# rogeliorjr/DyCON_Paper_Replication

Measured on AMD Instinct MI355X. Metric: train volumes/sec (96^3 patch), higher is better.
Workload: dtype bf16

## Files before the change

dycon_paper_replication_amd/_lib.py:

```python
from __future__ import annotations

import ctypes as C
import os

_HERE = os.path.dirname(os.path.abspath(__file__))
LIB_PATH = os.environ.get("DYCON_LIB", os.path.join(_HERE, "libdycon_hip.so"))

F32, BF16 = 0, 1
CONV_1X1, CONV_K3, CONV_K2S2 = 0, 1, 2

P, I, L, F, Z, U64 = C.c_void_p, C.c_int, C.c_longlong, C.c_float, C.c_size_t, C.c_uint64

SIGNATURES = {
    "dycon_version": (I, []),
    "dycon_last_error": (C.c_char_p, []),
    "dycon_bfrag_bytes": (Z, [I, I, I, I]),
    "dycon_pack_bfrag": (I, [P, P, I, I, I, I, I, L, L, L, L, I, P]),
    "dycon_pack_batch": (I, [P, I, I, P]),
    "dycon_pack_tcn": (I, [P, P, I, I, I, I, L, L, L, L, I, P]),
    "dycon_conv_gemm_workspace": (Z, [I, I, I, I, I, I, I, I, I]),
    "dycon_conv_gemm_plan": (I, [I, I, I, I, I, I, I, I, I, I, I, P]),
    "dycon_conv_kernel_name": (C.c_char_p, [I]),
    "dycon_conv_region_name": (C.c_char_p, [P]),
    "dycon_conv_gemm": (I, [P, P, P, P, I, I, I, I, I, I, I, I, I, I, I, P, Z, P]),
    "dycon_conv_gemm_splits": (I, [I, I, I, I, I, I, I, I, I]),
    "dycon_conv_gemm_ex": (I, [P, P, P, P, I, I, I, I, I, I, I, I, I, I, I, P, Z, I, P]),
    "dycon_conv_direct": (I, [P, I, P, P, P, I, I, I, I, I, I, I, I, I, P]),
    "dycon_conv_wgrad_workspace": (Z, [I, I, I, I, I, I, I]),
    "dycon_conv_wgrad_name": (C.c_char_p, [I, I, I, I, I, I, I, I, I]),
    "dycon_conv_wgrad": (I, [P, I, P, I, P, P, I, I, I, I, I, I, I, L, L, L, P, Z, P]),
    "dycon_colsum_workspace": (Z, [L, I]),
    "dycon_colsum": (I, [P, I, P, L, I, P, Z, P]),
    "dycon_norm_workspace": (Z, [I, L, I]),
    "dycon_norm_stats": (I, [P, I, I, L, I, I, F, P, P, P, F, P, Z, P]),
    "dycon_norm_fwd": (I, [P, P, I, I, L, I, I, F, P, P, P, I, P, P, P, P, F, P, Z, P]),
    "dycon_norm_fwd_is_fused": (I, [I, L, I, I]),
    "dycon_norm_fwd_slab": (I, [P, I, P, P, P, I, I, L, I, I, F, P, P, P, I, P, P, P]),
    "dycon_norm_apply": (I, [P, P, I, I, L, I, I, P, P, P, I, P, P, P]),
    "dycon_norm_bwd": (I, [P, I, P, P, I, I, L, I, I, P, P, P, I, P, P, P, P, Z, P]),
    "dycon_norm_bwd_ex": (I, [P, I, P, P, I, I, L, I, I, P, P, P, I, P, P, P, I, P, Z, P]),
    "dycon_norm_sum_dparams": (I, [P, I, I, P, P, P]),
    "dycon_norm_head_workspace": (Z, [I, L]),
    "dycon_norm_head_fwd": (I, [P, I, I, L, I, P, P, P, I, P, P, P, P, P]),
    "dycon_norm_head_bwd": (I, [P, P, P, I, I, L, I, P, P, P, I, P, P, P, P, P, Z, P]),
    "dycon_norm_head_dparams": (I, [P, I, L, P, P, P]),
    "dycon_norm_headc_workspace": (Z, [I, L, I]),
    "dycon_norm_headc_fwd": (I, [P, I, I, L, I, I, P, P, P, I, P, P, P, P, P]),
    "dycon_norm_headc_bwd": (I, [P, P, P, I, I, L, I, I, P, P, P, I, P, P, P, P, P, Z, P]),
    "dycon_norm_headc_dparams": (I, [P, I, L, I, P, P, P]),
    "dycon_conv_stats_chunks": (I, [I, I, I, I, I, I, I, I]),
    "dycon_conv_gemm_stats": (I, [P, P, P, P, I, I, I, I, I, I, I, P, Z, P]),
    "dycon_norm_fwd_parts": (I, [P, P, I, I, L, I, I, F, P, P, P, I, P, P, P, P, F, P, I, P]),
    "dycon_norm_stats_parts": (I, [I, I, L, I, I, F, P, P, P, F, P, I, P]),
    "dycon_norm_bwd_ab_offset": (Z, [I, L, I]),
    "dycon_norm_bwd_stats": (I, [P, P, I, I, L, I, I, P, P, P, I, P, P, P, P, Z, P]),
    "dycon_first_block_bwd_workspace": (Z, [I, I, I, I]),
    "dycon_first_block_bwd": (I, [P, P, P, I, I, I, I, I, I, P, P, P, I, P, P, P, P, P, L, L, L, P, Z, P]),
    "dycon_conv1_wgrad_normbwd_workspace": (Z, [I, I, I, I]),
    "dycon_conv1_wgrad_normbwd": (I, [P, P, P, I, I, I, I, I, I, P, P, P, I, P, P, P, P, L, L, L, P, Z, P]),
    "dycon_norm_acc_doubles": (Z, [I, L, I]),
    "dycon_norm_fwd_acc": (I, [P, P, I, I, L, I, I, F, P, P, P, I, P, P, P, P, F, P, P]),
    "dycon_norm_bwd_acc": (I, [P, P, P, I, I, L, I, I, P, P, P, I, P, P, P, P, P, Z, P]),
    "dycon_maxpool2_fwd": (I, [P, P, P, I, I, I, I, I, I, P]),
    "dycon_maxpool2_bwd": (I, [P, P, P, I, I, I, I, I, I, P]),
    "dycon_trilinear_fwd": (I, [P, P, I, I, I, I, I, I, I, I, I, I, I, I, P]),
    "dycon_trilinear_bwd": (I, [P, P, I, I, I, I, I, I, I, I, I, I, I, I, P]),
    "dycon_upconv_k3": (I, [P, P, P, P, I, I, I, I, I, I, I, P]),
    "dycon_copy_channels": (I, [P, I, I, P, I, I, L, I, I, P]),
    "dycon_relu_fwd": (I, [P, P, P, P, I, I, L, I, P]),
    "dycon_relu_bwd": (I, [P, P, P, P, I, I, L, I, P]),
    "dycon_scale_channels": (I, [P, P, P, I, I, L, I, P]),
    "dycon_mul_mask": (I, [P, P, F, P, I, L, P]),
    "dycon_dropout_philox": (I, [P, P, I, L, F, U64, U64, P]),
    "dycon_channel_mask_philox": (I, [P, L, F, U64, U64, P]),
    "dycon_add_noise": (I, [P, P, P, I, L, F, F, U64, U64, P]),
    "dycon_tanh": (I, [P, I, P, L, P]),
    "dycon_cast": (I, [P, I, P, I, L, P]),
    "dycon_add": (I, [P, P, P, I, L, P]),
    "dycon_seg_losses_fwd": (I, [P, P, P, I, I, I, L, F, P, I, P]),
    "dycon_seg_losses_bwd": (I, [P, P, P, I, I, I, L, F, P, P, I, P, I, P]),
    "dycon_seg_losses_finalize": (I, [P, I, I, L, F, P, P]),
    "dycon_step_loss": (I, [P, P, F, F, F, I, I, P, P, P]),
    "dycon_step_losses": (I, [P, P, I, I, L, F, C.c_double, F, I, F, F, F, I, I, P, P, P]),
    "dycon_seg_lossesc_nsums": (I, [I]),
    "dycon_seg_lossesc_fwd": (I, [P, P, P, I, I, I, L, I, F, I, P, I, P]),
    "dycon_seg_lossesc_bwd": (I, [P, P, P, I, I, I, L, I, F, P, P, I, P, I, P]),
    "dycon_seg_lossesc_finalize": (I, [P, I, I, L, I, F, P, P]),
    "dycon_step_lossesc": (I, [P, P, I, I, L, I, F, C.c_double, F, I, F, F, F, I, I, P, P, P]),
    "dycon_softmax_mse_fwd": (I, [P, P, P, L, I, L, I, P]),
    "dycon_softmax_mse_bwd": (I, [P, P, P, P, L, I, L, I, P]),
    "dycon_softmax_kl_fwd": (I, [P, P, L, I, L, I, P, P, P]),
    "dycon_softmax_kl_bwd": (I, [P, P, L, I, L, I, I, P, P, P]),
    "dycon_dice_fwd": (I, [P, P, I, I, L, I, L, I, P, F, P, P, P]),
    "dycon_dice_bwd": (I, [P, P, I, I, L, I, L, I, P, F, P, P, P, P]),
    "dycon_dice1_fwd": (I, [P, P, I, L, I, L, I, P, P, P]),
    "dycon_dice1_bwd": (I, [P, P, I, L, I, L, I, P, P, P, P]),
    "dycon_entropy_fwd": (I, [P, L, I, L, F, P, P, P, P]),
    "dycon_entropy_bwd": (I, [P, L, I, L, F, P, P, P, P]),
    "dycon_sym_mse_fwd": (I, [P, P, L, P, P, P]),
    "dycon_sym_mse_bwd": (I, [P, P, L, P, P, P]),
    "dycon_kl_rows_fwd": (I, [P, L, P, L, L, L, L, I, P, P, P]),
    "dycon_kl_rows_bwd": (I, [P, L, P, L, L, L, L, I, P, P, L, P]),
    "dycon_focal_fwd": (I, [P, P, I, L, I, L, F, P, I, P, P, P]),
    "dycon_focal_bwd": (I, [P, P, I, L, I, L, F, P, I, P, P, P]),
    "dycon_uncl_fwd": (I, [P, P, L, I, L, F, P, P, P]),
    "dycon_uncl_bwd": (I, [P, P, L, I, L, F, P, P, P]),
    "dycon_l2norm_fwd": (I, [P, P, P, I, L, I, F, P]),
    "dycon_l2norm_bwd": (I, [P, P, P, P, I, L, I, F, P]),
    "dycon_mask_pool": (I, [P, I, P, I, I, I, I, I, I, I, P]),
    "dycon_fecl_workspace": (Z, [I, I, I]),
    "dycon_fecl_fwd": (I, [P, P, P, P, I, I, I, I, F, F, I, F, F, P, P, P, Z, P]),
    "dycon_fecl_finalize": (I, [P, C.c_double, F, I, P, P]),
    "dycon_set_scalars": (I, [P, I, F, F, F, F, F, F, F, F, P]),
    "dycon_fecl_bwd": (I, [P, P, P, P, I, I, I, I, F, F, I, F, F, P, P, P, P, Z, P]),
    "dycon_fecl_rows_workspace": (Z, [I, I, I]),
    "dycon_fecl_fwd_rows": (I, [P, P, P, P, I, I, I, I, F, F, P, P, Z, Z, P]),
    "dycon_fecl_gambling_finalize": (I, [P, P, I, I, I, I, P, P, P, P, Z, P, Z, P]),
    "dycon_fecl_gambling_grad": (I, [P, P, L, P, P]),
    "dycon_gambling_softmax_fwd": (I, [P, P, L, I, P]),
    "dycon_gambling_softmax_bwd": (I, [P, P, P, L, I, P]),
    "dycon_gambling_uncertainty_fwd": (I, [P, I, I, I, I, I, I, I, P, I, P]),
    "dycon_gambling_uncertainty_bwd": (I, [P, I, I, I, I, I, I, I, P, P, I, P]),
    "dycon_sumsq": (I, [P, L, P, P]),
    "dycon_sgd_ema": (I, [P, P, P, P, L, L, P, F, F, F, F, F, F, P, P]),
    "dycon_nonfinite_flag": (I, [P, P, P]),
    "dycon_sw_accumulate": (I, [P, I, I, I, I, P, P, P, I, I, I, P]),
    "dycon_sw_accumulate_c": (I, [P, I, I, I, I, I, P, P, P, I, I, I, P]),
    "dycon_sw_finalize": (I, [P, P, L, F, P, P, P]),
    "dycon_binary_overlap": (I, [P, P, I, L, P, P]),
    "dycon_batch_overlap": (I, [P, P, I, I, L, P, P]),
    "dycon_sw_accumulate_all": (I, [P, I, I, I, I, I, P, P, P, I, I, I, P, P, P]),
    "dycon_sw_finalize_argmax": (I, [P, P, I, L, P, P, P]),
    "dycon_argmax_labels": (I, [P, I, L, P, P]),
    "dycon_class_confusion": (I, [P, P, I, L, I, P, P]),
    "dycon_batch_class_confusion": (I, [P, P, I, I, L, I, P, P]),
    "dycon_surface_workspace": (Z, [I, I, I, I]),
    "dycon_surface_hist": (I, [P, I, P, I, I, I, I, I, I, I, P, P, P, Z, P]),
    "dycon_surface_metrics": (I, [P, P, I, I, C.c_double, P, P]),
    "dycon_cc_workspace": (Z, [I, I, I, I]),
    "dycon_cc_roots": (I, [P, I, I, I, I, I, I, I, P, P]),
    "dycon_cc_labels": (I, [P, I, I, I, I, P, P, P, Z, P]),
    "dycon_cc_largest": (I, [P, I, P, I, I, I, I, I, P, P, P, P, Z, P]),
    "dycon_simhist_workspace": (Z, [I, I, I, I]),
    "dycon_simhist": (I, [P, P, I, I, I, I, F, I, P, P, P, P, Z, P]),
    "dycon_tap_gather": (I, [P, P, I, I, I, I, I, I, P, I, P]),
    "dycon_pack_wblocks": (I, [P, P, I, P, I, I, I, I, P, Z, I, P]),
    "dycon_unpack_wgrad": (I, [P, L, I, P, P, P, I, I, I, P]),
    "dycon_sample_colsum": (I, [P, I, P, I, L, I, F, I, P]),
    "dycon_sample_bcast": (I, [P, P, P, I, I, L, I, F, P]),
    "dycon_small_gemm": (I, [P, L, L, P, L, L, P, L, I, I, I, I, P]),
    "dycon_copy_segments": (I, [P, P, P, I, P]),
    "dycon_kernel_timing": (I, [I]),
    "dycon_kernel_timing_count": (L, []),
    "dycon_kernel_timing_fetch": (I, [L, L, P, P, P]),
    "dycon_kernel_timing_name": (C.c_char_p, [I]),
}


class ConvPlan(C.Structure):
    _fields_ = [("family", I), ("splits", I), ("chunks", I), ("weights", I), ("workspace", Z)]


CONV_NONE, CONV_C1, CONV_P16, CONV_P32, CONV_LDS, CONV_HALO, CONV_TILE, CONV_GEMM = range(8)
CONV_W_FRAG, CONV_W_CHUNK16 = 0, 1


class View(C.Structure):
    _fields_ = [("p", P), ("sn", L), ("sc", L), ("sv", L)]


class DyconLibraryError(RuntimeError):
    pass


_lib = None


def load():
    global _lib
    if _lib is not None:
        return _lib
    if not os.path.exists(LIB_PATH):
        raise DyconLibraryError(
            f"{LIB_PATH} not found: the HIP extension is not built.  Run "
            "`python -c 'import __graft_entry__ as g; g.build()'` from the repo root.  "
            "There is no CPU/PyTorch fallback for the DyCON hot path.")
    lib = C.CDLL(LIB_PATH)
    for name, (res, args) in SIGNATURES.items():
        try:
            fn = getattr(lib, name)
        except AttributeError as e:
            raise DyconLibraryError(f"{LIB_PATH} does not export {name}") from e
        fn.restype = res
        fn.argtypes = args
    _lib = lib
    return lib


class Recorder:

    def __init__(self):
        self.entries, self.keep = [], []

    def replay(self):
        for e in self.entries:
            if type(e) is list:
                rc = e[0](*e[1])
                if rc:
                    raise DyconLibraryError(f"{e[2]} failed ({rc}) in replay: {load().dycon_last_error().decode()}")
            else:
                e()


RECORDER = None

HIP_EVENT_DISABLE_TIMING, HIP_EVENT_NO_SYSTEM_FENCE = 0x2, 0x20000000
_hip = None


def hip():
    global _hip
    if _hip is None:
        h = C.CDLL("libamdhip64.so")
        h.hipEventCreateWithFlags.restype, h.hipEventCreateWithFlags.argtypes = I, [C.POINTER(P), C.c_uint]
        h.hipEventRecord.restype, h.hipEventRecord.argtypes = I, [P, P]
        h.hipStreamWaitEvent.restype, h.hipStreamWaitEvent.argtypes = I, [P, P, C.c_uint]
        h.hipEventDestroy.restype, h.hipEventDestroy.argtypes = I, [P]
        _hip = h
    return _hip


class HipEvent:
    __slots__ = ("h",)

    def __init__(self):
        ev = P()
        rc = hip().hipEventCreateWithFlags(C.byref(ev), HIP_EVENT_DISABLE_TIMING | HIP_EVENT_NO_SYSTEM_FENCE)
        if rc:
            raise DyconLibraryError(f"hipEventCreateWithFlags failed ({rc})")
        self.h = ev.value

    def __del__(self):
        try:
            if self.h and _hip is not None:
                _hip.hipEventDestroy(self.h)
        except Exception:
            pass


def hip_call(name, *args, keep=None):
    fn = getattr(hip(), name)
    rc = fn(*args)
    if rc:
        raise DyconLibraryError(f"{name} failed ({rc})")
    if RECORDER is not None:
        RECORDER.entries.append([fn, list(args), name])
        if keep is not None:
            RECORDER.keep.append(keep)


def call(name, *args):
    lib = load()
    fn = getattr(lib, name)
    rc = fn(*args)
    if rc != 0:
        raise DyconLibraryError(f"{name} failed ({rc}): {lib.dycon_last_error().decode()}")
    if RECORDER is not None:
        RECORDER.entries.append([fn, list(args), name])


_QUERY_CACHE = {}


def query(name, *args):
    key = (name,) + args
    try:
        return _QUERY_CACHE[key]
    except KeyError:
        v = _QUERY_CACHE[key] = getattr(load(), name)(*args)
        return v
```

dycon_paper_replication_amd/csrc/norm.hip:

```cpp
#include "common.h"
#include <type_traits>

struct NormPlan { int chunks; long long rows_per_chunk; };
static NormPlan norm_plan(long long V) {
    NormPlan p;
    constexpr long long maxc = 256, minr = 128;
    long long rpc = (V + maxc - 1) / maxc;
    if (rpc < minr) rpc = minr;
    p.rows_per_chunk = rpc;
    p.chunks = (int)((V + rpc - 1) / rpc);
    return p;
}

template <typename T, int MODE>
__global__ __launch_bounds__(256) void norm_partial_kernel(const T* __restrict__ S, const T* __restrict__ GY,
                                                           float* __restrict__ part, long long V, int C, int G,
                                                           long long rows_per_chunk, const float* __restrict__ stats,
                                                           const float* __restrict__ gamma, const float* __restrict__ beta,
                                                           int relu, int from_y, const float* __restrict__ chan_scale,
                                                           double* __restrict__ acc = nullptr, int nslots = 1) {
    constexpr int VN = Vec16<T>::N;
    typedef typename std::conditional<sizeof(T) == 4, double, float>::type A;
    __shared__ A sm[2][256][VN + 1];
    const int n = blockIdx.y, chunk = blockIdx.x;
// ... 417 lines not shown
            if (running_mean && gridDim.x == 1 && G == C) {
                running_mean[g] = (1.f - momentum) * running_mean[g] + momentum * (float)mean;
                const double unb = cnt > 1.0 ? var * cnt / (cnt - 1.0) : var;
                running_var[g] = (1.f - momentum) * running_var[g] + momentum * (float)unb;
            }
        }
    }
    T* yp = Y + (long long)n * V * C + c0;
    const T* sp = skip ? skip + (long long)n * V * C + c0 : nullptr;
    Vec16<T> sr[NF_ROWS][NVEC];
    if (sp) {
#pragma unroll
        for (int i = 0; i < NF_ROWS; ++i) {
            const long long v = threadIdx.x + 256 * i, vc = v < V ? v : V - 1;
#pragma unroll
            for (int q = 0; q < NVEC; ++q) sr[i][q] = ld16(sp + vc * C + q * VN);
        }
    }
#pragma unroll
    for (int i = 0; i < NF_ROWS; ++i) {
        const long long v = threadIdx.x + 256 * i;
        if (v < V) {
#pragma unroll
            for (int q = 0; q < NVEC; ++q) {
                Vec16<T> y;
#pragma unroll
                for (int k = 0; k < VN; ++k) {
                    float f = xr[i][q].get(k) * sc[q * VN + k] + sh[q * VN + k];
                    if (relu) f = f < 0.f ? 0.f : f;
                    f *= cs[q * VN + k];
                    if (sp) f += sr[i][q].get(k);
                    y.set(k, f);
                }
                st16(yp + v * C + q * VN, y);
            }
        }
    }
}

template <typename T, int SPAN, int CPG, int NF_ROWS>
__global__ __launch_bounds__(256) void norm_fused_bwd_kernel(const T* __restrict__ X, const T* __restrict__ GY, T* __restrict__ GX,
                                                             long long V, int C, int G, const float* __restrict__ stats,
                                                             const float* __restrict__ gamma, const float* __restrict__ beta,
                                                             int relu, const float* __restrict__ chan_scale,
                                                             float* __restrict__ dpart ) {
    constexpr int VN = Vec16<T>::N, NVEC = SPAN / VN;
    __shared__ float sm[4 * 2 * SPAN];
    constexpr int cpg = CPG;
    const int n = blockIdx.x, c0 = blockIdx.y * SPAN;
    const T* xp = X + (long long)n * V * C + c0;
    const T* gp = GY + (long long)n * V * C + c0;
    float mean[SPAN], rstd[SPAN], gm[SPAN], bt[SPAN], cs[SPAN];
#pragma unroll
    for (int k = 0; k < SPAN; ++k) {
        const int c = c0 + k, g = c / cpg;
        mean[k] = stats[((long long)n * G + g) * 2];
        rstd[k] = stats[((long long)n * G + g) * 2 + 1];
        gm[k] = gamma ? gamma[c] : 1.f;
        bt[k] = beta ? beta[c] : 0.f;
        cs[k] = chan_scale ? chan_scale[(long long)n * C + c] : 1.f;
    }
    float acc[2 * SPAN];
#pragma unroll
    for (int k = 0; k < 2 * SPAN; ++k) acc[k] = 0.f;
    Vec16<T> xr[NF_ROWS][NVEC], gr[NF_ROWS][NVEC];
#pragma unroll
    for (int i = 0; i < NF_ROWS; ++i) {
        const long long v = threadIdx.x + 256 * i, vc = v < V ? v : V - 1;
#pragma unroll
        for (int q = 0; q < NVEC; ++q) { xr[i][q] = ld16(xp + vc * C + q * VN); gr[i][q] = ld16(gp + vc * C + q * VN); }
    }
#pragma unroll
    for (int i = 0; i < NF_ROWS; ++i) {
        const bool ok = (long long)threadIdx.x + 256 * i < V;
#pragma unroll
        for (int q = 0; q < NVEC; ++q) {
#pragma unroll
            for (int k = 0; k < VN; ++k) {
                const int j = q * VN + k;
                const float xh = (xr[i][q].get(k) - mean[j]) * rstd[j];
                float g = gr[i][q].get(k) * cs[j];
                if ((relu && !(gm[j] * xh + bt[j] > 0.f)) || !ok) g = 0.f;
                acc[j] += g;
                acc[SPAN + j] += g * xh;
            }
        }
    }
    block_reduce_vec<2 * SPAN>(acc, sm);
    if (dpart && threadIdx.x == 0) {
#pragma unroll
        for (int k = 0; k < SPAN; ++k) {
            float* d = dpart + ((long long)n * C + c0 + k) * 2;
            d[0] = acc[k];
            d[1] = acc[SPAN + k];
        }
    }
    float A[SPAN], Bq[SPAN];
    const float inv_cnt = 1.f / ((float)V * (float)cpg);
#pragma unroll
    for (int k = 0; k < SPAN; ++k) {
        const int gl = k / cpg;
        float a = 0.f, bq = 0.f;
#pragma unroll
        for (int j = 0; j < SPAN; ++j)
            if (j / cpg == gl) { a += gm[j] * acc[j]; bq += gm[j] * acc[SPAN + j]; }
        A[k] = a * inv_cnt;
        Bq[k] = bq * inv_cnt;
    }
    T* op = GX + (long long)n * V * C + c0;
#pragma unroll
    for (int i = 0; i < NF_ROWS; ++i) {
        const long long v = threadIdx.x + 256 * i;
        if (v < V) {
#pragma unroll
            for (int q = 0; q < NVEC; ++q) {
                Vec16<T> o;
#pragma unroll
                for (int k = 0; k < VN; ++k) {
                    const int j = q * VN + k;
                    const float xh = (xr[i][q].get(k) - mean[j]) * rstd[j];
                    float g = gr[i][q].get(k) * cs[j];
                    if (relu && !(gm[j] * xh + bt[j] > 0.f)) g = 0.f;
                    o.set(k, rstd[j] * (gm[j] * g - (A[j] + xh * Bq[j])));
                }
                st16(op + v * C + q * VN, o);
            }
        }
    }
}

__global__ void norm_sum_dparams_kernel(const float* __restrict__ dpart, int Nb, int C, float* dgamma, float* dbeta) {
    const int c = blockIdx.x * blockDim.x + threadIdx.x;
    if (c >= C) return;
    float s0 = 0.f, s1 = 0.f;
    for (int n = 0; n < Nb; ++n) { s0 += dpart[((long long)n * C + c) * 2]; s1 += dpart[((long long)n * C + c) * 2 + 1]; }
    if (dbeta) dbeta[c] = s0;
    if (dgamma) dgamma[c] = s1;
}

static bool norm_fused_ok(int dtype, long long V, int C, int G) {
    const int VN = dtype == DYCON_BF16 ? 8 : 4, cpg = C / G;
    const int span = cpg > VN ? cpg : VN;
    return V <= 2048 && (cpg & (cpg - 1)) == 0 && cpg <= 16 && C % span == 0 && (span == 4 || span == 8 || span == 16);
}

extern "C" size_t dycon_norm_workspace(int Nb, long long V, int C) {
    const NormPlan p = norm_plan(V);
    return ((size_t)Nb * p.chunks * C * 2 + (size_t)Nb * C * 2 + 64) * sizeof(float);
}

static int norm_check(const char* who, int dtype, int Nb, long long V, int C, int G) {
    const int VN = dtype == DYCON_BF16 ? 8 : 4;
    DYCON_REQUIRE(Nb > 0 && V > 0 && C > 0 && G > 0 && C % G == 0, "%s: bad shape Nb=%d V=%lld C=%d G=%d", who, Nb, V, C, G);
    DYCON_REQUIRE(C % VN == 0 && C / VN <= 256, "%s: C=%d must be a multiple of %d and <= %d", who, C, VN, 256 * VN);
    DYCON_REQUIRE(Nb <= 65535, "%s: Nb too large", who);
    return DYCON_OK;
}

extern "C" int dycon_norm_fwd_is_fused(int dtype, long long V, int C, int G) {
    return (G > 0 && C % G == 0 && norm_fused_ok(dtype, V, C, G)) ? 1 : 0;
}

extern "C" int dycon_norm_fwd_slab(const float* slab, int splits, const float* conv_bias, void* x_out, void* y, int dtype, int Nb,
                                   long long V, int C, int G, float eps, float* stats, const float* gamma, const float* beta,
                                   int relu, const void* skip, const float* chan_scale, dycon_stream_t stream) {
    DYCON_REQUIRE(slab && x_out && y && stats && splits > 0, "norm_fwd_slab: bad arguments");
    DYCON_REQUIRE(dtype == DYCON_BF16, "norm_fwd_slab: bf16 storage only");
    if (int e = norm_check("norm_fwd_slab", dtype, Nb, V, C, G)) return e;
    DYCON_REQUIRE(norm_fused_ok(dtype, V, C, G), "norm_fwd_slab: this shape is not served by the one-launch norm (ask dycon_norm_fwd_is_fused)");
    const int cpg = C / G, span = cpg > 8 ? cpg : 8;
    const long long MN = (long long)Nb * V * C;
    dim3 grid(Nb, C / span);
#define DYCON_NFS_(SP, CP, RW) norm_fused_fwd_kernel<bf16, SP, CP, true, RW><<<grid, 256, 0, stream>>>((bf16*)x_out, (bf16*)y, V, C, G, eps, stats, gamma, beta, relu, (const bf16*)skip, chan_scale, nullptr, nullptr, 0.f, slab, splits, MN, conv_bias)
#define DYCON_NFS(SP, CP) do { if (V <= 256) DYCON_NFS_(SP, CP, 1); else DYCON_NFS_(SP, CP, 8); } while (0)
    if (cpg == 1) DYCON_NFS(8, 1); else if (cpg == 2) DYCON_NFS(8, 2); else if (cpg == 4) DYCON_NFS(8, 4);
    else if (cpg == 8) DYCON_NFS(8, 8); else DYCON_NFS(16, 16);
#undef DYCON_NFS
#undef DYCON_NFS_
    DYCON_LAUNCH_CHECK();
    return DYCON_OK;
}

extern "C" int dycon_norm_stats(const void* x, int dtype, int Nb, long long V, int C, int G, float eps, float* stats,
                                float* running_mean, float* running_var, float momentum, float* workspace, size_t ws_bytes,
                                dycon_stream_t stream) {
    DYCON_REQUIRE(x && stats && workspace, "norm_stats: null pointer");
    if (int e = norm_check("norm_stats", dtype, Nb, V, C, G)) return e;
    DYCON_REQUIRE(ws_bytes >= dycon_norm_workspace(Nb, V, C), "norm_stats: workspace too small");
    const NormPlan p = norm_plan(V);
    dim3 grid(p.chunks, Nb);
    DYCON_DISPATCH(dtype, {
        norm_partial_kernel<T, 0><<<grid, 256, 0, stream>>>((const T*)x, nullptr, workspace, V, C, G, p.rows_per_chunk, nullptr,
                                                            nullptr, nullptr, 0, 0, nullptr);
    });
    DYCON_LAUNCH_CHECK();
    norm_finalize_stats_kernel<<<Nb * G, 256, 0, stream>>>(workspace, Nb, p.chunks, C, G, V, eps, stats, running_mean, running_var, momentum);
    DYCON_LAUNCH_CHECK();
    return DYCON_OK;
}

extern "C" int dycon_norm_fwd(const void* x, void* y, int dtype, int Nb, long long V, int C, int G, float eps, float* stats,
                              const float* gamma, const float* beta, int relu, const void* skip, const float* chan_scale,
                              float* running_mean, float* running_var, float momentum, float* workspace, size_t ws_bytes,
                              dycon_stream_t stream) {
    DYCON_REQUIRE(x && y && stats, "norm_fwd: null pointer");
    if (int e = norm_check("norm_fwd", dtype, Nb, V, C, G)) return e;
    if (norm_fused_ok(dtype, V, C, G)) {
        const int VN = dtype == DYCON_BF16 ? 8 : 4, cpg = C / G;
        const int span = cpg > VN ? cpg : VN;
        dim3 grid(Nb, C / span);
#define DYCON_NF_(TT, SP, CP, RW) norm_fused_fwd_kernel<TT, SP, CP, false, RW><<<grid, 256, 0, stream>>>((TT*)const_cast<void*>(x), (TT*)y, V, C, G, eps, stats, gamma, beta, relu, (const TT*)skip, chan_scale, running_mean, running_var, momentum, nullptr, 0, 0, nullptr)
#define DYCON_NF(TT, SP, CP) do { if (V <= 256) DYCON_NF_(TT, SP, CP, 1); else DYCON_NF_(TT, SP, CP, 8); } while (0)
        if (dtype == DYCON_BF16) {
            if (cpg == 1) DYCON_NF(bf16, 8, 1); else if (cpg == 2) DYCON_NF(bf16, 8, 2); else if (cpg == 4) DYCON_NF(bf16, 8, 4);
            else if (cpg == 8) DYCON_NF(bf16, 8, 8); else DYCON_NF(bf16, 16, 16);
        } else {
            if (cpg == 1) DYCON_NF(float, 4, 1); else if (cpg == 2) DYCON_NF(float, 4, 2); else if (cpg == 4) DYCON_NF(float, 4, 4);
            else if (cpg == 8) DYCON_NF(float, 8, 8); else DYCON_NF(float, 16, 16);
        }
#undef DYCON_NF
#undef DYCON_NF_
        DYCON_LAUNCH_CHECK();
        return DYCON_OK;
    }
    DYCON_REQUIRE(workspace, "norm_fwd: workspace missing");
    if (int e = dycon_norm_stats(x, dtype, Nb, V, C, G, eps, stats, running_mean, running_var, momentum, workspace, ws_bytes, stream)) return e;
    return dycon_norm_apply(x, y, dtype, Nb, V, C, G, stats, gamma, beta, relu, skip, chan_scale, stream);
}

static int apply_grid(long long V, int C, int VN) {
    constexpr long long vpt = 4, cap = 2048;
    long long blocks = (V * C / VN + 256 * vpt - 1) / (256 * vpt);
    if (blocks > cap) blocks = cap;
    if (blocks < 1) blocks = 1;
    return (int)blocks;
}

extern "C" int dycon_norm_apply(const void* x, void* y, int dtype, int Nb, long long V, int C, int G, const float* stats,
                                const float* gamma, const float* beta, int relu, const void* skip, const float* chan_scale,
                                dycon_stream_t stream) {
    DYCON_REQUIRE(x && y && stats, "norm_apply: null pointer");
    if (int e = norm_check("norm_apply", dtype, Nb, V, C, G)) return e;
    DYCON_DISPATCH(dtype, {
        dim3 grid(apply_grid(V, C, Vec16<T>::N), Nb);
        norm_apply_kernel<T, false><<<grid, 256, 3 * C * sizeof(float), stream>>>((const T*)x, (T*)y, V, C, G, stats, gamma, beta, relu,
                                                                                  (const T*)skip, chan_scale);
    });
    DYCON_LAUNCH_CHECK();
    return DYCON_OK;
}

extern "C" int dycon_norm_fwd_parts(const void* x, void* y, int dtype, int Nb, long long V, int C, int G, float eps, float* stats,
                                    const float* gamma, const float* beta, int relu, const void* skip, const float* chan_scale,
                                    float* running_mean, float* running_var, float momentum, const float* part, int chunks,
                                    dycon_stream_t stream) {
    DYCON_REQUIRE(x && y && stats && part && chunks > 0, "norm_fwd_parts: bad arguments");
    if (int e = norm_check("norm_fwd_parts", dtype, Nb, V, C, G)) return e;
    norm_finalize_stats_kernel<<<Nb * G, 256, 0, stream>>>(part, Nb, chunks, C, G, V, eps, stats, running_mean, running_var, momentum);
    DYCON_LAUNCH_CHECK();
    return dycon_norm_apply(x, y, dtype, Nb, V, C, G, stats, gamma, beta, relu, skip, chan_scale, stream);
}

extern "C" int dycon_norm_stats_parts(int dtype, int Nb, long long V, int C, int G, float eps, float* stats, float* running_mean,
                                      float* running_var, float momentum, const float* part, int chunks, dycon_stream_t stream) {
    DYCON_REQUIRE(stats && part && chunks > 0, "norm_stats_parts: bad arguments");
    if (int e = norm_check("norm_stats_parts", dtype, Nb, V, C, G)) return e;
    norm_finalize_stats_kernel<<<Nb * G, 256, 0, stream>>>(part, Nb, chunks, C, G, V, eps, stats, running_mean, running_var, momentum);
    DYCON_LAUNCH_CHECK();
    return DYCON_OK;
}

extern "C" int dycon_norm_bwd(const void* src, int from_y, const void* gy, void* gx, int dtype, int Nb, long long V, int C,
                              int G, const float* stats, const float* gamma, const float* beta, int relu,
                              const float* chan_scale, float* dgamma, float* dbeta, float* workspace, size_t ws_bytes,
                              dycon_stream_t stream) {
    return dycon_norm_bwd_ex(src, from_y, gy, gx, dtype, Nb, V, C, G, stats, gamma, beta, relu, chan_scale, dgamma, dbeta, 0, workspace,
                             ws_bytes, stream);
}

extern "C" size_t dycon_norm_bwd_ab_offset(int Nb, long long V, int C) {
    const NormPlan p = norm_plan(V);
    return (size_t)Nb * p.chunks * C * 2;
}
extern "C" int dycon_norm_bwd_stats(const void* src, const void* gy, int dtype, int Nb, long long V, int C, int G, const float* stats,
                                    const float* gamma, const float* beta, int relu, const float* chan_scale, float* dgamma,
                                    float* dbeta, float* workspace, size_t ws_bytes, dycon_stream_t stream) {
    DYCON_REQUIRE(src && gy && stats && workspace, "norm_bwd_stats: null pointer");
    if (int e = norm_check("norm_bwd_stats", dtype, Nb, V, C, G)) return e;
    DYCON_REQUIRE(ws_bytes >= dycon_norm_workspace(Nb, V, C), "norm_bwd_stats: workspace too small");
    const NormPlan p = norm_plan(V);
    float* ab = workspace + dycon_norm_bwd_ab_offset(Nb, V, C);
    dim3 grid(p.chunks, Nb);
    DYCON_DISPATCH(dtype, {
        norm_partial_kernel<T, 1><<<grid, 256, 0, stream>>>((const T*)src, (const T*)gy, workspace, V, C, G, p.rows_per_chunk,
                                                            stats, gamma, beta, relu, 0, chan_scale);
    });
    DYCON_LAUNCH_CHECK();
    const int nfin = Nb * G + ((dgamma || dbeta) ? C : 0);
    norm_finalize_bwd_kernel<<<nfin, 256, 0, stream>>>(workspace, Nb, p.chunks, C, G, gamma, ab, dgamma, dbeta);
    DYCON_LAUNCH_CHECK();
    return DYCON_OK;
}

extern "C" int dycon_norm_sum_dparams(const float* workspace, int Nb, int C, float* dgamma, float* dbeta, dycon_stream_t stream) {
    DYCON_REQUIRE(workspace && Nb > 0 && C > 0 && (dgamma || dbeta), "norm_sum_dparams: bad arguments");
    norm_sum_dparams_kernel<<<cdiv(C, 256), 256, 0, stream>>>(workspace, Nb, C, dgamma, dbeta);
    DYCON_LAUNCH_CHECK();
    return DYCON_OK;
}

extern "C" int dycon_norm_bwd_ex(const void* src, int from_y, const void* gy, void* gx, int dtype, int Nb, long long V, int C,
                                 int G, const float* stats, const float* gamma, const float* beta, int relu,
                                 const float* chan_scale, float* dgamma, float* dbeta, int defer_dparams, float* workspace,
                                 size_t ws_bytes, dycon_stream_t stream) {
    DYCON_REQUIRE(src && gy && gx && stats && workspace, "norm_bwd: null pointer");
    if (int e = norm_check("norm_bwd", dtype, Nb, V, C, G)) return e;
    DYCON_REQUIRE(ws_bytes >= dycon_norm_workspace(Nb, V, C), "norm_bwd: workspace too small");
    if (!from_y && norm_fused_ok(dtype, V, C, G)) {
        const int VN = dtype == DYCON_BF16 ? 8 : 4, cpg = C / G;
        const int span = cpg > VN ? cpg : VN;
        const bool want = dgamma || dbeta;
        dim3 grid(Nb, C / span);
#define DYCON_NB_(TT, SP, CP, RW) norm_fused_bwd_kernel<TT, SP, CP, RW><<<grid, 256, 0, stream>>>((const TT*)src, (const TT*)gy, (TT*)gx, V, C, G, stats, gamma, beta, relu, chan_scale, want ? workspace : nullptr)
#define DYCON_NB(TT, SP, CP) do { if (V <= 256) DYCON_NB_(TT, SP, CP, 1); else DYCON_NB_(TT, SP, CP, 8); } while (0)
        if (dtype == DYCON_BF16) {
            if (cpg == 1) DYCON_NB(bf16, 8, 1); else if (cpg == 2) DYCON_NB(bf16, 8, 2); else if (cpg == 4) DYCON_NB(bf16, 8, 4);
            else if (cpg == 8) DYCON_NB(bf16, 8, 8); else DYCON_NB(bf16, 16, 16);
        } else {
            if (cpg == 1) DYCON_NB(float, 4, 1); else if (cpg == 2) DYCON_NB(float, 4, 2); else if (cpg == 4) DYCON_NB(float, 4, 4);
            else if (cpg == 8) DYCON_NB(float, 8, 8); else DYCON_NB(float, 16, 16);
        }
#undef DYCON_NB
#undef DYCON_NB_
        DYCON_LAUNCH_CHECK();
        if (want && !defer_dparams) {
            norm_sum_dparams_kernel<<<cdiv(C, 256), 256, 0, stream>>>(workspace, Nb, C, dgamma, dbeta);
            DYCON_LAUNCH_CHECK();
        }
        return DYCON_OK;
    }
    const NormPlan p = norm_plan(V);
    float* ab = workspace + (size_t)Nb * p.chunks * C * 2;
    dim3 grid(p.chunks, Nb);
    DYCON_DISPATCH(dtype, {
        norm_partial_kernel<T, 1><<<grid, 256, 0, stream>>>((const T*)src, (const T*)gy, workspace, V, C, G, p.rows_per_chunk,
                                                            stats, gamma, beta, relu, from_y, chan_scale);
    });
    DYCON_LAUNCH_CHECK();
    const int nfin = Nb * G + ((dgamma || dbeta) ? C : 0);
    norm_finalize_bwd_kernel<<<nfin, 256, 0, stream>>>(workspace, Nb, p.chunks, C, G, gamma, ab, dgamma, dbeta);
    DYCON_LAUNCH_CHECK();
    DYCON_DISPATCH(dtype, {
        dim3 grid2(apply_grid(V, C, Vec16<T>::N), Nb);
        norm_bwd_apply_kernel<T, false><<<grid2, 256, 7 * C * sizeof(float), stream>>>((const T*)src, (const T*)gy, (T*)gx, V, C, G, stats,
                                                                                       gamma, beta, ab, relu, from_y, chan_scale);
    });
    DYCON_LAUNCH_CHECK();
    return DYCON_OK;
}

constexpr int HC = 16;
constexpr int HK_MAX = 8;
constexpr int hpart_len(int hk) { return hk * HC + hk; }

template <typename T> __device__ __forceinline__ float round_to(float v) { T t; stf(&t, v); return ldf(&t); }

template <int HK> __device__ __forceinline__ void ld_row(const float* __restrict__ p, float (&r)[HK]) {
    if constexpr (HK % 4 == 0) {
#pragma unroll
        for (int k = 0; k < HK; k += 4) {
            const float4 t = *reinterpret_cast<const float4*>(p + k);
            r[k] = t.x; r[k + 1] = t.y; r[k + 2] = t.z; r[k + 3] = t.w;
        }
    } else if constexpr (HK % 2 == 0) {
#pragma unroll
        for (int k = 0; k < HK; k += 2) {
            const float2 t = *reinterpret_cast<const float2*>(p + k);
            r[k] = t.x; r[k + 1] = t.y;
        }
    } else {
#pragma unroll
        for (int k = 0; k < HK; ++k) r[k] = p[k];
    }
}
template <int HK> __device__ __forceinline__ void st_row(float* __restrict__ p, const float (&r)[HK]) {
    if constexpr (HK % 4 == 0) {
#pragma unroll
        for (int k = 0; k < HK; k += 4) *reinterpret_cast<float4*>(p + k) = make_float4(r[k], r[k + 1], r[k + 2], r[k + 3]);
    } else if constexpr (HK % 2 == 0) {
#pragma unroll
        for (int k = 0; k < HK; k += 2) *reinterpret_cast<float2*>(p + k) = make_float2(r[k], r[k + 1]);
    } else {
#pragma unroll
        for (int k = 0; k < HK; ++k) p[k] = r[k];
    }
}

template <typename T, int HK>
__device__ __forceinline__ void norm_apply_head_body(const T* __restrict__ X, long long V, int G, const float* __restrict__ stats,
                                                     const float* __restrict__ gamma, const float* __restrict__ beta, int relu,
                                                     const float* __restrict__ chan_scale, const float* __restrict__ W,
                                                     const float* __restrict__ hb, float* __restrict__ L) {
    constexpr int VN = Vec16<T>::N;
    __shared__ float ss[3 * HC + HK * HC + HK];
    const int n = blockIdx.y, cpg = HC / G;
    if (threadIdx.x < HC) {
        const int c = threadIdx.x, g = c / cpg;
        const float mean = stats[((long long)n * G + g) * 2], rstd = stats[((long long)n * G + g) * 2 + 1];
        const float gm = gamma ? gamma[c] : 1.f, bt = beta ? beta[c] : 0.f;
        ss[c] = rstd * gm;
        ss[HC + c] = bt - mean * rstd * gm;
        ss[2 * HC + c] = chan_scale ? chan_scale[(long long)n * HC + c] : 1.f;
    }
    if (threadIdx.x < HK * HC) ss[3 * HC + threadIdx.x] = W[threadIdx.x];
    if (threadIdx.x < HK) ss[3 * HC + HK * HC + threadIdx.x] = hb ? hb[threadIdx.x] : 0.f;
    __syncthreads();
    constexpr bool WREG = HK == 1;
    float sc[HC], sh[HC], dr[HC], wr[WREG ? HK * HC : 1], hbias[HK];
#pragma unroll
    for (int c = 0; c < HC; ++c) { sc[c] = ss[c]; sh[c] = ss[HC + c]; dr[c] = ss[2 * HC + c]; }
    if constexpr (WREG) {
#pragma unroll
        for (int j = 0; j < HK * HC; ++j) wr[j] = ss[3 * HC + j];
    }
#pragma unroll
    for (int k = 0; k < HK; ++k) hbias[k] = ss[3 * HC + HK * HC + k];
    const float* wl = ss + 3 * HC;
    const T* xp = X + (long long)n * V * HC;
    float* lp = L + (long long)n * V * HK;
    for (long long v = (long long)blockIdx.x * 256 + threadIdx.x; v < V; v += (long long)gridDim.x * 256) {
        float o[HK];
#pragma unroll
        for (int k = 0; k < HK; ++k) o[k] = hbias[k];
#pragma unroll
        for (int c0 = 0; c0 < HC; c0 += VN) {
            const Vec16<T> x = ld16(xp + v * HC + c0);
#pragma unroll
            for (int k = 0; k < VN; ++k) {
                const int c = c0 + k;
                float y = x.get(k) * sc[c] + sh[c];
                if (relu) y = y < 0.f ? 0.f : y;
                y = round_to<T>(y * dr[c]);
#pragma unroll
                for (int kk = 0; kk < HK; ++kk) o[kk] = fmaf(y, WREG ? wr[WREG ? kk * HC + c : 0] : wl[kk * HC + c], o[kk]);
            }
        }
        st_row<HK>(lp + v * HK, o);
    }
}
template <typename T, int HK>
__global__ __launch_bounds__(256) void norm_apply_headc_kernel(const T* __restrict__ X, long long V, int G,
                                                               const float* __restrict__ stats, const float* __restrict__ gamma,
                                                               const float* __restrict__ beta, int relu,
                                                               const float* __restrict__ chan_scale, const float* __restrict__ W,
                                                               const float* __restrict__ hb, float* __restrict__ L) {
    norm_apply_head_body<T, HK>(X, V, G, stats, gamma, beta, relu, chan_scale, W, hb, L);
}

template <typename T, int HK>
__device__ __forceinline__ void norm_head_partial_body(const T* __restrict__ S, const float* __restrict__ GL, float* __restrict__ part,
                                                       float* __restrict__ hpart, long long V, int G, long long rows_per_chunk,
                                                       const float* __restrict__ stats, const float* __restrict__ gamma,
                                                       const float* __restrict__ beta, int relu, const float* __restrict__ chan_scale,
                                                       const float* __restrict__ W) {
    constexpr int VN = Vec16<T>::N;
    constexpr int NGRP = HC / VN, RPI = 256 / NGRP;
    constexpr int NQ = 2 + HK;
    constexpr int NR = NQ < 4 ? NQ : 4;
    constexpr int HPART = hpart_len(HK);
    constexpr bool WREG = HK == 1;
    __shared__ float sm[NR][256][VN + 1];
    __shared__ float sb[256][HK];
    __shared__ float sw[WREG ? 1 : HK * HC];
    const int n = blockIdx.y, chunk = blockIdx.x;
    const int cg = threadIdx.x % NGRP, rr = threadIdx.x / NGRP;
    const long long v0 = chunk * rows_per_chunk, v1 = min(V, v0 + rows_per_chunk);
    const int cpg = HC / G;
    if constexpr (!WREG) {
        if (threadIdx.x < HK * HC) sw[threadIdx.x] = W[threadIdx.x];
        __syncthreads();
    }
    float acc[NQ][VN], e[HK];
    float mean[VN], rstd[VN], gm[VN], bt[VN], cs[VN], sc[VN], sh[VN], wr[WREG ? HK : 1][VN];
#pragma unroll
    for (int kk = 0; kk < HK; ++kk) e[kk] = 0.f;
#pragma unroll
    for (int k = 0; k < VN; ++k) {
        const int c = cg * VN + k, g = c / cpg;
#pragma unroll
        for (int q = 0; q < NQ; ++q) acc[q][k] = 0.f;
        cs[k] = chan_scale ? chan_scale[(long long)n * HC + c] : 1.f;
        mean[k] = stats[((long long)n * G + g) * 2];
        rstd[k] = stats[((long long)n * G + g) * 2 + 1];
        gm[k] = gamma ? gamma[c] : 1.f;
        bt[k] = beta ? beta[c] : 0.f;
        sc[k] = rstd[k] * gm[k];
        sh[k] = bt[k] - mean[k] * rstd[k] * gm[k];
        if constexpr (WREG) {
#pragma unroll
            for (int kk = 0; kk < HK; ++kk) wr[kk][k] = W[kk * HC + c];
        }
    }
    const float* wl = sw + cg * VN;
    const T* sp = S + ((long long)n * V) * HC + cg * VN;
    const float* gp = GL + (long long)n * V * HK;
    for (long long v = v0 + rr; v < v1; v += RPI) {
        const Vec16<T> s = ld16(sp + v * HC);
        float gl[HK];
        ld_row<HK>(gp + v * HK, gl);
#pragma unroll
        for (int k = 0; k < VN; ++k) {
            float gyv = 0.f;
#pragma unroll
            for (int kk = 0; kk < HK; ++kk) gyv = fmaf(gl[kk], WREG ? wr[WREG ? kk : 0][k] : wl[kk * HC + k], gyv);
            float g = round_to<T>(gyv) * cs[k];
            const float x = s.get(k);
            const float xh = (x - mean[k]) * rstd[k];
            if (relu && !(gm[k] * xh + bt[k] > 0.f)) g = 0.f;
            acc[0][k] += g;
            acc[1][k] += g * xh;
            float y = x * sc[k] + sh[k];
            if (relu) y = y < 0.f ? 0.f : y;
            y = round_to<T>(y * cs[k]);
#pragma unroll
            for (int kk = 0; kk < HK; ++kk) acc[2 + kk][k] += gl[kk] * y;
        }
        if (cg == 0) {
#pragma unroll
            for (int kk = 0; kk < HK; ++kk) e[kk] += gl[kk];
        }
    }
#pragma unroll
    for (int kk = 0; kk < HK; ++kk) sb[threadIdx.x][kk] = e[kk];
    const long long item = (long long)n * gridDim.x + chunk;
#pragma unroll
    for (int r0 = 0; r0 < NQ; r0 += NR) {
        if (r0) __syncthreads();
#pragma unroll
        for (int j = 0; j < NR; ++j) {
            if (r0 + j < NQ) {
#pragma unroll
                for (int k = 0; k < VN; ++k) sm[j][threadIdx.x][k] = acc[r0 + j < NQ ? r0 + j : 0][k];
            }
        }
        __syncthreads();
        if (threadIdx.x < NR * HC) {
            const int j = threadIdx.x / HC, o = threadIdx.x % HC, og = o / VN, ok = o % VN, q = r0 + j;
            if (q < NQ) {
                float s0 = 0.f;
                for (int i = 0; i < RPI; ++i) s0 += sm[j][i * NGRP + og][ok];
                if (q < 2) part[((item * HC) + o) * 2 + q] = s0;
                else hpart[item * HPART + (q - 2) * HC + o] = s0;
            }
        } else if (r0 == 0 && threadIdx.x >= 128 && threadIdx.x < 128 + HK) {
            const int kk = threadIdx.x - 128;
            float s0 = 0.f;
            for (int i = 0; i < 256; ++i) s0 += sb[i][kk];
            hpart[item * HPART + HK * HC + kk] = s0;
        }
    }
}
template <typename T, int HK>
__global__ __launch_bounds__(256) void norm_head_partialc_kernel(const T* __restrict__ S, const float* __restrict__ GL,
                                                                 float* __restrict__ part, float* __restrict__ hpart, long long V,
                                                                 int G, long long rows_per_chunk, const float* __restrict__ stats,
                                                                 const float* __restrict__ gamma, const float* __restrict__ beta,
                                                                 int relu, const float* __restrict__ chan_scale,
                                                                 const float* __restrict__ W) {
    norm_head_partial_body<T, HK>(S, GL, part, hpart, V, G, rows_per_chunk, stats, gamma, beta, relu, chan_scale, W);
}

__global__ __launch_bounds__(256) void norm_headc_finalize_kernel(const float* __restrict__ hpart, int items, int hk,
                                                                 float* __restrict__ dW, float* __restrict__ db) {
    const int j = blockIdx.x, hpart_n = hpart_len(hk);
    double s0 = 0.0, s1 = 0.0;
    for (int e = threadIdx.x; e < items; e += 256) s0 += hpart[(long long)e * hpart_n + j];
    block_sum2_double(s0, s1);
    if (threadIdx.x == 0) {
        if (j < hk * HC) { if (dW) dW[j] = (float)s0; }
        else if (db) db[j - hk * HC] = (float)s0;
    }
}

template <typename T, int HK>
__device__ __forceinline__ void norm_head_bwd_apply_body(const T* __restrict__ S, const float* __restrict__ GL, T* __restrict__ GX,
                                                         long long V, int G, const float* __restrict__ stats,
                                                         const float* __restrict__ gamma, const float* __restrict__ beta,
                                                         const float* __restrict__ ab, int relu, const float* __restrict__ chan_scale,
                                                         const float* __restrict__ W) {
    constexpr int VN = Vec16<T>::N;
    constexpr int NGRP = HC / VN;
    constexpr bool WREG = HK == 1;
    __shared__ float sw[WREG ? 1 : HK * HC];
    if constexpr (!WREG) {
        if (threadIdx.x < HK * HC) sw[threadIdx.x] = W[threadIdx.x];
        __syncthreads();
    }
    const int n = blockIdx.y, cpg = HC / G;
    const float inv_cnt = 1.f / ((float)V * (float)cpg);
    const long long total = V * NGRP;
    const int cg = threadIdx.x % NGRP;
    float mu[VN], rs[VN], gmv[VN], btv[VN], pa[VN], pb[VN], dr[VN], wr[WREG ? HK : 1][VN];
#pragma unroll
    for (int k = 0; k < VN; ++k) {
        const int c = cg * VN + k, g = c / cpg;
        mu[k] = stats[((long long)n * G + g) * 2];
// ... 428 lines not shown
```

dycon_paper_replication_amd/engine.py:

```python
from __future__ import annotations

from collections import OrderedDict
from typing import Dict, Optional

import torch

from . import ops
from ._lib import CONV_1X1, CONV_C1, CONV_K2S2, CONV_K3, CONV_W_CHUNK16

UNET_FILTERS = (16, 32, 64, 128, 256)
VNET_NORMS = ("groupnorm", "instancenorm", "batchnorm", "none")


def _projection_spec(spec, c_in):
    spec["projection.0.weight"] = (512, c_in, 1, 1, 1)
    spec["projection.0.bias"] = (512,)
    spec["projection.1.weight"] = (512,)
    spec["projection.1.bias"] = (512,)
    spec["projection.3.weight"] = (256, 512, 1, 1, 1)
    spec["projection.3.bias"] = (256,)
    spec["projection.4.weight"] = (256,)
    spec["projection.4.bias"] = (256,)


def projection_buffers():
    return OrderedDict([("projection.1.running_mean", (512,)), ("projection.1.running_var", (512,)),
                        ("projection.1.num_batches_tracked", ()), ("projection.4.running_mean", (256,)),
                        ("projection.4.running_var", (256,)), ("projection.4.num_batches_tracked", ())])


def vnet_param_spec(in_ch=1, n_classes=2, normalization="groupnorm", nf=16):
    if normalization not in VNET_NORMS:
        raise ValueError(f"normalization must be one of {VNET_NORMS}")
    spec = OrderedDict()
    affine = normalization in ("groupnorm", "batchnorm")
    step = 2 if normalization == "none" else 3

    def block(name, n, cin, cout):
        for i in range(n):
            ci = cin if i == 0 else cout
            spec[f"{name}.conv.{step * i}.weight"] = (cout, ci, 3, 3, 3)
            spec[f"{name}.conv.{step * i}.bias"] = (cout,)
            if affine:
                spec[f"{name}.conv.{step * i + 1}.weight"] = (cout,)
                spec[f"{name}.conv.{step * i + 1}.bias"] = (cout,)

    def down(name, cin, cout):
        spec[f"{name}.conv.0.weight"] = (cout, cin, 2, 2, 2)
        spec[f"{name}.conv.0.bias"] = (cout,)
        if affine:
            spec[f"{name}.conv.1.weight"] = (cout,)
            spec[f"{name}.conv.1.bias"] = (cout,)

    def up(name, cin, cout):
        spec[f"{name}.conv.0.weight"] = (cin, cout, 2, 2, 2)
        spec[f"{name}.conv.0.bias"] = (cout,)
        if affine:
            spec[f"{name}.conv.1.weight"] = (cout,)
            spec[f"{name}.conv.1.bias"] = (cout,)

    block("block_one", 1, in_ch, nf); down("block_one_dw", nf, 2 * nf)
    block("block_two", 2, 2 * nf, 2 * nf); down("block_two_dw", 2 * nf, 4 * nf)
    block("block_three", 3, 4 * nf, 4 * nf); down("block_three_dw", 4 * nf, 8 * nf)
    block("block_four", 3, 8 * nf, 8 * nf); down("block_four_dw", 8 * nf, 16 * nf)
    block("block_five", 3, 16 * nf, 16 * nf); up("block_five_up", 16 * nf, 8 * nf)
    block("block_six", 3, 8 * nf, 8 * nf); up("block_six_up", 8 * nf, 4 * nf)
    block("block_seven", 3, 4 * nf, 4 * nf); up("block_seven_up", 4 * nf, 2 * nf)
    block("block_eight", 2, 2 * nf, 2 * nf); up("block_eight_up", 2 * nf, nf)
    block("block_nine", 1, nf, nf)
    spec["out_conv.weight"] = (n_classes, nf, 1, 1, 1)
    spec["out_conv.bias"] = (n_classes,)
    _projection_spec(spec, 16 * nf)
    return spec


def vnet_norm_sites(normalization="groupnorm"):
    if normalization == "none":
        return []
    sites = []
    for blk, n, nxt in (("block_one", 1, "block_one_dw"), ("block_two", 2, "block_two_dw"), ("block_three", 3, "block_three_dw"),
                        ("block_four", 3, "block_four_dw"), ("block_five", 3, "block_five_up"), ("block_six", 3, "block_six_up"),
                        ("block_seven", 3, "block_seven_up"), ("block_eight", 2, "block_eight_up"), ("block_nine", 1, None)):
        sites += [f"{blk}.conv.{3 * i + 1}" for i in range(n)]
        if nxt:
            sites.append(f"{nxt}.conv.1")
    return sites


ASPP_BN_SITES = tuple(f"aspp.aspp{j}.bn" for j in range(1, 5)) + ("aspp.bn_after_pool", "aspp.bn1")


def net_buffers(net_type, normalization="groupnorm", params=None):
    bufs = OrderedDict()
    if net_type == "vnet" and normalization == "batchnorm":
        spec = params if params is not None else vnet_param_spec(normalization=normalization)
        for site in vnet_norm_sites(normalization):
            c = tuple(spec[site + ".weight"])
            bufs[site + ".running_mean"], bufs[site + ".running_var"], bufs[site + ".num_batches_tracked"] = c, c, ()
    if net_type == "unet_3D" and params is not None and "aspp.conv1.weight" in params:
        for site in ASPP_BN_SITES:
            c = tuple(params[site + ".weight"])
            bufs[site + ".running_mean"], bufs[site + ".running_var"], bufs[site + ".num_batches_tracked"] = c, c, ()
    bufs.update(projection_buffers())
    return bufs


def aspp_param_spec(spec, c=256):
    for j, k in ((1, 1), (2, 3), (3, 3), (4, 3)):
        spec[f"aspp.aspp{j}.atrous_conv.weight"] = (c, c, k, k, k)
        spec[f"aspp.aspp{j}.bn.weight"] = (c,)
        spec[f"aspp.aspp{j}.bn.bias"] = (c,)
    spec["aspp.global_avg_pool.1.weight"] = (c, c, 1, 1, 1)
    spec["aspp.bn_after_pool.weight"] = (c,)
    spec["aspp.bn_after_pool.bias"] = (c,)
    spec["aspp.conv1.weight"] = (c, 5 * c, 1, 1, 1)
    spec["aspp.bn1.weight"] = (c,)
    spec["aspp.bn1.bias"] = (c,)


def unet_param_spec(in_ch=1, n_classes=2, use_aspp=False):
    spec = OrderedDict()
    f = UNET_FILTERS

    def uc(prefix, cin, cout):
        spec[f"{prefix}.conv1.0.weight"] = (cout, cin, 3, 3, 3)
        spec[f"{prefix}.conv1.0.bias"] = (cout,)
        spec[f"{prefix}.conv2.0.weight"] = (cout, cout, 3, 3, 3)
        spec[f"{prefix}.conv2.0.bias"] = (cout,)

    uc("conv1", in_ch, f[0]); uc("conv2", f[0], f[1]); uc("conv3", f[1], f[2]); uc("conv4", f[2], f[3])
    uc("center", f[3], f[4])
    uc("up_concat4.conv", f[4] + f[3], f[3]); uc("up_concat3.conv", f[3] + f[2], f[2])
    uc("up_concat2.conv", f[2] + f[1], f[1]); uc("up_concat1.conv", f[1] + f[0], f[0])
    spec["final.weight"] = (n_classes, f[0], 1, 1, 1)
    spec["final.bias"] = (n_classes,)
    spec["out_conv2.weight"] = (n_classes, f[0], 1, 1, 1)
    spec["out_conv2.bias"] = (n_classes,)
    if use_aspp:
        aspp_param_spec(spec, f[4])
    _projection_spec(spec, f[4])
    return spec


def param_spec(net_type, in_ch=1, n_classes=2, normalization="groupnorm", use_aspp=False):
    if net_type == "vnet":
        if use_aspp:
            raise ValueError("use_aspp applies to the U-Net only (the reference's VNet takes no use_aspp)")
        return vnet_param_spec(in_ch, n_classes, normalization)
    if net_type == "unet_3D":
        return unet_param_spec(in_ch, n_classes, use_aspp)
    raise ValueError(f"unknown net_type {net_type!r}")


class DropoutSpec:

    def __init__(self, mode="off", masks=None, seed=0, offset=0):
        self.mode, self.masks, self.seed, self.offset = mode, masks or {}, seed, offset


class Engine:
    def __init__(self, net_type: str, params: Dict[str, torch.Tensor], grads: Optional[Dict[str, torch.Tensor]] = None,
                 buffers: Optional[Dict[str, torch.Tensor]] = None, dtype=torch.float32, scale_factor=2,
                 normalization="groupnorm"):
        if net_type == "vnet" and normalization not in VNET_NORMS:
            raise ValueError(f"normalization must be one of {VNET_NORMS} (VNet.py:17-24)")
        self.net_type, self.p, self.g, self.buf = net_type, params, grads, buffers or {}
        self.dtype, self.scale_factor, self.normalization = dtype, scale_factor, normalization
        self.gen = 0
        self._packed = {}
        self._jobs, self._jobs_dev, self._packed_gen = [], None, -1
        self._xjobs = []
        self.use_aspp = net_type == "unet_3D" and "aspp.conv1.weight" in params
        self._aspp_plans = {}
        self._jobs_split, self._pack_event = False, None
        self.on_param_grads = None
        self.wgrad_stream = None
        self.wgrad_stream2 = None
        self._wg_flip = 0
        self.feat_stream = None
        self.mark = None
        self.Gs = {}
        self._head_range = (0, 0)
        self._wws = {}
        self.fuse_finish = False
        self.conv_stats = False
        self.conv_stats96 = False
        self._stat_parts = {}
        self._deferred = {}
        self._pending_dparams = []
        self.tape = []
        self.G = {}

    def params_changed(self):
        self.gen += 1

    def _pk(self, key, kind, w, T, Cin, N, N0, s_t, s_c, s_n1, s_n0, flip=False):
        hit = self._packed.get(key)
        if hit is not None and hit[0] == self.gen:
            return hit[1]
        buf = hit[1] if hit is not None else None
        if kind == "frag":
            buf = ops.pack_bfrag(w, self.dtype, T, Cin, N, N0, s_t, s_c, s_n1, s_n0, flip, out=buf)
            code = 0 if self.dtype == torch.bfloat16 else 1
        else:
            buf = ops.pack_tcn(w, T, Cin, N, N0, s_t, s_c, s_n1, s_n0, flip, out=buf)
            code = 2
        if hit is None:
            self._jobs.append((key, ops.pack_job(w, buf, code, T, Cin, N, N0, s_t, s_c, s_n1, s_n0, flip)))
            self._jobs_dev = None
        self._packed[key] = (self.gen, buf)
        return buf

    def _pk_chunked16(self, key, w, nchunks, N, s_t, s_c, s_n0, flip=False):
        hit = self._packed.get(key)
        if hit is not None and hit[0] == self.gen:
            return hit[1]
        per = ops.query("dycon_bfrag_bytes", ops.BF16, 27, 16, N) // 2
        buf = hit[1] if hit is not None else torch.empty(per * nchunks, dtype=torch.bfloat16, device=w.device)
        wflat = w.reshape(-1)
        for ch in range(nchunks):
            src, dst = wflat[ch * 16 * s_c:], buf[ch * per:(ch + 1) * per]
            ops.pack_bfrag(src, self.dtype, 27, 16, N, N, s_t, s_c, 0, s_n0, flip, out=dst)
            if hit is None:
                self._jobs.append(((key, ch), ops.pack_job(src, dst, 0, 27, 16, N, N, s_t, s_c, 0, s_n0, flip)))
                self._jobs_dev = None
        self._packed[key] = (self.gen, buf)
        return buf

    def repack(self, early=None, helper=None):
        self._pack_event = None
        if (not self._jobs and not self._xjobs) or self._packed_gen == self.gen:
            return
        split = early is not None and helper is not None
        if self._jobs_dev is None or self._jobs_split != split:
            dev = next(iter(self._packed.values()))[1].device
            name = lambda key: (key[0][0] if isinstance(key[0], tuple) else key[0])
            first = [j for k, j in self._jobs if split and name(k).startswith(early)]
            rest = [j for k, j in self._jobs if not (split and name(k).startswith(early))]
            self._jobs_dev = [(ops.upload_pack_jobs(js, dev), len(js), max(1, min(512, (max(j[6] for j in js) + 2047) // 2048)))
                              for js in (first, rest) if js]
            self._jobs_split = split
        if split and len(self._jobs_dev) == 2:
            (d0, n0, b0), (d1, n1, b1) = self._jobs_dev
            ops.pack_batch(d0, n0, b0)
            ops.fork(ops.cur_stream(), helper)
            with ops.on_stream(helper, light=True):
                ops.pack_batch(d1, n1, b1)
                self._repack_blocks()
                ev1 = ops.Event()
                ev1.record(helper)
            self._pack_event = ev1
        else:
            for d, n, b in self._jobs_dev:
                ops.pack_batch(d, n, b)
            self._repack_blocks()
        for key, _ in self._jobs:
            key = key[0] if isinstance(key[0], tuple) else key
            self._packed[key] = (self.gen, self._packed[key][1])
        self._packed_gen = self.gen

    def _pk_blocks(self, key, tables, KB, NB, kblk, nblk, device):
        hit = self._packed.get(key)
        if hit is not None and hit[0] == self.gen:
            return hit[1]
        buf = ops.pack_wblocks(tables, KB, NB, kblk, nblk, self.dtype, device, out=hit[1] if hit is not None else None)
        if hit is None:
            self._xjobs.append((key, tables, KB, NB, kblk, nblk))
        self._packed[key] = (self.gen, buf)
        return buf

    def _repack_blocks(self):
        for key, tables, KB, NB, kblk, nblk in self._xjobs:
            buf = self._packed[key][1]
            ops.pack_wblocks(tables, KB, NB, kblk, nblk, self.dtype, buf.device, out=buf)
            self._packed[key] = (self.gen, buf)

    def pack_ready(self):
        ev = getattr(self, "_pack_event", None)
        if ev is not None:
            ev.wait(ops.cur_stream())
            self._pack_event = None

    def _sync_to(self, key, g):
        if self.feat_stream is None:
            return
        cur = ops.cur_stream()
        src = self.Gs.get(key)
        if src is not None and src != cur:
            ops.fork(src, cur)
            g.record_stream(cur)

    def _take(self, t):
        g = self.G.pop(id(t))
        self._sync_to(id(t), g)
        self.Gs.pop(id(t), None)
        return g

    def _peek(self, t):
        g = self.G.get(id(t))
        if g is not None:
            self._sync_to(id(t), g)
        return g

    def _put(self, t, g):
        self.G[id(t)] = g
        if self.feat_stream is not None:
            self.Gs[id(t)] = ops.cur_stream()

    def _give(self, t, g):
        cur = self._peek(t)
        self._put(t, g if cur is None else ops.add(cur, g))

    def _conv(self, name, x, kind, need_gx=True, out_dtype=None, norm_groups=0):
        w, b = self.p[name + ".weight"], self.p[name + ".bias"]
        dtype = self.dtype
        if kind == "deconv":
            Cin, Cout = w.shape[0], w.shape[1]
        else:
            Cout, Cin = w.shape[0], w.shape[1]
        T = {"k3": 27, "k2s2": 8, "deconv": 8, "1x1": 1}[kind]
        mode = {"k3": CONV_K3, "k2s2": CONV_K2S2, "deconv": CONV_1X1, "1x1": CONV_1X1}[kind]
        gq = 8 if dtype == torch.bfloat16 else 4
        skinny = (Cin % gq != 0) or (Cout % 16 != 0)
        out_dtype = out_dtype or dtype
        plan = ops.conv_plan_for(x, mode, Cout, Cout) if kind == "k3" and out_dtype == dtype else None
        first_lds = plan is not None and plan.family == CONV_C1

        def conv_with_stats(wf, want):
            chunks = plan.chunks if (norm_groups and want) else 0
            if not chunks:
                return None
            y, part = ops.conv_gemm_stats(x, wf, b, Cout, chunks)
            self._stat_parts[id(y)] = (part, chunks)
            return y

        if first_lds:
            wf = self._pk((name, "f1"), "frag", w, 27, 1, Cout, Cout, 1, 27, 0, 27)
            y = conv_with_stats(wf, self.conv_stats96 and Cout == 16)
            if y is None:
                y = ops.conv_gemm(x, wf, b, CONV_K3, Cout, Cout)
        elif skinny:
            assert kind in ("k3", "1x1"), "skinny path only for the first conv and the 1x1 heads"
            wt = self._pk((name, "tcn"), "tcn", w, T, Cin, Cout, Cout, 1, T, 0, Cin * T)
            y = ops.conv_direct(x, wt, b, mode, Cout, out_dtype)
        elif kind == "deconv":
            wf = self._pk((name, "f"), "frag", w, 1, Cin, 8 * Cout, Cout, 0, Cout * 8, 1, 8)
            y = ops.conv_gemm(x, wf, b, CONV_1X1, 8 * Cout, Cout, scatter=True)
        elif plan is not None and plan.weights == CONV_W_CHUNK16:
            wf = self._pk_chunked16((name, "f48"), w, 3, Cout, 1, 27, Cin * 27)
            y = ops.conv_gemm(x, wf, b, mode, Cout, Cout)
        else:
            wf = self._pk((name, "f"), "frag", w, T, Cin, Cout, Cout, 1, T, 0, Cin * T)
            Vo = (x.shape[1] * x.shape[2] * x.shape[3]) // (8 if kind == "k2s2" else 1)
            want_stats = self.conv_stats96 if (Cin, Cout) == (16, 16) else self.conv_stats
            y = conv_with_stats(wf, want_stats and kind == "k3" and out_dtype == dtype and dtype == torch.bfloat16)
            if y is None and (norm_groups and self.fuse_finish and dtype == torch.bfloat16 and out_dtype == dtype
                              and ops.norm_fwd_is_fused(x, Vo, Cout, norm_groups)):
                y, dc = ops.conv_gemm(x, wf, b, mode, Cout, Cout, defer_finish=True)
                if dc is not None:
                    self._deferred[id(y)] = dc
            elif y is None:
                y = ops.conv_gemm(x, wf, b, mode, Cout, Cout)

        if self.recording:
            def wgrad(gy):
                gw, gb = self.g[name + ".weight"], self.g[name + ".bias"]
                wkey = (name, tuple(x.shape[:4]))
                ws = self._wws.get(wkey)
                if kind == "deconv":
                    if ws is None:
                        ws = self._wws[wkey] = (ops._ws(ops.query("dycon_colsum_workspace", gy.numel() // gy.shape[-1], gy.shape[-1]), gy),
                                                ops.conv_wgrad_workspace(gy, x, CONV_K2S2))
                    ops.colsum(gy, gb, ws=ws[0])
                    ops.conv_wgrad(gy, x, gw, CONV_K2S2, 1, 8, Cout * 8, ws=ws[1])
                else:
                    if ws is None:
                        ws = self._wws[wkey] = ops.conv_wgrad_workspace(x, gy, mode)
                    ops.conv_wgrad(x, gy, gw, mode, 1 if T > 1 else 0, T, Cin * T, dbias=gb, ws=ws)
                if self.on_param_grads is not None:
                    self.on_param_grads(name + ".weight")

            def bwd():
                gy = self._take(y)
                if self.wgrad_stream is not None:
                    wst = self.wgrad_stream
                    if self.wgrad_stream2 is not None:
                        self._wg_flip = (self._wg_flip + 1) % 2
                        wst = (self.wgrad_stream, self.wgrad_stream2)[self._wg_flip]
                    ops.fork(ops.cur_stream(), wst)
                    with ops.on_stream(wst, light=True):
                        self._flush_dparams()
                        wgrad(gy)
                    gy.record_stream(wst)
                else:
                    wgrad(gy)
                if not need_gx:
                    return
                cur = self._peek(x)
                if skinny:
                    wd = self._pk((name, "tcn_d"), "tcn", w, 1, Cout, Cin, Cin, 0, Cin, 0, 1)
                    gx = ops.conv_direct(gy, wd, None, CONV_1X1, Cin, x.dtype, out=cur, accumulate=cur is not None)
                elif kind == "k3":
                    if ops.conv_plan_for(gy, CONV_K3, Cin, Cin).weights == CONV_W_CHUNK16:
                        wd = self._pk_chunked16((name, "d48"), w, 3, Cin, 1, Cin * 27, 27, flip=True)
                    else:
                        wd = self._pk((name, "d"), "frag", w, 27, Cout, Cin, Cin, 1, Cin * 27, 0, 27, flip=True)
                    gx = ops.conv_gemm(gy, wd, None, CONV_K3, Cin, Cin, out=cur, accumulate=cur is not None)
                elif kind == "k2s2":
                    wd = self._pk((name, "d"), "frag", w, 1, Cout, 8 * Cin, Cin, 0, Cin * 8, 1, 8)
                    gx = ops.conv_gemm(gy, wd, None, CONV_1X1, 8 * Cin, Cin, scatter=True, out=cur, accumulate=cur is not None)
                elif kind == "deconv":
                    wd = self._pk((name, "d"), "frag", w, 8, Cout, Cin, Cin, 1, 8, 0, Cout * 8)
                    gx = ops.conv_gemm(gy, wd, None, CONV_K2S2, Cin, Cin, out=cur, accumulate=cur is not None)
                else:
                    wd = self._pk((name, "d"), "frag", w, 1, Cout, Cin, Cin, 0, Cin, 0, 1)
                    gx = ops.conv_gemm(gy, wd, None, CONV_1X1, Cin, Cin, out=cur, accumulate=cur is not None)
                self._put(x, gx)
            self.tape.append(bwd)
        return y

    def _flush_dparams(self):
        for pend in self._pending_dparams:
            ops.norm_sum_dparams(pend)
            pend[0].record_stream(ops.cur_stream())
        self._pending_dparams = []

    def _norm_site(self, prefix, z, kind):
        B, C = z.shape[0], z.shape[-1]
        V = z.numel() // (B * C)
        if kind == "in":
            return B, V, C, C, None, None, None, None
        if kind not in ("gn", "bn"):
            raise ValueError(kind)
        gamma, beta = self.p[prefix + ".weight"], self.p[prefix + ".bias"]
        if kind == "gn":
            return B, V, C, 16, gamma, beta, None, None
        return 1, B * V, C, C, gamma, beta, self.buf.get(prefix + ".running_mean"), self.buf.get(prefix + ".running_var")

    @staticmethod
    def _eval_stats(rm, rv):
        return torch.stack([rm, torch.rsqrt(rv + 1e-5)], 1).reshape(-1).contiguous()

    def _count_batch(self, prefix):
        nbt = self.buf.get(prefix + ".num_batches_tracked")
        if nbt is not None:
            ops.rec(lambda: nbt.add_(1))

    def _norm(self, prefix, z, kind, relu=True, skip=None, training=True, chan_scale=None):
        if kind == "bn" and chan_scale is not None:
            y = self._norm(prefix, z, kind, relu=relu, skip=skip, training=training)
            y2 = ops.scale_channels(y, chan_scale)
            if self.recording:
                def bwd_scale():
                    self._give(y, ops.scale_channels(self._take(y2), chan_scale))
                self.tape.append(bwd_scale)
            return y2
        if kind == "none":
            assert relu
            y = ops.relu_fwd(z, skip, chan_scale)
            if self.recording:
                def bwd_relu():
                    gy = self._take(y)
                    if skip is not None:
                        self._give(skip, gy)
                    self._give(z, ops.relu_bwd(z, gy, chan_scale))
                self.tape.append(bwd_relu)
            return y
        Nb, V, C, G, gamma, beta, rm, rv = self._norm_site(prefix, z, kind)
        if kind == "bn" and not training:
            stats = self._eval_stats(rm, rv)
            y = ops.norm_apply(z, stats, Nb, V, C, G, gamma, beta, relu, skip, chan_scale=chan_scale)
        elif id(z) in self._stat_parts and kind in ("gn", "in"):
            part, chunks = self._stat_parts.pop(id(z))
            y, stats = ops.norm_fwd_parts(z, part, chunks, Nb, V, C, G, gamma, beta, relu, skip, chan_scale)
        elif id(z) in self._deferred:
            y, stats = ops.norm_fwd_slab(z, self._deferred.pop(id(z)), Nb, V, C, G, gamma, beta, relu, skip, chan_scale)
        else:
            upd = kind == "bn" and training and self.update_bn
            y, stats = ops.norm_fwd(z, Nb, V, C, G, gamma, beta, relu, skip, chan_scale, 1e-5, rm if upd else None,
                                    rv if upd else None, 0.1)
            if upd:
                self._count_batch(prefix)
        if self.recording:
            def bwd():
                gy = self._take(y)
                if skip is not None:
                    self._give(skip, gy)
                dg = self.g[prefix + ".weight"] if gamma is not None else None
                db = self.g[prefix + ".bias"] if beta is not None else None
                if self.wgrad_stream is not None and dg is not None:
                    gz, pend = ops.norm_bwd(z, False, gy, stats, Nb, V, C, G, gamma, beta, relu, dg, db, chan_scale=chan_scale,
                                            defer_dparams=True)
                    if pend is not None:
                        self._pending_dparams.append(pend)
                else:
                    gz = ops.norm_bwd(z, False, gy, stats, Nb, V, C, G, gamma, beta, relu, dg, db, chan_scale=chan_scale)
                if self.on_param_grads is not None and gamma is not None:
                    self.on_param_grads(prefix + ".weight")
                self._give(z, gz)
            self.tape.append(bwd)
        return y

    def _first_block(self, name, x, kind, training):
        cname, nname = f"{name}.conv.0", f"{name}.conv.1"
        rec, self.recording = self.recording, False
        try:
            z = self._conv(cname, x, "k3", need_gx=False, norm_groups=(16 if kind == "gn" else (16 if kind == "in" else 0)))
        finally:
            self.recording = rec
        Nb, V, C, G, gamma, beta, rm, rv = self._norm_site(nname, z, kind)
        upd = kind == "bn" and training and self.update_bn
        if id(z) in self._stat_parts and kind in ("gn", "in"):
            part, chunks = self._stat_parts.pop(id(z))
            y, stats = ops.norm_fwd_parts(z, part, chunks, Nb, V, C, G, gamma, beta, True, None, None)
        else:
            self._stat_parts.pop(id(z), None)
            y, stats = ops.norm_fwd(z, Nb, V, C, G, gamma, beta, True, None, None, 1e-5, rm if upd else None, rv if upd else None, 0.1)
        if upd:
            self._count_batch(nname)
        if rec:
            def bwd():
                gy = self._take(y)
                dg = self.g[nname + ".weight"] if gamma is not None else None
                db = self.g[nname + ".bias"] if beta is not None else None
                gw, gb = self.g[cname + ".weight"], self.g[cname + ".bias"]
                wws = self._wws.get((cname, "#fb", tuple(x.shape[:4])))
                if wws is None:
                    wws = self._wws[(cname, "#fb", tuple(x.shape[:4]))] = ops._ws(ops.query("dycon_first_block_bwd_workspace", *x.shape[:4]), x)
                ops.first_block_bwd(x, z, gy, stats, Nb, G, gw, gb, gamma, beta, True, dg, db, None, ws=wws)
                if self.on_param_grads is not None:
                    if gamma is not None:
                        self.on_param_grads(nname + ".weight")
                    self.on_param_grads(cname + ".weight")
            self.tape.append(bwd)
        return y

    def _norm_head(self, prefix, z, kind, head, training=True, chan_scale=None):
        Nb, V, C, G, gamma, beta, rm, rv = self._norm_site(prefix, z, kind)
        hw, hb = self.p[head + ".weight"], self.p[head + ".bias"]
        if kind == "bn" and not training:
            self._stat_parts.pop(id(z), None)
            stats = self._eval_stats(rm, rv)
        elif id(z) in self._stat_parts and kind in ("gn", "in"):
            part, chunks = self._stat_parts.pop(id(z))
            stats = ops.norm_stats_parts(z, part, chunks, Nb, V, C, G)
        else:
            self._stat_parts.pop(id(z), None)
            upd = kind == "bn" and training and self.update_bn
            stats = ops.norm_stats(z, Nb, V, C, G, 1e-5, rm if upd else None, rv if upd else None, 0.1)
            if upd:
                self._count_batch(prefix)
        logits = ops.norm_head_fwd(z, stats, Nb, V, G, hw, hb, gamma, beta, True, chan_scale)
        if self.recording:
            def bwd():
                gl = self._take(logits)
                dg = self.g[prefix + ".weight"] if gamma is not None else None
                db = self.g[prefix + ".bias"] if beta is not None else None
                gz, pend = ops.norm_head_bwd(z, gl, stats, Nb, V, G, hw, gamma, beta, True, dg, db, chan_scale)
                gw, gb = self.g[head + ".weight"], self.g[head + ".bias"]
                if self.wgrad_stream is not None:
                    ops.fork(ops.cur_stream(), self.wgrad_stream)
                    with ops.on_stream(self.wgrad_stream, light=True):
                        ops.norm_head_dparams(pend, gw, gb)
                    pend[0].record_stream(self.wgrad_stream)
                else:
                    ops.norm_head_dparams(pend, gw, gb)
                if self.on_param_grads is not None:
                    self.on_param_grads(head + ".weight")
                    if gamma is not None:
                        self.on_param_grads(prefix + ".weight")
                self._give(z, gz)
            self.tape.append(bwd)
        return logits

    def _channel_scale(self, B, C, key, p, site, device):
        d = self.dropout
        if d.mode == "off":
            return None
        if d.mode == "mask":
            m = d.masks.get(key)
            if m is None:
                return None
            return (m.to(torch.float32) / (1.0 - p)).contiguous().reshape(-1)
        return ops.channel_mask_philox(B * C, p, d.seed, d.offset + site * (1 << 20), device)

    def _drop_elements(self, x, key, p, site):
        d = self.dropout
        if d.mode == "off":
            return x
        if d.mode == "mask":
            m = d.masks.get(key)
            if m is None:
                return x
            f = lambda t: ops.mul_mask(t, m, 1.0 / (1.0 - p))
        else:
            off = d.offset + site * (1 << 40)
            f = lambda t: ops.dropout_philox(t, p, d.seed, off)
        y = f(x)
        if self.recording:
            def bwd():
                self._give(x, f(self._take(y)))
            self.tape.append(bwd)
        return y

    def _aspp_tables(self, dhw):
        key = tuple(dhw)
        t = self._aspp_plans.get(key)
        if t is None:
            import ctypes as C
            from .aspp import ASPP_BRANCHES, TapPlan
            plan = TapPlan(dhw, ASPP_BRANCHES)
            ws = [self.p[f"aspp.aspp{j}.atrous_conv.weight"] for j in range(1, 5)]
            c = ws[0].shape[0]
            t = {"plan": plan, "fwd": plan.fwd_tables(ws, c), "dgrad": plan.dgrad_tables(ws, c), "c": c, "gkey": None}
            dev = ws[0].device
            t["aff"] = aff = torch.empty(16 * c, dtype=torch.float32, device=dev)
            t["dgb"] = dgb = torch.empty(8 * c, dtype=torch.float32, device=dev)
            sites = [f"aspp.aspp{j}.bn" for j in range(1, 5)]

            def segs(pairs):
                return (ops.host_array(C.c_void_p, [a.data_ptr() for a, _ in pairs]),
                        ops.host_array(C.c_void_p, [b.data_ptr() for _, b in pairs]),
                        ops.host_array(C.c_int, [a.numel() for a, _ in pairs]), len(pairs))
            gather = []
            for q, leaf in enumerate((".weight", ".bias")):
                gather += [(self.p[sj + leaf], aff[(4 * q + j) * c:(4 * q + j + 1) * c]) for j, sj in enumerate(sites)]
            stats = []
            if all(sj + ".running_mean" in self.buf for sj in sites):
                for q, leaf in enumerate((".running_mean", ".running_var")):
                    stats += [(self.buf[sj + leaf], aff[(8 + 4 * q + j) * c:(8 + 4 * q + j + 1) * c]) for j, sj in enumerate(sites)]
            t["gather"] = segs(gather + stats)
            if stats:
                t["scatter_stats"] = segs([(b, a) for a, b in stats])
            t["segs"] = segs
            self._aspp_plans[key] = t
        return t

    def _aspp_grad_tables(self, t):
        wn = [f"aspp.aspp{j}.atrous_conv.weight" for j in range(1, 5)]
        bn = [f"aspp.aspp{j}.bn{leaf}" for leaf in (".weight", ".bias") for j in range(1, 5)]
        gs = [self.g[n] for n in wn + bn]
        key = tuple(g.data_ptr() for g in gs)
        if t["gkey"] != key:
            c, dgb = t["c"], t["dgb"]
            t["unpack"] = t["plan"].unpack_tables(gs[:4])
            t["scatter_dgb"] = t["segs"]([(dgb[i * c:(i + 1) * c], g) for i, g in enumerate(gs[4:])])
            t["gkey"] = key

    def _aspp(self, x, training):
        B, d, h, w, c = x.shape
        V, M = d * h * w, B * d * h * w
        t = self._aspp_tables((d, h, w))
        plan, NB = t["plan"], 4
        N = NB * c
        dev, f32 = x.device, dict(dtype=torch.float32, device=x.device)
        upd = training and self.update_bn
        wf = self._pk_blocks(("aspp", "f", (d, h, w)), t["fwd"], plan.KB, NB, c, c, dev)
        a = x if plan.KB == 1 else ops.tap_gather(x, plan.taps_host, plan.KB)
        z = ops.conv_gemm(a, wf, None, CONV_1X1, N, N)
        aff = t["aff"]
        ops.copy_segments(t["gather"])
        gam, bet, rm, rv = aff[:N], aff[N:2 * N], aff[2 * N:3 * N], aff[3 * N:]
        if training:
            ybr, st = ops.norm_fwd(z, 1, M, N, N, gam, bet, True, None, None, 1e-5, rm if upd else None, rv if upd else None, 0.1)
            if upd and "scatter_stats" in t:
                ops.copy_segments(t["scatter_stats"])
                for j in range(1, 5):
                    self._count_batch(f"aspp.aspp{j}.bn")
        else:
            st = self._eval_stats(rm, rv)
            ybr = ops.norm_apply(z, st, 1, M, N, N, gam, bet, True)
        wp, wc1 = self.p["aspp.global_avg_pool.1.weight"], self.p["aspp.conv1.weight"]
        wc1_pool = wc1.reshape(-1)[N:]
        v = ops.sample_colsum(x, torch.empty((B, c), **f32), 1.0 / V)
        zp = ops.small_gemm(v, 1, c, wp, 1, c, torch.empty((B, c), **f32), c, B, c, c)
        pool_bn = B > 1
        if pool_bn:
            pg, pb_ = self.p["aspp.bn_after_pool.weight"], self.p["aspp.bn_after_pool.bias"]
            prm, prv = self.buf.get("aspp.bn_after_pool.running_mean"), self.buf.get("aspp.bn_after_pool.running_var")
            if training:
                pv, pst = ops.norm_fwd(zp, 1, B, c, c, pg, pb_, True, None, None, 1e-5, prm if upd else None, prv if upd else None, 0.1)
                if upd:
                    self._count_batch("aspp.bn_after_pool")
            else:
                pst = self._eval_stats(prm, prv)
                pv = ops.norm_apply(zp, pst, 1, B, c, c, pg, pb_, True)
        else:
            pv = ops.relu_fwd(zp)
        bias = ops.small_gemm(pv, 1, c, wc1_pool, 1, 5 * c, torch.empty((B, c), **f32), c, B, c, c)
        wc1f = self._pk(("aspp.conv1", "f"), "frag", wc1, 1, N, c, c, 0, 1, 0, 5 * c)
        z1 = ops.conv_gemm(ybr, wc1f, None, CONV_1X1, c, c)
        ops.sample_bcast(z1, bias, z1)
        if self.recording:
            def bwd():
                gz1 = self._take(z1)
                g = self.g
                self._flush_dparams()
                self._aspp_grad_tables(t)
                wc1d = self._pk(("aspp.conv1", "d"), "frag", wc1, 1, c, N, N, 0, 5 * c, 0, 1)
                gbr = ops.conv_gemm(gz1, wc1d, None, CONV_1X1, N, N)
                ops.conv_wgrad(ybr, gz1, g["aspp.conv1.weight"], CONV_1X1, 0, 1, 5 * c)
                gbias = ops.sample_colsum(gz1, torch.empty((B, c), **f32), 1.0)
                gw1p = g["aspp.conv1.weight"].reshape(-1)[N:]
                ops.small_gemm(gbias, c, 1, pv, c, 1, gw1p, 5 * c, c, c, B)
                gpv = ops.small_gemm(gbias, 1, c, wc1_pool, 5 * c, 1, torch.empty((B, c), **f32), c, B, c, c)
                if pool_bn:
                    gzp = ops.norm_bwd(zp, False, gpv, pst, 1, B, c, c, pg, pb_, True, g["aspp.bn_after_pool.weight"],
                                       g["aspp.bn_after_pool.bias"])
                else:
                    gzp = ops.relu_bwd(zp, gpv)
                ops.small_gemm(gzp, c, 1, v, c, 1, g["aspp.global_avg_pool.1.weight"], c, c, c, B)
                gv = ops.small_gemm(gzp, 1, c, wp, c, 1, torch.empty((B, c), **f32), c, B, c, c)
                dgb = t["dgb"]
                gz = ops.norm_bwd(z, False, gbr, st, 1, M, N, N, gam, bet, True, dgb[:N], dgb[N:])
                ops.copy_segments(t["scatter_dgb"])
                dense = torch.empty(plan.KB * c * N, **f32)
                ops.conv_wgrad(a, gz, dense, CONV_1X1, 0, N, 1)
                ops.unpack_wgrad(dense, N, plan.KB, t["unpack"], c, c)
                wd = self._pk_blocks(("aspp", "d", (d, h, w)), t["dgrad"], plan.KB * NB, 1, c, c, dev)
                ag = gz if plan.KB == 1 else ops.tap_gather(gz, plan.neg_taps_host, plan.KB)
                gx = ops.conv_gemm(ag, wd, None, CONV_1X1, c, c)
                ops.sample_bcast(gx, gv, gx, 1.0 / V)
                if self.on_param_grads is not None:
                    names = ["aspp.bn1.weight", "aspp.conv1.weight"]
                    names += (["aspp.bn_after_pool.weight"] if pool_bn else []) + ["aspp.global_avg_pool.1.weight"]
                    for j in range(4, 0, -1):
                        names += [f"aspp.aspp{j}.bn.weight", f"aspp.aspp{j}.atrous_conv.weight"]
                    for n in names:
                        self.on_param_grads(n)
                self._give(x, gx)
            self.tape.append(bwd)
        y = self._norm("aspp.bn1", z1, "bn", relu=True, training=training)
        return self._drop_elements(y, "drop_aspp", 0.5, 2)

    def _head(self, center, training):
        if self.use_aspp:
            center = self._aspp(center, training)
        B, d, h, w, C = center.shape
        s = self.scale_factor
        c = ops.trilinear_fwd(center, (d * s, h * s, w * s), True)
        if self.recording:
            def bwd():
                self._give(center, ops.trilinear_bwd(self._take(c), center.shape, True))
            self.tape.append(bwd)
        hdn = self._conv("projection.0", c, "1x1")
        hdn = self._norm("projection.1", hdn, "bn", relu=True, training=training)
        out = self._conv("projection.3", hdn, "1x1")
        return self._norm("projection.4", out, "bn", relu=False, training=training)

    def _mark_ready(self):
        if self.feat_stream is None:
            return None
        ev = ops.Event()
        ev.record(ops.cur_stream())
        return ev

    def _head_branch(self, center, ready, training):
        h0 = len(self.tape)
        if self.feat_stream is None:
            feats = self._head(center, training)
        else:
            with ops.on_stream(self.feat_stream):
                ready.wait(self.feat_stream)
                feats = self._head(center, training)
            center.record_stream(self.feat_stream)
        self._head_range = (h0, len(self.tape))
        return feats

    def _fuses_first_block(self, x, nk, training):
        w1 = self.p["block_one.conv.0.weight"]
        return (self.dtype == torch.bfloat16 and nk != "none" and not (nk == "bn" and not training)
                and w1.shape[0] == 16 and w1.shape[1] == 1 and x.shape[0] <= 16)

    def _vnet(self, x, training):
        nk = {"groupnorm": "gn", "instancenorm": "in", "batchnorm": "bn", "none": "none"}[self.normalization]
        st = 2 if nk == "none" else 3

        def ngroups(t, conv):
            return 16 if nk == "gn" else (self.p[conv + ".weight"].shape[0] if nk == "in" else 0)

        def block(name, t, n, first=False, drop=None):
            for i in range(n):
                t = self._conv(f"{name}.conv.{st * i}", t, "k3", need_gx=not (first and i == 0), norm_groups=ngroups(t, f"{name}.conv.{st * i}"))
                cs = None
                if drop is not None and i == n - 1:
                    cs = self._channel_scale(t.shape[0], t.shape[-1], drop[0], 0.5, drop[1], t.device)
                t = self._norm(f"{name}.conv.{st * i + 1}", t, nk, chan_scale=cs, training=training)
            return t

        def down(name, t):
            return self._norm(f"{name}.conv.1", self._conv(f"{name}.conv.0", t, "k2s2", norm_groups=ngroups(t, f"{name}.conv.0")), nk,
                              training=training)

        def up(name, t, skip):
            return self._norm(f"{name}.conv.1", self._conv(f"{name}.conv.0", t, "deconv"), nk, skip=skip, training=training)

        if self._fuses_first_block(x, nk, training):
            x1 = self._first_block("block_one", x, nk, training)
        else:
            x1 = block("block_one", x, 1, first=True)
        self.pack_ready()
        x2 = block("block_two", down("block_one_dw", x1), 2)
        x3 = block("block_three", down("block_two_dw", x2), 3)
        x4 = block("block_four", down("block_three_dw", x3), 3)
        x5 = block("block_five", down("block_four_dw", x4), 3, drop=("drop5", 0))
        x5_ready = self._mark_ready()
        u = up("block_five_up", x5, x4)
        u = up("block_six_up", block("block_six", u, 3), x3)
        u = up("block_seven_up", block("block_seven", u, 3), x2)
        u = up("block_eight_up", block("block_eight", u, 2), x1)
        w9, wo = self.p["block_nine.conv.0.weight"], self.p["out_conv.weight"]
        head_ok = w9.shape[0] == 16 and 1 <= wo.shape[0] <= 8
        bn_drop = nk == "bn" and self.dropout.mode != "off"
        if nk != "none" and head_ok and not bn_drop:
            z9 = self._conv("block_nine.conv.0", u, "k3", norm_groups=ngroups(u, "block_nine.conv.0"))
            cs9 = self._channel_scale(z9.shape[0], z9.shape[-1], "drop9", 0.5, 1, z9.device)
            logits = self._norm_head("block_nine.conv.1", z9, nk, "out_conv", training=training, chan_scale=cs9)
        else:
            x9 = block("block_nine", u, 1, drop=("drop9", 1))
            logits = self._conv("out_conv", x9, "1x1", out_dtype=torch.float32)
        feats = self._head_branch(x5, x5_ready, training)
        return logits, feats, None

    def _unet(self, x, training, want_sdf):
        def uconv(prefix, t, first=False):
            c1, c2 = self.p[prefix + ".conv1.0.weight"].shape[0], self.p[prefix + ".conv2.0.weight"].shape[0]
            t = self._norm(None, self._conv(prefix + ".conv1.0", t, "k3", need_gx=not first, norm_groups=c1), "in")
            return self._norm(None, self._conv(prefix + ".conv2.0", t, "k3", norm_groups=c2), "in")

        def pool(t):
            y, idx = ops.maxpool2_fwd(t)
            if self.recording:
                def bwd():
                    self._give(t, ops.maxpool2_bwd(self._take(y), idx, t.shape))
                self.tape.append(bwd)
            return y

        def upcat(prefix, skip, low):
            B, D, H, W, C1 = skip.shape
            C2 = low.shape[-1]
            cat = torch.empty((B, D, H, W, C1 + C2), dtype=skip.dtype, device=skip.device)
            ops.copy_channels(skip, 0, cat, 0, C1)
            ops.trilinear_fwd(low, (D, H, W), False, out=cat, coff=C1)
            if self.recording:
                def bwd():
                    gc = self._take(cat)
                    gs = torch.empty(skip.shape, dtype=gc.dtype, device=gc.device)
                    ops.copy_channels(gc, 0, gs, 0, C1)
                    self._give(skip, gs)
                    self._give(low, ops.trilinear_bwd(gc, low.shape, False, coff=C1))
                self.tape.append(bwd)
            return uconv(prefix + ".conv", cat)

        c1 = uconv("conv1", x, first=True)
        c2 = uconv("conv2", pool(c1))
        c3 = uconv("conv3", pool(c2))
        c4 = uconv("conv4", pool(c3))
        center = self._drop_elements(uconv("center", pool(c4)), "drop_center", 0.3, 0)
        center_ready = self._mark_ready()
        u4 = upcat("up_concat4", c4, center)
        u3 = upcat("up_concat3", c3, u4)
        u2 = upcat("up_concat2", c2, u3)
        u1 = self._drop_elements(upcat("up_concat1", c1, u2), "drop_up1", 0.3, 1)
        logits = self._conv("out_conv2", u1, "1x1", out_dtype=torch.float32)
        feats = self._head_branch(center, center_ready, training)
        sdf = None
        if want_sdf:
            rec, self.recording = self.recording, False
            sdf = ops.tanh(self._conv("final", u1, "1x1", out_dtype=torch.float32))
            self.recording = rec
        return logits, feats, sdf

    def forward(self, x, training=True, record=True, dropout: Optional[DropoutSpec] = None, update_bn=True,
                want_sdf=False):
        assert x.dim() == 5 and x.is_contiguous()
        self.recording = bool(record)
        self.update_bn = update_bn
        self.dropout = dropout or DropoutSpec("off")
        self.tape, self.G = [], {}
        self._deferred = {}
        self._stat_parts = {}
        if x.dtype != self.dtype:
            x = ops.cast(x, self.dtype)
        if self.net_type == "vnet":
            logits, feats, sdf = self._vnet(x, training)
            if want_sdf:
                sdf = ops.tanh(logits)
        else:
            logits, feats, sdf = self._unet(x, training, want_sdf)
        self._out = (logits, feats)
        return logits, feats, sdf

    def backward(self, g_logits: Optional[torch.Tensor], g_feats: Optional[torch.Tensor]):
        logits, feats = self._out
        if g_logits is None:
            g_logits = torch.zeros_like(logits)
        if g_feats is None:
            g_feats = torch.zeros_like(feats)
        self.Gs = {}
        self._put(logits, g_logits)
        if self.feat_stream is not None:
            with ops.on_stream(self.feat_stream):
                self._put(feats, g_feats)
        else:
            self._put(feats, g_feats)
        h0, h1 = self._head_range
        for i in range(len(self.tape) - 1, -1, -1):
            if self.feat_stream is not None and h0 <= i < h1:
                with ops.on_stream(self.feat_stream):
                    self.tape[i]()
            else:
                self.tape[i]()
        cs = ops.cur_stream()
        if self._pending_dparams:
            ops.fork(cs, self.wgrad_stream)
            with ops.on_stream(self.wgrad_stream, light=True):
                self._flush_dparams()
        if self.mark is not None:
            self.mark("bwd_chain_end", cs)
            if self.feat_stream is not None:
                self.mark("feat_bwd_end", self.feat_stream)
            if self.wgrad_stream is not None:
                self.mark("wgrad_end", self.wgrad_stream)
        if self.feat_stream is not None:
            ops.fork(self.feat_stream, cs)
        if self.wgrad_stream is not None:
            ops.fork(self.wgrad_stream, cs)
            if self.wgrad_stream2 is not None:
                ops.fork(self.wgrad_stream2, cs)
        self.tape, self.G = [], {}
```

dycon_paper_replication_amd/ops.py:

```python
from __future__ import annotations

import collections
import ctypes
import functools
from typing import Optional

import torch

from . import _lib
from ._lib import BF16, CONV_1X1, CONV_K2S2, CONV_K3, F32, call, query

_DT = {torch.float32: F32, torch.bfloat16: BF16}


def dt(t: torch.Tensor) -> int:
    try:
        return _DT[t.dtype]
    except KeyError:
        raise TypeError(f"unsupported dtype {t.dtype}: the HIP path stores fp32 or bf16") from None


_STREAMS = []


# ... 171 lines not shown
    nbytes = query("dycon_bfrag_bytes", d, T, Cin, N)
    if out is None:
        out = torch.empty(nbytes // (2 if d == BF16 else 4), dtype=dtype, device=w.device)
    call("dycon_pack_bfrag", _p(w), _p(out), d, T, Cin, N, N0, s_t, s_c, s_n1, s_n0, int(flip), _s())
    return out


def pack_tcn(w: torch.Tensor, T, Cin, N, N0, s_t, s_c, s_n1, s_n0, flip=False, out=None):
    if out is None:
        out = torch.empty(T * Cin * N, dtype=torch.float32, device=w.device)
    call("dycon_pack_tcn", _p(w), _p(out), T, Cin, N, N0, s_t, s_c, s_n1, s_n0, int(flip), _s())
    return out


PACK_JOB_DTYPE = [("w", "<u8"), ("out", "<u8"), ("s_t", "<i8"), ("s_c", "<i8"), ("s_n1", "<i8"), ("s_n0", "<i8"), ("total", "<i8"),
                  ("kind", "<i4"), ("T", "<i4"), ("Cin", "<i4"), ("N", "<i4"), ("N0", "<i4"), ("flip", "<i4"), ("NT", "<i4"), ("pad_", "<i4")]


def pack_job(w, out, kind, T, Cin, N, N0, s_t, s_c, s_n1, s_n0, flip):
    return (w.data_ptr(), out.data_ptr(), s_t, s_c, s_n1, s_n0, out.numel(), kind, T, Cin, N, N0, int(flip), (N + 15) // 16, 0)


def upload_pack_jobs(jobs, device):
    import numpy as np
    arr = np.array(jobs, dtype=np.dtype(PACK_JOB_DTYPE))
    assert arr.dtype.itemsize == 88
    return torch.from_numpy(arr.view(np.uint8).copy()).to(device)


def pack_batch(jobs_dev, njobs, blocks_per_job=8):
    call("dycon_pack_batch", _p(jobs_dev), njobs, blocks_per_job, _s())


ConvPlan = collections.namedtuple("ConvPlan", "family splits chunks weights workspace name")


@functools.lru_cache(maxsize=None)
def conv_plan(dtype, mode, scatter, accumulate, B, D, H, W, Cin, N, Cout):
    lib, p = _lib.load(), _lib.ConvPlan()
    rc = lib.dycon_conv_gemm_plan(dtype, mode, scatter, accumulate, B, D, H, W, Cin, N, Cout, ctypes.byref(p))
    if rc:
        raise _lib.DyconLibraryError(f"dycon_conv_gemm_plan failed ({rc}): {lib.dycon_last_error().decode()}")
    return ConvPlan(p.family, p.splits, p.chunks, p.weights, p.workspace, lib.dycon_conv_region_name(ctypes.byref(p)).decode())


def conv_plan_for(x, mode, N, Cout, scatter=False, accumulate=False):
    B, D, H, W, Cin = x.shape
    return conv_plan(dt(x), mode, int(scatter), int(accumulate), B, D, H, W, Cin, N, Cout)


class DeferredConv:
    __slots__ = ("ws", "splits", "bias")

    def __init__(self, ws, splits, bias):
        self.ws, self.splits, self.bias = ws, splits, bias


_TAPS = {CONV_K3: 27, CONV_K2S2: 8, CONV_1X1: 1}


def conv_gemm(x, wfrag, bias, mode, N, Cout, scatter=False, out=None, accumulate=False, defer_finish=False):
    B, D, H, W, Cin = x.shape
    plan = conv_plan_for(x, mode, N, Cout, scatter, accumulate)
    if defer_finish:
        assert out is None and not accumulate and not scatter
        if plan.splits <= 1:
            return conv_gemm(x, wfrag, bias, mode, N, Cout), None
    if out is None:
        assert not accumulate
        if scatter:
            shape = (B, 2 * D, 2 * H, 2 * W, Cout)
        elif mode == CONV_K2S2:
            shape = (B, D // 2, H // 2, W // 2, N)
        else:
            shape = (B, D, H, W, N)
        out = torch.empty(shape, dtype=x.dtype, device=x.device)
    nws = plan.workspace
    ws = _ws(nws, x) if nws else None
    args = (_p(x), _p(wfrag), _p(bias), _p(out), dt(x), mode, int(scatter), int(accumulate), B, D, H, W, Cin, N, Cout, _p(ws), nws)
    if PROFILER is None and not defer_finish:
        call("dycon_conv_gemm", *args, _s())
        return out
    rows = out.numel() // Cout if not scatter else x.numel() // Cin
    with _Region(plan.name, (x.numel() + out.numel() * (2 if accumulate else 1)) * _es(x) + _TAPS[mode] * Cin * N * _es(x),
                 2 * rows * _TAPS[mode] * Cin * N):
        call("dycon_conv_gemm_ex", *args, int(defer_finish), _s())
    return (out, DeferredConv(ws, plan.splits, bias)) if defer_finish else out


def conv_stats_chunks(x, Cin, Cout):
    return conv_plan_for(x, CONV_K3, Cout, Cout).chunks


def conv_gemm_stats(x, wfrag, bias, Cout, chunks):
    B, D, H, W, Cin = x.shape
    y = torch.empty((B, D, H, W, Cout), dtype=x.dtype, device=x.device)
    part = torch.empty(B * chunks * Cout * 2, dtype=torch.float32, device=x.device)
    with _Region(conv_plan_for(x, CONV_K3, Cout, Cout).name, (x.numel() + y.numel()) * _es(x) + 27 * Cin * Cout * _es(x),
                 2 * (y.numel() // Cout) * 27 * Cin * Cout):
        call("dycon_conv_gemm_stats", _p(x), _p(wfrag), _p(bias), _p(y), dt(x), B, D, H, W, Cin, Cout, _p(part), part.numel() * 4, _s())
    return y, part


def conv_direct(x, w_tcn, bias, mode, N, out_dtype, out=None, accumulate=False):
    B, D, H, W, Cin = x.shape
    if out is None:
        assert not accumulate
        shape = (B, D // 2, H // 2, W // 2, N) if mode == CONV_K2S2 else (B, D, H, W, N)
        out = torch.empty(shape, dtype=out_dtype, device=x.device)
    taps = _TAPS[mode]
    with _Region("conv_direct", x.numel() * _es(x) + out.numel() * _es(out), 2 * (out.numel() // N) * taps * Cin * N):
        call("dycon_conv_direct", _p(x), dt(x), _p(w_tcn), _p(bias), _p(out), dt(out), mode, int(accumulate),
             B, D, H, W, Cin, N, _s())
    return out


def conv_wgrad_workspace(x, gy, mode):
    B, D, H, W, Cin = x.shape
    return _ws(query("dycon_conv_wgrad_workspace", mode, B, D, H, W, Cin, gy.shape[-1]), x)


def conv_wgrad(x, gy, dw, mode, s_t, s_c, s_n, dbias=None, ws=None):
    B, D, H, W, Cin = x.shape
    Cout = gy.shape[-1]
    if ws is None:
        ws = _ws(query("dycon_conv_wgrad_workspace", mode, B, D, H, W, Cin, Cout), x)
    taps = _TAPS[mode]
    rname = "" if PROFILER is None else _lib.load().dycon_conv_wgrad_name(dt(x), dt(gy), mode, B, D, H, W, Cin, Cout).decode()
    with _Region(rname, x.numel() * _es(x) + gy.numel() * _es(gy) + taps * Cin * Cout * 4, 2 * (gy.numel() // Cout) * taps * Cin * Cout):
        call("dycon_conv_wgrad", _p(x), dt(x), _p(gy), dt(gy), _p(dw), _p(dbias), mode, B, D, H, W, Cin, Cout, s_t, s_c, s_n,
             _p(ws), ws.numel() * 4, _s())
    return dw


def colsum(x2d_like, out, ws=None):
    C = x2d_like.shape[-1]
    rows = x2d_like.numel() // C
    if ws is None:
        ws = _ws(query("dycon_colsum_workspace", rows, C), x2d_like)
    with _Region("colsum", x2d_like.numel() * _es(x2d_like), x2d_like.numel()):
        call("dycon_colsum", _p(x2d_like), dt(x2d_like), _p(out), rows, C, _p(ws), ws.numel() * 4, _s())
    return out


def norm_stats(x, Nb, V, C, G, eps=1e-5, running_mean=None, running_var=None, momentum=0.1):
    stats = torch.empty(Nb * G * 2, dtype=torch.float32, device=x.device)
    ws = _ws(query("dycon_norm_workspace", Nb, V, C), x)
    with _Region("norm_stats", x.numel() * _es(x), 3 * x.numel()):
        call("dycon_norm_stats", _p(x), dt(x), Nb, V, C, G, eps, _p(stats), _p(running_mean), _p(running_var), momentum,
             _p(ws), ws.numel() * 4, _s())
    return stats


def norm_fwd(x, Nb, V, C, G, gamma=None, beta=None, relu=True, skip=None, chan_scale=None, eps=1e-5, running_mean=None,
             running_var=None, momentum=0.1, acc=None):
    y = torch.empty_like(x)
    stats = torch.empty(Nb * G * 2, dtype=torch.float32, device=x.device)
    if acc is not None:
        with _Region("norm_fwd", x.numel() * _es(x) * (4 if skip is not None else 3), 6 * x.numel()):
            call("dycon_norm_fwd_acc", _p(x), _p(y), dt(x), Nb, V, C, G, eps, _p(stats), _p(gamma), _p(beta), int(relu), _p(skip),
                 _p(chan_scale), _p(running_mean), _p(running_var), momentum, _p(acc), _s())
        return y, stats
    ws = _ws(query("dycon_norm_workspace", Nb, V, C), x)
    nb = x.numel() * _es(x)
    with _Region("norm_fwd", nb * (4 if skip is not None else 3), 6 * x.numel(),
                 parts=[("partial", nb, 3 * x.numel()), ("apply", nb * (3 if skip is not None else 2), 3 * x.numel())]):
        call("dycon_norm_fwd", _p(x), _p(y), dt(x), Nb, V, C, G, eps, _p(stats), _p(gamma), _p(beta), int(relu), _p(skip),
             _p(chan_scale), _p(running_mean), _p(running_var), momentum, _p(ws), ws.numel() * 4, _s())
    return y, stats


def norm_fwd_parts(x, part, chunks, Nb, V, C, G, gamma=None, beta=None, relu=True, skip=None, chan_scale=None, eps=1e-5,
                   running_mean=None, running_var=None, momentum=0.1):
    y = torch.empty_like(x)
    stats = torch.empty(Nb * G * 2, dtype=torch.float32, device=x.device)
    with _Region("norm_fwd", x.numel() * _es(x) * (3 if skip is not None else 2), 3 * x.numel()):
        call("dycon_norm_fwd_parts", _p(x), _p(y), dt(x), Nb, V, C, G, eps, _p(stats), _p(gamma), _p(beta), int(relu), _p(skip),
             _p(chan_scale), _p(running_mean), _p(running_var), momentum, _p(part), chunks, _s())
    return y, stats


def norm_stats_parts(x, part, chunks, Nb, V, C, G, eps=1e-5, running_mean=None, running_var=None, momentum=0.1):
    stats = torch.empty(Nb * G * 2, dtype=torch.float32, device=x.device)
    with _Region("norm_stats", 0, 0):
        call("dycon_norm_stats_parts", dt(x), Nb, V, C, G, eps, _p(stats), _p(running_mean), _p(running_var), momentum, _p(part), chunks, _s())
    return stats


def norm_fwd_is_fused(x, V, C, G):
    return bool(query("dycon_norm_fwd_is_fused", dt(x), V, C, G))


def norm_fwd_slab(x_out, dc: DeferredConv, Nb, V, C, G, gamma=None, beta=None, relu=True, skip=None, chan_scale=None, eps=1e-5):
    y = torch.empty_like(x_out)
    stats = torch.empty(Nb * G * 2, dtype=torch.float32, device=x_out.device)
    with _Region("norm_fwd", x_out.numel() * _es(x_out) * (4 if skip is not None else 3), 6 * x_out.numel()):
        call("dycon_norm_fwd_slab", _p(dc.ws), dc.splits, _p(dc.bias), _p(x_out), _p(y), dt(x_out), Nb, V, C, G, eps, _p(stats),
             _p(gamma), _p(beta), int(relu), _p(skip), _p(chan_scale), _s())
    return y, stats


def norm_apply(x, stats, Nb, V, C, G, gamma=None, beta=None, relu=True, skip=None, out=None, chan_scale=None):
    if out is None:
        out = torch.empty_like(x)
    with _Region("norm_apply", x.numel() * _es(x) * (3 if skip is not None else 2), 3 * x.numel()):
        call("dycon_norm_apply", _p(x), _p(out), dt(x), Nb, V, C, G, _p(stats), _p(gamma), _p(beta), int(relu), _p(skip),
             _p(chan_scale), _s())
    return out


def norm_bwd(src, from_y, gy, stats, Nb, V, C, G, gamma=None, beta=None, relu=True, dgamma=None, dbeta=None, out=None,
             chan_scale=None, acc=None, defer_dparams=False):
    if out is None:
        out = torch.empty_like(gy)
    if acc is not None and not from_y:
        fused = norm_fwd_is_fused(gy, V, C, G)
        ws = _ws(query("dycon_norm_workspace", Nb, V, C), gy) if fused else None
        with _Region("norm_bwd", gy.numel() * _es(gy) * 5, 12 * gy.numel()):
            call("dycon_norm_bwd_acc", _p(src), _p(gy), _p(out), dt(gy), Nb, V, C, G, _p(stats), _p(gamma), _p(beta), int(relu),
                 _p(chan_scale), _p(dgamma), _p(dbeta), _p(acc), _p(ws), ws.numel() * 4 if fused else 0, _s())
        return out
    ws = _ws(query("dycon_norm_workspace", Nb, V, C), gy)
    nb = gy.numel() * _es(gy)
    deferred = bool(defer_dparams) and not from_y and (dgamma is not None or dbeta is not None) and norm_fwd_is_fused(gy, V, C, G)
    with _Region("norm_bwd", nb * 5, 12 * gy.numel(), parts=[("partial", 2 * nb, 6 * gy.numel()), ("apply", 3 * nb, 6 * gy.numel())]):
        call("dycon_norm_bwd_ex", _p(src), int(from_y), _p(gy), _p(out), dt(gy), Nb, V, C, G, _p(stats), _p(gamma), _p(beta),
             int(relu), _p(chan_scale), _p(dgamma), _p(dbeta), int(deferred), _p(ws), ws.numel() * 4, _s())
    if defer_dparams:
        return out, ((ws, Nb, C, dgamma, dbeta) if deferred else None)
    return out


def norm_head_fwd(x, stats, Nb, V, G, head_w, head_b, gamma=None, beta=None, relu=True, chan_scale=None):
    K = head_w.shape[0]
    logits = torch.empty(x.shape[:-1] + (K,), dtype=torch.float32, device=x.device)
    with _Region("norm_fwd", x.numel() * _es(x) + logits.numel() * 4, 8 * x.numel()):
        if K == 2:
            call("dycon_norm_head_fwd", _p(x), dt(x), Nb, V, G, _p(stats), _p(gamma), _p(beta), int(relu), _p(chan_scale), _p(head_w),
                 _p(head_b), _p(logits), _s())
        else:
            call("dycon_norm_headc_fwd", _p(x), dt(x), Nb, V, G, K, _p(stats), _p(gamma), _p(beta), int(relu), _p(chan_scale),
                 _p(head_w), _p(head_b), _p(logits), _s())
    return logits


def norm_head_bwd(x, g_logits, stats, Nb, V, G, head_w, gamma=None, beta=None, relu=True, dgamma=None, dbeta=None, chan_scale=None):
    K = head_w.shape[0]
    gx = torch.empty_like(x)
    ws = _ws(query("dycon_norm_head_workspace", Nb, V) if K == 2 else query("dycon_norm_headc_workspace", Nb, V, K), x)
    nb = x.numel() * _es(x)
    with _Region("norm_bwd", nb * 3 + g_logits.numel() * 8, 14 * x.numel(),
                 parts=[("partial", nb + g_logits.numel() * 4, 7 * x.numel()), ("apply", 2 * nb + g_logits.numel() * 4, 7 * x.numel())]):
        if K == 2:
            call("dycon_norm_head_bwd", _p(x), _p(g_logits), _p(gx), dt(x), Nb, V, G, _p(stats), _p(gamma), _p(beta), int(relu),
                 _p(chan_scale), _p(head_w), _p(dgamma), _p(dbeta), _p(ws), ws.numel() * 4, _s())
        else:
            call("dycon_norm_headc_bwd", _p(x), _p(g_logits), _p(gx), dt(x), Nb, V, G, K, _p(stats), _p(gamma), _p(beta), int(relu),
                 _p(chan_scale), _p(head_w), _p(dgamma), _p(dbeta), _p(ws), ws.numel() * 4, _s())
    return gx, (ws, Nb, V, K)


def norm_head_dparams(pending, d_head_w, d_head_b):
    ws, Nb, V, K = pending
    if K == 2:
        call("dycon_norm_head_dparams", _p(ws), Nb, V, _p(d_head_w), _p(d_head_b), _s())
    else:
        call("dycon_norm_headc_dparams", _p(ws), Nb, V, K, _p(d_head_w), _p(d_head_b), _s())


def norm_bwd_stats(src, gy, stats, Nb, V, C, G, gamma=None, beta=None, relu=True, dgamma=None, dbeta=None, chan_scale=None):
    ws = _ws(query("dycon_norm_workspace", Nb, V, C), gy)
    with _Region("norm_bwd", gy.numel() * _es(gy) * 2, 6 * gy.numel()):
        call("dycon_norm_bwd_stats", _p(src), _p(gy), dt(gy), Nb, V, C, G, _p(stats), _p(gamma), _p(beta), int(relu), _p(chan_scale),
             _p(dgamma), _p(dbeta), _p(ws), ws.numel() * 4, _s())
    off = query("dycon_norm_bwd_ab_offset", Nb, V, C)
    return ws, ws[off:off + Nb * G * 2]


def first_block_bwd(x, z, gy, stats, Nb, G, dw, dbias, gamma=None, beta=None, relu=True, dgamma=None, dbeta=None, chan_scale=None, ws=None):
    B, D, H, W, _ = x.shape
    if ws is None:
        ws = _ws(query("dycon_first_block_bwd_workspace", B, D, H, W), x)
    with _Region("wgrad_k3_bf16", (x.numel() + z.numel() + gy.numel()) * 2 + 27 * 16 * 4, 6 * (gy.numel() // 16) * 27 * 16):
        call("dycon_first_block_bwd", _p(x), _p(z), _p(gy), B, D, H, W, Nb, G, _p(stats), _p(gamma), _p(beta), int(relu),
             _p(chan_scale), _p(dgamma), _p(dbeta), _p(dw), _p(dbias), 1, 27, 27, _p(ws), ws.numel() * 4, _s())
    return dw


def conv1_wgrad_normbwd(x, z, gy, stats, ab, Nb, G, dw, dbias, gamma=None, beta=None, relu=True, chan_scale=None, ws=None):
    B, D, H, W, _ = x.shape
    if ws is None:
        ws = _ws(query("dycon_conv1_wgrad_normbwd_workspace", B, D, H, W), x)
    with _Region("wgrad_k3_bf16", (x.numel() + z.numel() + gy.numel()) * 2 + 27 * 16 * 4, 2 * (gy.numel() // 16) * 27 * 16):
        call("dycon_conv1_wgrad_normbwd", _p(x), _p(z), _p(gy), B, D, H, W, Nb, G, _p(stats), _p(gamma), _p(beta), int(relu),
             _p(chan_scale), _p(ab), _p(dw), _p(dbias), 1, 27, 27, _p(ws), ws.numel() * 4, _s())
    return dw


def norm_sum_dparams(pending):
    ws, Nb, C, dgamma, dbeta = pending
    call("dycon_norm_sum_dparams", _p(ws), Nb, C, _p(dgamma), _p(dbeta), _s())


def maxpool2_fwd(x):
    B, D, H, W, C = x.shape
    y = torch.empty((B, D // 2, H // 2, W // 2, C), dtype=x.dtype, device=x.device)
    idx = torch.empty(y.shape, dtype=torch.uint8, device=x.device)
    call("dycon_maxpool2_fwd", _p(x), _p(y), _p(idx), dt(x), B, D, H, W, C, _s())
    return y, idx


def maxpool2_bwd(gy, idx, in_shape):
    B, D, H, W, C = in_shape
    gx = torch.empty(in_shape, dtype=gy.dtype, device=gy.device)
    call("dycon_maxpool2_bwd", _p(gy), _p(idx), _p(gx), dt(gy), B, D, H, W, C, _s())
    return gx


def trilinear_fwd(x, out_dhw, align_corners, out=None, coff=0):
    B, D, H, W, C = x.shape
    Do, Ho, Wo = out_dhw
    if out is None:
        out = torch.empty((B, Do, Ho, Wo, C), dtype=x.dtype, device=x.device)
    call("dycon_trilinear_fwd", _p(x), _p(out), dt(x), B, D, H, W, Do, Ho, Wo, C, out.shape[-1], coff, int(align_corners), _s())
    return out


def trilinear_bwd(gy, in_shape, align_corners, coff=0):
    B, D, H, W, C = in_shape
    _, Do, Ho, Wo, ld = gy.shape
    gx = torch.empty(in_shape, dtype=gy.dtype, device=gy.device)
    call("dycon_trilinear_bwd", _p(gy), _p(gx), dt(gy), B, D, H, W, Do, Ho, Wo, C, ld, coff, int(align_corners), _s())
    return gx


def upconv_k3(x, wfrag, bias, Cout, out=None):
    B, D, H, W, Cin = x.shape
    if out is None:
        out = torch.empty((B, 2 * D, 2 * H, 2 * W, Cout), dtype=x.dtype, device=x.device)
    with _Region("upconv_k3", (x.numel() + out.numel()) * _es(x) + 27 * Cin * Cout * _es(x), 2 * (out.numel() // Cout) * 27 * Cin * Cout):
        call("dycon_upconv_k3", _p(x), _p(wfrag), _p(bias), _p(out), dt(x), B, D, H, W, Cin, Cout, _s())
    return out


def copy_channels(src, soff, dst, doff, C):
    rows = src.numel() // src.shape[-1]
    call("dycon_copy_channels", _p(src), src.shape[-1], soff, _p(dst), dst.shape[-1], doff, rows, C, dt(src), _s())
    return dst


def scale_channels(x, scale):
    B, C = x.shape[0], x.shape[-1]
    V = x.numel() // (B * C)
    y = torch.empty_like(x)
    call("dycon_scale_channels", _p(x), _p(scale), _p(y), dt(x), B, V, C, _s())
    return y


def relu_fwd(z, skip=None, chan_scale=None):
    B, C = z.shape[0], z.shape[-1]
    y = torch.empty_like(z)
    with _Region("relu", z.numel() * _es(z) * (3 if skip is not None else 2), z.numel()):
        call("dycon_relu_fwd", _p(z), _p(skip), _p(chan_scale), _p(y), dt(z), B, z.numel() // (B * C), C, _s())
    return y


def relu_bwd(z, gy, chan_scale=None):
    B, C = z.shape[0], z.shape[-1]
    gz = torch.empty_like(gy)
    with _Region("relu", z.numel() * _es(z) * 3, z.numel()):
        call("dycon_relu_bwd", _p(z), _p(gy), _p(chan_scale), _p(gz), dt(z), B, z.numel() // (B * C), C, _s())
    return gz


def mul_mask(x, mask, inv_keep):
    y = torch.empty_like(x)
    call("dycon_mul_mask", _p(x), _p(mask), inv_keep, _p(y), dt(x), x.numel(), _s())
    return y


def dropout_philox(x, p, seed, offset):
    y = torch.empty_like(x)
    call("dycon_dropout_philox", _p(x), _p(y), dt(x), x.numel(), p, seed, offset, _s())
    return y


def channel_mask_philox(n, p, seed, offset, device):
    s = torch.empty(n, dtype=torch.float32, device=device)
    call("dycon_channel_mask_philox", _p(s), n, p, seed, offset, _s())
    return s


def add_noise(x, noise=None, sigma=0.1, clip=0.2, seed=0, offset=0):
    y = torch.empty_like(x)
    call("dycon_add_noise", _p(x), _p(noise), _p(y), dt(x), x.numel(), sigma, clip, seed, offset, _s())
    return y


def tanh(x):
    y = torch.empty(x.shape, dtype=torch.float32, device=x.device)
    call("dycon_tanh", _p(x), dt(x), _p(y), x.numel(), _s())
    return y


def cast(x, dtype):
    y = torch.empty(x.shape, dtype=dtype, device=x.device)
    call("dycon_cast", _p(x), dt(x), _p(y), _DT[dtype], x.numel(), _s())
    return y


def add(a, b=None, out=None):
    if out is None:
        out = torch.empty_like(a)
    call("dycon_add", _p(a), _p(b), _p(out), dt(a), a.numel(), _s())
    return out


def _label_bytes(labels):
    if labels.dtype == torch.int64:
        return 8
    if labels.dtype == torch.uint8:
        return 1
    raise TypeError("labels must be int64 or uint8")


def seg_losses_fwd(s_logits, t_logits, labels, LB, beta, fast=False, out=None):
    B = s_logits.shape[0]
    V = s_logits.numel() // (2 * B)
    sums = out if out is not None else torch.empty(16, dtype=torch.float64, device=s_logits.device)
    call("dycon_seg_losses_fwd", _p(s_logits), _p(t_logits), _p(labels), _label_bytes(labels), B, LB, V, float(beta), _p(sums), int(fast), _s())
    return sums


def seg_losses_bwd(s_logits, t_logits, labels, LB, beta, sums, coef, cons_kind=0, fast=False):
    B = s_logits.shape[0]
    V = s_logits.numel() // (2 * B)
    g = torch.empty_like(s_logits)
    call("dycon_seg_losses_bwd", _p(s_logits), _p(t_logits), _p(labels), _label_bytes(labels), B, LB, V, float(beta), _p(sums),
         _p(coef), cons_kind, _p(g), int(fast), _s())
    return g


def seg_losses_finalize(sums, B, LB, V, beta):
    vals = torch.empty(8, dtype=torch.float32, device=sums.device)
    call("dycon_seg_losses_finalize", _p(sums), B, LB, V, float(beta), _p(vals), _s())
    return vals


def step_losses(sums, fecl_out, B, LB, V, beta, fecl_rows, lambda_cross, has_teacher, l_w, cons_w, u_w, dice_kind, cons_kind,
                nonfinite=None):
    out = torch.empty(8, dtype=torch.float32, device=sums.device)
    call("dycon_step_losses", _p(sums), _p(fecl_out), B, LB, V, float(beta), float(fecl_rows), float(lambda_cross), int(bool(has_teacher)),
         float(l_w), float(cons_w), float(u_w), dice_kind, cons_kind, _p(out), _p(nonfinite), _s())
    return out


def seg_lossesc_nsums(classes):
    n = _lib.query("dycon_seg_lossesc_nsums", int(classes))
    if n <= 0:
        raise ValueError(f"the C-class voxel losses take 2..8 classes, got {classes}")
    return n


def seg_lossesc_fwd(s_logits, t_logits, labels, LB, beta, cons_kind=2, fast=False, out=None):
    B, C = s_logits.shape[0], s_logits.shape[-1]
    V = s_logits.numel() // (C * B)
    n = seg_lossesc_nsums(C)
    sums = out if out is not None else torch.empty(n, dtype=torch.float64, device=s_logits.device)
    assert sums.numel() >= n and t_logits.shape == s_logits.shape
    call("dycon_seg_lossesc_fwd", _p(s_logits), _p(t_logits), _p(labels), _label_bytes(labels), B, LB, V, C, float(beta), int(cons_kind),
         _p(sums), int(fast), _s())
    return sums


def seg_lossesc_bwd(s_logits, t_logits, labels, LB, beta, sums, coef, cons_kind=0, fast=False):
    B, C = s_logits.shape[0], s_logits.shape[-1]
    V = s_logits.numel() // (C * B)
    g = torch.empty_like(s_logits)
    call("dycon_seg_lossesc_bwd", _p(s_logits), _p(t_logits), _p(labels), _label_bytes(labels), B, LB, V, C, float(beta), _p(sums),
         _p(coef), cons_kind, _p(g), int(fast), _s())
    return g


def seg_lossesc_finalize(sums, B, LB, V, classes, beta):
    vals = torch.empty(8, dtype=torch.float32, device=sums.device)
    call("dycon_seg_lossesc_finalize", _p(sums), B, LB, V, int(classes), float(beta), _p(vals), _s())
    return vals


def step_lossesc(sums, fecl_out, B, LB, V, classes, beta, fecl_rows, lambda_cross, has_teacher, l_w, cons_w, u_w, dice_kind, cons_kind,
                 nonfinite=None):
    out = torch.empty(8, dtype=torch.float32, device=sums.device)
    call("dycon_step_lossesc", _p(sums), _p(fecl_out), B, LB, V, int(classes), float(beta), float(fecl_rows), float(lambda_cross),
         int(bool(has_teacher)), float(l_w), float(cons_w), float(u_w), dice_kind, cons_kind, _p(out), _p(nonfinite), _s())
    return out


def step_loss(vals, fecl, l_w, cons_w, u_w, dice_kind, cons_kind, nonfinite=None):
    out = torch.empty(8, dtype=torch.float32, device=vals.device)
    call("dycon_step_loss", _p(vals), _p(fecl), float(l_w), float(cons_w), float(u_w), dice_kind, cons_kind, _p(out),
         _p(nonfinite), _s())
    return out


def l2norm_fwd(x, eps=1e-12):
    C = x.shape[-1]
    R = x.numel() // C
    y = torch.empty_like(x)
    norms = torch.empty(R, dtype=torch.float32, device=x.device)
    call("dycon_l2norm_fwd", _p(x), _p(y), _p(norms), dt(x), R, C, eps, _s())
    return y, norms


def l2norm_bwd(y, norms, gy, eps=1e-12):
    C = y.shape[-1]
    gx = torch.empty_like(gy)
    call("dycon_l2norm_bwd", _p(y), _p(norms), _p(gy), _p(gx), dt(y), y.numel() // C, C, eps, _s())
    return gx


def mask_pool(labels, k):
    B, D, H, W = labels.shape
    kd, kh, kw = (k, k, k) if isinstance(k, int) else k
    m = torch.empty((B, (D // kd) * (H // kh) * (W // kw)), dtype=torch.float32, device=labels.device)
    call("dycon_mask_pool", _p(labels), _label_bytes(labels), _p(m), B, D, H, W, kd, kh, kw, _s())
    return m


class FeclState:
    __slots__ = ("out", "ws", "loss", "rows")


def fecl_fwd(feat, teacher, mask, gambling, temperature, gamma, use_focal, cross_thresh, lambda_cross, out=None):
    B, N, Dm = feat.shape
    st = FeclState()
    st.out = out if out is not None else torch.empty(4, dtype=torch.float64, device=feat.device)
    st.loss = torch.empty(1, dtype=torch.float32, device=feat.device)
    st.ws = _ws(query("dycon_fecl_workspace", B, N, Dm), feat)
    call("dycon_fecl_fwd", _p(feat), _p(teacher), _p(mask), _p(gambling), dt(feat), B, N, Dm, temperature, gamma,
         int(use_focal), cross_thresh, lambda_cross, _p(st.out), _p(st.loss), _p(st.ws), st.ws.numel() * 4, _s())
    return st.loss, st


def fecl_finalize(st, rows, lambda_cross, has_teacher):
    call("dycon_fecl_finalize", _p(st.out), float(rows), float(lambda_cross), int(bool(has_teacher)), _p(st.loss), _s())
    return st.loss


def set_scalars(dst, values):
    v = [float(x) for x in values] + [0.0] * (8 - len(values))
    call("dycon_set_scalars", _p(dst), len(values), *v, _s())
    return dst


def fecl_bwd(feat, teacher, mask, gambling, temperature, gamma, use_focal, cross_thresh, lambda_cross, st, coef):
    B, N, Dm = feat.shape
    g = torch.empty_like(feat)
    call("dycon_fecl_bwd", _p(feat), _p(teacher), _p(mask), _p(gambling), dt(feat), B, N, Dm, temperature, gamma,
         int(use_focal), cross_thresh, lambda_cross, _p(st.out), _p(coef), _p(g), _p(st.ws), st.ws.numel() * 4, _s())
    return g


def _gambling_channels(x):
    if x.dtype != torch.float32 or x.dim() < 1 or not 1 <= x.shape[-1] <= 8:
        raise ValueError(f"gambling_softmax: expected fp32 (..., C) with C in 1..8, got {tuple(x.shape)} {x.dtype}")


def gambling_softmax(x):
    _gambling_channels(x)
    y = torch.empty_like(x)
    call("dycon_gambling_softmax_fwd", _p(x), _p(y), x.numel() // x.shape[-1], x.shape[-1], _s())
    return y


def gambling_softmax_bwd(y, gy):
    _gambling_channels(y)
    if gy.shape != y.shape or gy.dtype != torch.float32:
        raise ValueError("gambling_softmax_bwd: gy must match y (fp32)")
    gx = torch.empty_like(y)
    call("dycon_gambling_softmax_bwd", _p(y), _p(gy), _p(gx), y.numel() // y.shape[-1], y.shape[-1], _s())
    return gx


def _gambling_k(k):
    kd, kh, kw = (k, k, k) if isinstance(k, int) else tuple(int(v) for v in k)
    if kd % 2 or kh % 2 or kw % 2:
        raise ValueError(f"gambling uncertainty: the patch factor must be even per axis, got {(kd, kh, kw)}")
    return kd, kh, kw


def _gambling_logits(logits, k):
    if logits.dim() != 5 or logits.shape[-1] != 2 or logits.dtype != torch.float32:
        raise ValueError(f"gambling uncertainty: expected fp32 logits (B, D, H, W, 2), got {tuple(logits.shape)} {logits.dtype}")
    kd, kh, kw = _gambling_k(k)
    B, D, H, W, _ = logits.shape
    if D < kd or H < kh or W < kw:
        raise ValueError(f"gambling uncertainty: volume {(D, H, W)} smaller than one patch {(kd, kh, kw)}")
    return B, D, H, W, kd, kh, kw


def gambling_uncertainty(logits, k, fast=False, out=None):
    B, D, H, W, kd, kh, kw = _gambling_logits(logits, k)
    N = (D // kd) * (H // kh) * (W // kw)
    if out is not None and (out.dtype != torch.float32 or out.numel() != B * N):
        raise ValueError(f"gambling_uncertainty: out must hold B*N = {B * N} fp32 values")
    u = out if out is not None else torch.empty((B, N), dtype=torch.float32, device=logits.device)
# ... 144 lines not shown
```

include/dycon_hip.h:

```cpp
#ifndef DYCON_HIP_H
#define DYCON_HIP_H

#include <stddef.h>
#include <stdint.h>

#ifdef __cplusplus
extern "C" {
#endif

typedef struct ihipStream_t* dycon_stream_t;

#define DYCON_F32 0
#define DYCON_BF16 1

#define DYCON_OK 0
#define DYCON_ERR_INVALID (-22)
#define DYCON_ERR_LAUNCH (-5)

#define DYCON_CONV_1X1 0
#define DYCON_CONV_K3 1
#define DYCON_CONV_K2S2 2

int dycon_version(void);
const char* dycon_last_error(void);

size_t dycon_bfrag_bytes(int dtype, int T, int Cin, int N);
int dycon_pack_bfrag(const float* w, void* out, int dtype, int T, int Cin, int N, int N0,
                     long long s_t, long long s_c, long long s_n1, long long s_n0, int flip_taps,
                     dycon_stream_t stream);
typedef struct {
    const float* w;
    void* out;
    long long s_t, s_c, s_n1, s_n0, total;
    int kind, T, Cin, N, N0, flip, NT, pad_;
} dycon_pack_job_t;
int dycon_pack_batch(const dycon_pack_job_t* jobs_dev, int njobs, int blocks_per_job, dycon_stream_t stream);
int dycon_pack_tcn(const float* w, float* out, int T, int Cin, int N, int N0, long long s_t,
                   long long s_c, long long s_n1, long long s_n0, int flip_taps, dycon_stream_t stream);

enum {
    DYCON_CONV_NONE = 0, DYCON_CONV_C1, DYCON_CONV_P16, DYCON_CONV_P32, DYCON_CONV_LDS, DYCON_CONV_HALO, DYCON_CONV_TILE,
    DYCON_CONV_GEMM
};
enum { DYCON_CONV_W_FRAG = 0, DYCON_CONV_W_CHUNK16 = 1 };
typedef struct {
    int family, splits, chunks, weights;
    size_t workspace;
} dycon_conv_plan_t;
int dycon_conv_gemm_plan(int dtype, int mode, int scatter, int accumulate, int B, int Di, int Hi, int Wi, int Cin, int N,
                         int Cout, dycon_conv_plan_t* plan);
const char* dycon_conv_kernel_name(int family);
const char* dycon_conv_region_name(const dycon_conv_plan_t* plan);
size_t dycon_conv_gemm_workspace(int dtype, int mode, int scatter, int B, int Di, int Hi, int Wi,
                                 int Cin, int N);
int dycon_conv_gemm(const void* x, const void* wfrag, const float* bias, void* y, int dtype,
                    int mode, int scatter, int accumulate, int B, int Di, int Hi, int Wi, int Cin,
                    int N, int Cout, float* workspace, size_t ws_bytes, dycon_stream_t stream);
int dycon_conv_gemm_splits(int dtype, int mode, int scatter, int B, int Di, int Hi, int Wi, int Cin, int N);
int dycon_conv_gemm_ex(const void* x, const void* wfrag, const float* bias, void* y, int dtype,
                       int mode, int scatter, int accumulate, int B, int Di, int Hi, int Wi, int Cin,
                       int N, int Cout, float* workspace, size_t ws_bytes, int defer_finish,
                       dycon_stream_t stream);
int dycon_conv_direct(const void* x, int x_dtype, const float* w_tcn, const float* bias, void* y,
                      int y_dtype, int mode, int accumulate, int B, int Di, int Hi, int Wi, int Cin,
                      int N, dycon_stream_t stream);

size_t dycon_conv_wgrad_workspace(int mode, int B, int Di, int Hi, int Wi, int Cin, int Cout);
const char* dycon_conv_wgrad_name(int x_dtype, int g_dtype, int mode, int B, int Di, int Hi, int Wi, int Cin, int Cout);
int dycon_conv_wgrad(const void* x, int x_dtype, const void* gy, int g_dtype, float* dw, float* dbias,
                     int mode, int B, int Di, int Hi, int Wi, int Cin, int Cout, long long s_t,
                     long long s_c, long long s_n, float* workspace, size_t ws_bytes,
                     dycon_stream_t stream);

size_t dycon_colsum_workspace(long long rows, int C);
int dycon_colsum(const void* x, int dtype, float* out, long long rows, int C, float* workspace,
                 size_t ws_bytes, dycon_stream_t stream);

size_t dycon_norm_workspace(int Nb, long long V, int C);
int dycon_norm_stats(const void* x, int dtype, int Nb, long long V, int C, int G, float eps,
                     float* stats, float* running_mean, float* running_var, float momentum,
                     float* workspace, size_t ws_bytes, dycon_stream_t stream);
int dycon_norm_fwd(const void* x, void* y, int dtype, int Nb, long long V, int C, int G, float eps,
                   float* stats, const float* gamma, const float* beta, int relu, const void* skip,
                   const float* chan_scale, float* running_mean, float* running_var, float momentum,
                   float* workspace, size_t ws_bytes, dycon_stream_t stream);
int dycon_norm_fwd_is_fused(int dtype, long long V, int C, int G);
int dycon_norm_fwd_slab(const float* slab, int splits, const float* conv_bias, void* x_out, void* y,
                        int dtype, int Nb, long long V, int C, int G, float eps, float* stats,
                        const float* gamma, const float* beta, int relu, const void* skip,
                        const float* chan_scale, dycon_stream_t stream);
int dycon_norm_apply(const void* x, void* y, int dtype, int Nb, long long V, int C, int G,
                     const float* stats, const float* gamma, const float* beta, int relu,
                     const void* skip, const float* chan_scale, dycon_stream_t stream);
int dycon_norm_bwd(const void* src, int from_y, const void* gy, void* gx, int dtype, int Nb,
                   long long V, int C, int G, const float* stats, const float* gamma,
                   const float* beta, int relu, const float* chan_scale, float* dgamma, float* dbeta,
                   float* workspace, size_t ws_bytes, dycon_stream_t stream);
int dycon_norm_bwd_ex(const void* src, int from_y, const void* gy, void* gx, int dtype, int Nb,
                      long long V, int C, int G, const float* stats, const float* gamma,
                      const float* beta, int relu, const float* chan_scale, float* dgamma, float* dbeta,
                      int defer_dparams, float* workspace, size_t ws_bytes, dycon_stream_t stream);
int dycon_norm_sum_dparams(const float* workspace, int Nb, int C, float* dgamma, float* dbeta,
                           dycon_stream_t stream);
size_t dycon_norm_head_workspace(int Nb, long long V);
int dycon_norm_head_fwd(const void* x, int dtype, int Nb, long long V, int G, const float* stats, const float* gamma,
                        const float* beta, int relu, const float* chan_scale, const float* head_w, const float* head_b,
                        float* logits, dycon_stream_t stream);
int dycon_norm_head_bwd(const void* x, const float* g_logits, void* gx, int dtype, int Nb, long long V, int G,
                        const float* stats, const float* gamma, const float* beta, int relu, const float* chan_scale,
                        const float* head_w, float* dgamma, float* dbeta, float* workspace, size_t ws_bytes,
                        dycon_stream_t stream);
int dycon_norm_head_dparams(const float* workspace, int Nb, long long V, float* d_head_w, float* d_head_b,
                            dycon_stream_t stream);
size_t dycon_norm_headc_workspace(int Nb, long long V, int classes);
int dycon_norm_headc_fwd(const void* x, int dtype, int Nb, long long V, int G, int classes, const float* stats,
                         const float* gamma, const float* beta, int relu, const float* chan_scale, const float* head_w,
                         const float* head_b, float* logits, dycon_stream_t stream);
int dycon_norm_headc_bwd(const void* x, const float* g_logits, void* gx, int dtype, int Nb, long long V, int G, int classes,
                         const float* stats, const float* gamma, const float* beta, int relu, const float* chan_scale,
                         const float* head_w, float* dgamma, float* dbeta, float* workspace, size_t ws_bytes,
                         dycon_stream_t stream);
int dycon_norm_headc_dparams(const float* workspace, int Nb, long long V, int classes, float* d_head_w, float* d_head_b,
                             dycon_stream_t stream);
int dycon_conv_stats_chunks(int dtype, int mode, int B, int Di, int Hi, int Wi, int Cin, int Cout);
int dycon_norm_stats_parts(int dtype, int Nb, long long V, int C, int G, float eps, float* stats, float* running_mean,
                           float* running_var, float momentum, const float* part, int chunks, dycon_stream_t stream);
int dycon_conv_gemm_stats(const void* x, const void* wfrag, const float* bias, void* y, int dtype, int B, int Di, int Hi,
                          int Wi, int Cin, int Cout, float* stat_part, size_t stat_bytes, dycon_stream_t stream);
int dycon_norm_fwd_parts(const void* x, void* y, int dtype, int Nb, long long V, int C, int G, float eps, float* stats,
                         const float* gamma, const float* beta, int relu, const void* skip, const float* chan_scale,
                         float* running_mean, float* running_var, float momentum, const float* part, int chunks,
                         dycon_stream_t stream);
size_t dycon_norm_bwd_ab_offset(int Nb, long long V, int C);
int dycon_norm_bwd_stats(const void* src, const void* gy, int dtype, int Nb, long long V, int C, int G, const float* stats,
                         const float* gamma, const float* beta, int relu, const float* chan_scale, float* dgamma,
                         float* dbeta, float* workspace, size_t ws_bytes, dycon_stream_t stream);
size_t dycon_first_block_bwd_workspace(int B, int D, int H, int W);
int dycon_first_block_bwd(const void* x, const void* z, const void* gy, int B, int D, int H, int W, int Nb, int G,
                          const float* stats, const float* gamma, const float* beta, int relu, const float* chan_scale,
                          float* dgamma, float* dbeta, float* dw, float* dbias, long long s_t, long long s_c, long long s_n,
                          float* workspace, size_t ws_bytes, dycon_stream_t stream);
size_t dycon_conv1_wgrad_normbwd_workspace(int B, int D, int H, int W);
int dycon_conv1_wgrad_normbwd(const void* x, const void* z, const void* gy, int B, int D, int H, int W, int Nb, int G,
                              const float* stats, const float* gamma, const float* beta, int relu, const float* chan_scale,
                              const float* ab, float* dw, float* dbias, long long s_t, long long s_c, long long s_n,
                              float* workspace, size_t ws_bytes, dycon_stream_t stream);
size_t dycon_norm_acc_doubles(int Nb, long long V, int C);
int dycon_norm_fwd_acc(const void* x, void* y, int dtype, int Nb, long long V, int C, int G, float eps,
                       float* stats, const float* gamma, const float* beta, int relu, const void* skip,
                       const float* chan_scale, float* running_mean, float* running_var, float momentum,
                       double* acc, dycon_stream_t stream);
int dycon_norm_bwd_acc(const void* src, const void* gy, void* gx, int dtype, int Nb, long long V, int C,
                       int G, const float* stats, const float* gamma, const float* beta, int relu,
                       const float* chan_scale, float* dgamma, float* dbeta, double* acc, float* workspace,
                       size_t ws_bytes, dycon_stream_t stream);

int dycon_maxpool2_fwd(const void* x, void* y, uint8_t* idx, int dtype, int B, int D, int H, int W,
                       int C, dycon_stream_t stream);
int dycon_maxpool2_bwd(const void* gy, const uint8_t* idx, void* gx, int dtype, int B, int D, int H,
                       int W, int C, dycon_stream_t stream);
int dycon_trilinear_fwd(const void* x, void* y, int dtype, int B, int Di, int Hi, int Wi, int Do,
                        int Ho, int Wo, int C, int ldy, int coff, int align_corners,
                        dycon_stream_t stream);
int dycon_trilinear_bwd(const void* gy, void* gx, int dtype, int B, int Di, int Hi, int Wi, int Do,
                        int Ho, int Wo, int C, int ldy, int coff, int align_corners,
                        dycon_stream_t stream);
int dycon_upconv_k3(const void* x, const void* wfrag, const float* bias, void* y, int dtype, int B,
                    int Di, int Hi, int Wi, int Cin, int Cout, dycon_stream_t stream);
int dycon_copy_channels(const void* src, int lds, int soff, void* dst, int ldd, int doff,
                        long long rows, int C, int dtype, dycon_stream_t stream);
int dycon_relu_fwd(const void* z, const void* skip, const float* chan_scale, void* y, int dtype, int B, long long V, int C,
                   dycon_stream_t stream);
int dycon_relu_bwd(const void* z, const void* gy, const float* chan_scale, void* gz, int dtype, int B, long long V, int C,
                   dycon_stream_t stream);

int dycon_scale_channels(const void* x, const float* scale, void* y, int dtype, int B, long long V,
                         int C, dycon_stream_t stream);
int dycon_mul_mask(const void* x, const float* mask, float inv_keep, void* y, int dtype,
                   long long n, dycon_stream_t stream);
int dycon_dropout_philox(const void* x, void* y, int dtype, long long n, float p, uint64_t seed,
                         uint64_t offset, dycon_stream_t stream);
int dycon_channel_mask_philox(float* scale, long long n, float p, uint64_t seed, uint64_t offset,
                              dycon_stream_t stream);
int dycon_add_noise(const void* x, const float* noise, void* y, int dtype, long long n, float sigma,
                    float clip, uint64_t seed, uint64_t offset, dycon_stream_t stream);
int dycon_tanh(const void* x, int x_dtype, float* y, long long n, dycon_stream_t stream);
int dycon_cast(const void* x, int x_dtype, void* y, int y_dtype, long long n, dycon_stream_t stream);
int dycon_add(const void* a, const void* b, void* y, int dtype, long long n, dycon_stream_t stream);

int dycon_seg_losses_fwd(const float* s_logits, const float* t_logits, const void* labels,
                         int label_bytes, int B, int LB, long long V, float beta, double* sums,
                         int fast, dycon_stream_t stream);
int dycon_seg_losses_bwd(const float* s_logits, const float* t_logits, const void* labels,
                         int label_bytes, int B, int LB, long long V, float beta, const double* sums,
                         const float* coef, int cons_kind, float* g_logits, int fast,
                         dycon_stream_t stream);

int dycon_seg_losses_finalize(const double* sums, int B, int LB, long long V, float beta, float* vals,
                              dycon_stream_t stream);
int dycon_step_loss(const float* vals, const float* fecl, float l_weight, float cons_weight,
                    float u_weight, int dice_kind, int cons_kind, float* out, int* nonfinite,
                    dycon_stream_t stream);
int dycon_step_losses(const double* sums, const double* fecl_out, int B, int LB, long long V, float beta,
                      double fecl_rows, float lambda_cross, int has_teacher, float l_weight, float cons_weight,
                      float u_weight, int dice_kind, int cons_kind, float* out, int* nonfinite,
                      dycon_stream_t stream);

int dycon_seg_lossesc_nsums(int classes);
int dycon_seg_lossesc_fwd(const float* s_logits, const float* t_logits, const void* labels, int label_bytes, int B, int LB,
                          long long V, int classes, float beta, int cons_kind, double* sums, int fast, dycon_stream_t stream);
int dycon_seg_lossesc_bwd(const float* s_logits, const float* t_logits, const void* labels, int label_bytes, int B, int LB,
                          long long V, int classes, float beta, const double* sums, const float* coef, int cons_kind,
                          float* g_logits, int fast, dycon_stream_t stream);
int dycon_seg_lossesc_finalize(const double* sums, int B, int LB, long long V, int classes, float beta, float* vals,
                               dycon_stream_t stream);
int dycon_step_lossesc(const double* sums, const double* fecl_out, int B, int LB, long long V, int classes, float beta,
                       double fecl_rows, float lambda_cross, int has_teacher, float l_weight, float cons_weight,
                       float u_weight, int dice_kind, int cons_kind, float* out, int* nonfinite, dycon_stream_t stream);

typedef struct {
    const void* p;
    long long sn, sc, sv;
} dycon_view_t;
int dycon_softmax_mse_fwd(const dycon_view_t* a, const dycon_view_t* b, const dycon_view_t* out, long long n, int C,
                          long long V, int sigmoid, dycon_stream_t stream);
int dycon_softmax_mse_bwd(const dycon_view_t* a, const dycon_view_t* b, const dycon_view_t* g, const dycon_view_t* ga,
                          long long n, int C, long long V, int sigmoid, dycon_stream_t stream);
int dycon_softmax_kl_fwd(const dycon_view_t* a, const dycon_view_t* b, long long n, int C, long long V, int sigmoid,
                         double* sum, float* out, dycon_stream_t stream);
int dycon_softmax_kl_bwd(const dycon_view_t* a, const dycon_view_t* b, long long n, int C, long long V, int sigmoid,
                         int which, const float* g_up, const dycon_view_t* grad, dycon_stream_t stream);
int dycon_dice_fwd(const dycon_view_t* score, const dycon_view_t* target, int target_kind, int onehot, long long n, int C,
                   long long V, int softmax, const float* weights_host, float n_div, double* sums, float* out,
                   dycon_stream_t stream);
int dycon_dice_bwd(const dycon_view_t* score, const dycon_view_t* target, int target_kind, int onehot, long long n, int C,
                   long long V, int softmax, const float* weights_host, float n_div, const double* sums, const float* g_up,
                   const dycon_view_t* grad, dycon_stream_t stream);

int dycon_dice1_fwd(const dycon_view_t* score, const dycon_view_t* target, int target_kind, long long n, int C, long long V,
                    int softmax, double* sums, float* out, dycon_stream_t stream);
int dycon_dice1_bwd(const dycon_view_t* a, const dycon_view_t* b, int b_kind, long long n, int C, long long V, int softmax,
                    const double* sums, const float* g_up, const dycon_view_t* grad, dycon_stream_t stream);
int dycon_entropy_fwd(const dycon_view_t* p, long long n, int C, long long V, float scale, float* map, double* sum, float* out,
                      dycon_stream_t stream);
int dycon_entropy_bwd(const dycon_view_t* p, long long n, int C, long long V, float scale, const float* g_map, const float* g_up,
                      const dycon_view_t* grad, dycon_stream_t stream);
int dycon_sym_mse_fwd(const dycon_view_t* a, const dycon_view_t* b, long long count, double* sum, float* out, dycon_stream_t stream);
int dycon_sym_mse_bwd(const dycon_view_t* a, const dycon_view_t* b, long long count, const float* g_up, const dycon_view_t* grad,
                      dycon_stream_t stream);
int dycon_kl_rows_fwd(const dycon_view_t* a, long long sla, const dycon_view_t* b, long long slb, long long n, long long C,
                      long long V, int L, double* sum, float* out, dycon_stream_t stream);
int dycon_kl_rows_bwd(const dycon_view_t* a, long long sla, const dycon_view_t* b, long long slb, long long n, long long C,
                      long long V, int L, const float* g_up, const dycon_view_t* grad, long long slg, dycon_stream_t stream);
int dycon_focal_fwd(const dycon_view_t* x, const void* target, int target_kind, long long n, int C, long long V, float gamma,
                    const float* alpha_host, int size_average, double* sum, float* out, dycon_stream_t stream);
int dycon_focal_bwd(const dycon_view_t* x, const void* target, int target_kind, long long n, int C, long long V, float gamma,
                    const float* alpha_host, int size_average, const float* g_up, const dycon_view_t* grad, dycon_stream_t stream);
int dycon_uncl_fwd(const dycon_view_t* s, const dycon_view_t* t, long long n, int C, long long V, float beta, double* sum, float* out,
                   dycon_stream_t stream);
int dycon_uncl_bwd(const dycon_view_t* s, const dycon_view_t* t, long long n, int C, long long V, float beta, const float* g_up,
                   const dycon_view_t* grad, dycon_stream_t stream);

int dycon_l2norm_fwd(const void* x, void* y, float* norms, int dtype, long long R, int C, float eps,
                     dycon_stream_t stream);
int dycon_l2norm_bwd(const void* y, const float* norms, const void* gy, void* gx, int dtype,
                     long long R, int C, float eps, dycon_stream_t stream);
int dycon_mask_pool(const void* labels, int label_bytes, float* mask, int B, int D, int H, int W,
                    int kd, int kh, int kw, dycon_stream_t stream);

size_t dycon_fecl_workspace(int B, int N, int Dm);
int dycon_fecl_fwd(const void* feat, const void* teacher, const float* mask, const float* gambling,
                   int dtype, int B, int N, int Dm, float temperature, float gamma, int use_focal,
                   float cross_thresh, float lambda_cross, double* out, float* loss, float* workspace,
                   size_t ws_bytes, dycon_stream_t stream);
int dycon_fecl_finalize(const double* out, double rows, float lambda_cross, int has_teacher, float* loss,
                        dycon_stream_t stream);
int dycon_fecl_bwd(const void* feat, const void* teacher, const float* mask, const float* gambling,
                   int dtype, int B, int N, int Dm, float temperature, float gamma, int use_focal,
                   float cross_thresh, float lambda_cross, const double* out, const float* coef,
                   void* g_feat, float* workspace, size_t ws_bytes, dycon_stream_t stream);

int dycon_gambling_softmax_fwd(const float* x, float* y, long long nvox, int C, dycon_stream_t stream);
int dycon_gambling_softmax_bwd(const float* y, const float* gy, float* gx, long long nvox, int C, dycon_stream_t stream);
int dycon_gambling_uncertainty_fwd(const float* logits, int B, int D, int H, int W, int kd, int kh, int kw, float* u,
                                   int fast, dycon_stream_t stream);
int dycon_gambling_uncertainty_bwd(const float* logits, int B, int D, int H, int W, int kd, int kh, int kw,
                                   const float* gu, float* g_logits, int fast, dycon_stream_t stream);
size_t dycon_fecl_rows_workspace(int B, int N, int Dm);
int dycon_fecl_fwd_rows(const void* feat, const void* teacher, const float* mask, float* rows, int dtype, int B, int N,
                        int Dm, float temperature, float cross_thresh, double* out, float* workspace, size_t ws_bytes,
                        size_t rows_bytes, dycon_stream_t stream);
int dycon_fecl_gambling_finalize(const float* u, const float* coef, int dtype, int B, int N, int Dm, double* out, float* r,
                                 float* gu, float* workspace, size_t ws_bytes, const float* rows, size_t rows_bytes,
                                 dycon_stream_t stream);
int dycon_fecl_gambling_grad(const float* r, const float* coef, long long n, float* gu, dycon_stream_t stream);

int dycon_sumsq(const float* g, long long n, double* sumsq, dycon_stream_t stream);
int dycon_sgd_ema(float* p, const float* g, float* mom, float* teacher, long long n_sgd,
                  long long n_all, const double* sumsq, float max_norm, float grad_scale, float lr,
                  float momentum, float weight_decay, float ema_alpha, const int* skip_flag,
                  dycon_stream_t stream);
int dycon_set_scalars(float* dst, int n, float v0, float v1, float v2, float v3, float v4, float v5,
                      float v6, float v7, dycon_stream_t stream);
int dycon_nonfinite_flag(const float* x, int* flag, dycon_stream_t stream);

int dycon_sw_accumulate(const float* logits, int n_patches, int p0, int p1, int p2, const int* origins_dev,
                        float* score, float* cnt, int D0, int D1, int D2, dycon_stream_t stream);
int dycon_sw_accumulate_c(const float* logits, int C, int n_patches, int p0, int p1, int p2, const int* origins_dev,
                          float* score, float* cnt, int D0, int D1, int D2, dycon_stream_t stream);
int dycon_sw_finalize(const float* score, const float* cnt, long long n, float thresh, uint8_t* label,
                      float* prob, dycon_stream_t stream);
int dycon_binary_overlap(const uint8_t* pred, const void* gt, int gt_bytes, long long n,
                         unsigned long long* out3, dycon_stream_t stream);

int dycon_batch_overlap(const float* logits, const void* gt, int gt_bytes, int B, long long V,
                        unsigned long long* out3b, dycon_stream_t stream);

int dycon_sw_accumulate_all(const float* logits, int C, int n_patches, int p0, int p1, int p2, const int* origins_dev,
                            float* score, float* cnt, int D0, int D1, int D2, const int* box_lo, const int* box_hi,
                            dycon_stream_t stream);
int dycon_sw_finalize_argmax(const float* score, const float* cnt, int C, long long n, uint8_t* label, float* prob,
                             dycon_stream_t stream);
int dycon_argmax_labels(const float* logits, int C, long long nvox, uint8_t* label, dycon_stream_t stream);
int dycon_class_confusion(const uint8_t* pred, const void* gt, int gt_bytes, long long n, int C, unsigned long long* out,
                          dycon_stream_t stream);
int dycon_batch_class_confusion(const float* logits, const void* gt, int gt_bytes, int B, long long V, int C,
                                unsigned long long* out, dycon_stream_t stream);

size_t dycon_surface_workspace(int S, int X, int Y, int Z);
int dycon_surface_hist(const void* a, int a_bytes, const void* b, int b_bytes, int n_vol, int cls_lo, int n_cls, int X, int Y, int Z,
                       unsigned int* hist, unsigned int* nborder, void* workspace, size_t ws_bytes, dycon_stream_t stream);
int dycon_surface_metrics(const unsigned int* hist, const unsigned int* nborder, int S, int nbins, double q, double* out,
                          dycon_stream_t stream);

size_t dycon_cc_workspace(int n_vol, int X, int Y, int Z);
int dycon_cc_roots(const void* vol, int vol_bytes, int n_vol, int X, int Y, int Z, int connectivity, int by_value, int* root,
                   dycon_stream_t stream);
int dycon_cc_labels(const int* root, int n_vol, int X, int Y, int Z, int* labels, int* ncomp, void* workspace, size_t ws_bytes,
                    dycon_stream_t stream);
int dycon_cc_largest(const void* vol, int vol_bytes, const int* root, int n_vol, int X, int Y, int Z, int n_cls, uint8_t* out,
                     int* win_size, int* win_root, void* workspace, size_t ws_bytes, dycon_stream_t stream);

size_t dycon_simhist_workspace(int B, int N, int Dm, int bins);
int dycon_simhist(const void* feat, const float* mask, int dtype, int B, int N, int Dm, float tau, int bins,
                  long long* counts, float* edges, float* minmax, float* workspace, size_t ws_bytes, dycon_stream_t stream);

#define DYCON_TAPS_MAX 64
#define DYCON_WBLK_SRC_MAX 8
#define DYCON_WBLK_MAX 512
#define DYCON_SEGS_MAX 16
int dycon_tap_gather(const void* x, void* y, int dtype, int B, int D, int H, int W, int C, const int* taps_host, int ntaps,
                     dycon_stream_t stream);
int dycon_pack_wblocks(const float* const* w_host, const long long* strides_host, int nsrc, const short* blk_host, int KB, int NB,
                       int kblk, int nblk, void* out, size_t out_bytes, int dtype, dycon_stream_t stream);
int dycon_unpack_wgrad(const float* dense, long long ldd, int KB, float* const* g_host, const int* taps_host, const short* kb_host,
                       int ndst, int Ci, int Co, dycon_stream_t stream);
int dycon_sample_colsum(const void* x, int dtype, float* out, int B, long long V, int C, float scale, int accumulate,
                        dycon_stream_t stream);
int dycon_sample_bcast(const void* x, const float* vec, void* y, int dtype, int B, long long V, int C, float scale,
                       dycon_stream_t stream);
int dycon_small_gemm(const float* a, long long sar, long long sai, const float* b, long long sbr, long long sbj, float* c,
                     long long ldc, int I, int J, int R, int accumulate, dycon_stream_t stream);
int dycon_copy_segments(const float* const* src_host, float* const* dst_host, const int* n_host, int nseg, dycon_stream_t stream);

int dycon_kernel_timing(int on);
long long dycon_kernel_timing_count(void);
int dycon_kernel_timing_fetch(long long first, long long n, float* ms, unsigned long long* stream, int* name_id);
const char* dycon_kernel_timing_name(int id);

#ifdef __cplusplus
}
#endif
#endif
```

Measured before the change: 912.1.

## Fuse decoder transposed-conv with group norm, ReLU and skip-add via recompute

Adds upnorm kernels that recompute the 2x2x2 stride-2 transposed convolution output on the fly with MFMA, then accumulate group-norm statistics or apply normalization, ReLU, channel scaling and the skip add directly. The full-resolution pre-norm activation is never written to memory. The backward pass likewise recomputes the deconv output for the norm-backward statistics and apply steps. This is meant to cut the memory traffic of the largest decoder tensors, at the cost of running the small deconv GEMM two or three times per pass.

Result: no change. 911.3 (-0.1%).

```diff
diff --git a/dycon_paper_replication_amd/_lib.py b/dycon_paper_replication_amd/_lib.py
--- a/dycon_paper_replication_amd/_lib.py
+++ b/dycon_paper_replication_amd/_lib.py
@@ -66,6 +66,14 @@
     "dycon_trilinear_fwd": (I, [P, P, I, I, I, I, I, I, I, I, I, I, I, I, P]),
     "dycon_trilinear_bwd": (I, [P, P, I, I, I, I, I, I, I, I, I, I, I, I, P]),
     "dycon_upconv_k3": (I, [P, P, P, P, I, I, I, I, I, I, I, P]),
+    "dycon_upnorm_served": (I, [I, I, I, I]),
+    "dycon_upnorm_chunks": (I, [I, I, I]),
+    "dycon_upnorm_stats_chunks": (I, [I, I, I]),
+    "dycon_upnorm_stats": (I, [P, P, P, I, I, I, I, I, I, I, I, P, Z, P]),
+    "dycon_upnorm_apply": (I, [P, P, P, P, I, I, I, I, I, I, I, I, P, P, P, I, P, P, P]),
+    "dycon_upnorm_bwd_stats": (I, [P, P, P, P, I, I, I, I, I, I, I, I, P, P, P, I, P, P, Z, P]),
+    "dycon_norm_bwd_parts": (I, [I, I, I, P, P, I, P, P, P, P]),
+    "dycon_upnorm_bwd_apply": (I, [P, P, P, P, P, I, I, I, I, I, I, I, I, P, P, P, P, I, P, P]),
     "dycon_copy_channels": (I, [P, I, I, P, I, I, L, I, I, P]),
     "dycon_relu_fwd": (I, [P, P, P, P, I, I, L, I, P]),
     "dycon_relu_bwd": (I, [P, P, P, P, I, I, L, I, P]),
diff --git a/dycon_paper_replication_amd/csrc/norm.hip b/dycon_paper_replication_amd/csrc/norm.hip
--- a/dycon_paper_replication_amd/csrc/norm.hip
+++ b/dycon_paper_replication_amd/csrc/norm.hip
@@ -743,6 +743,16 @@
     return DYCON_OK;
 }
 
+extern "C" int dycon_norm_bwd_parts(int Nb, int C, int G, const float* gamma, const float* part, int chunks, float* ab, float* dgamma,
+                                    float* dbeta, dycon_stream_t stream) {
+    DYCON_REQUIRE(part && ab && chunks > 0, "norm_bwd_parts: bad arguments");
+    DYCON_REQUIRE(Nb > 0 && C > 0 && G > 0 && C % G == 0, "norm_bwd_parts: bad shape Nb=%d C=%d G=%d", Nb, C, G);
+    const int nfin = Nb * G + ((dgamma || dbeta) ? C : 0);
+    norm_finalize_bwd_kernel<<<nfin, 256, 0, stream>>>(part, Nb, chunks, C, G, gamma, ab, dgamma, dbeta);
+    DYCON_LAUNCH_CHECK();
+    return DYCON_OK;
+}
+
 extern "C" int dycon_norm_sum_dparams(const float* workspace, int Nb, int C, float* dgamma, float* dbeta, dycon_stream_t stream) {
     DYCON_REQUIRE(workspace && Nb > 0 && C > 0 && (dgamma || dbeta), "norm_sum_dparams: bad arguments");
     norm_sum_dparams_kernel<<<cdiv(C, 256), 256, 0, stream>>>(workspace, Nb, C, dgamma, dbeta);
diff --git a/dycon_paper_replication_amd/csrc/upnorm.hip b/dycon_paper_replication_amd/csrc/upnorm.hip
--- /dev/null
+++ b/dycon_paper_replication_amd/csrc/upnorm.hip
@@ -0,0 +1,533 @@
+#include "common.h"
+
+namespace {
+
+typedef float f32x4 __attribute__((ext_vector_type(4)));
+typedef __bf16 bf16x8 __attribute__((ext_vector_type(8)));
+
+__device__ __forceinline__ void up_mma(f32x4& acc, const Vec16<bf16>& a, const Vec16<bf16>& b) {
+    acc = __builtin_amdgcn_mfma_f32_16x16x32_bf16(__builtin_bit_cast(bf16x8, a.v), __builtin_bit_cast(bf16x8, b.v), acc, 0, 0, 0);
+}
+__device__ __forceinline__ float round_bf16(float v) { return __bfloat162float(__float2bfloat16(v)); }
+
+constexpr int UN_ROWS = 64;
+constexpr int UN_GC = 64;
+constexpr int UN_OS = UN_GC + 8;
+constexpr int UN_APPLY_WGS = 1024;
+constexpr int UN_MAX_CHUNKS = 256;
+constexpr int UN_UNROLL = 2, UN_UNROLL_BWD_APPLY = 1;
+#define UN_WAVES __attribute__((amdgpu_waves_per_eu(4)))
+
+template <int CIN>
+__device__ __forceinline__ void up_load_a(const bf16* __restrict__ Xn, int v, int Vin, int kg, Vec16<bf16> (&a)[CIN / 32]) {
+#pragma unroll
+    for (int u = 0; u < CIN / 32; ++u) {
+        a[u].v = decltype(a[u].v){};
+        if (v < Vin) a[u] = ld16(Xn + (long long)v * CIN + u * 32 + 8 * kg);
+    }
+}
+
+template <int CIN>
+__device__ __forceinline__ void up_group(const Vec16<bf16> (&a)[CIN / 32], const bf16* __restrict__ Wf, int jg, int lane, f32x4 (&acc)[4]) {
+    constexpr int NKC = CIN / 32, NT = CIN / 4;
+    Vec16<bf16> bq[NKC][4];
+#pragma unroll
+    for (int u = 0; u < NKC; ++u)
+#pragma unroll
+        for (int j = 0; j < 4; ++j) bq[u][j] = ld16(Wf + (((long long)u * NT + jg * 4 + j) * 64 + lane) * 8);
+#pragma unroll
+    for (int j = 0; j < 4; ++j) acc[j] = f32x4{0.f, 0.f, 0.f, 0.f};
+#pragma unroll
+    for (int u = 0; u < NKC; ++u)
+#pragma unroll
+        for (int j = 0; j < 4; ++j) up_mma(acc[j], a[u], bq[u][j]);
+}
+
+template <int CIN>
+__device__ __forceinline__ void up_stage(const f32x4 (&acc)[4], const float (&bv)[CIN / 32], bf16* __restrict__ Ot, int wave, int lane) {
+    constexpr int COUT = CIN / 2;
+    const int r = lane & 15, kg = lane >> 4;
+#pragma unroll
+    for (int j = 0; j < 4; ++j) {
+        const float b = bv[COUT == 32 ? (j & 1) : 0];
+#pragma unroll
+        for (int i = 0; i < 4; ++i) stf(Ot + (wave * 16 + kg * 4 + i) * UN_OS + j * 16 + r, acc[j][i] + b);
+    }
+}
+
+template <int CIN>
+struct UpPiece {
+    static constexpr int COUT = CIN / 2, PPT = COUT / 8;
+    int pc, co0, tl;
+    __device__ __forceinline__ UpPiece() {
+        pc = threadIdx.x & 7;
+        co0 = (pc % PPT) * 8;
+        tl = pc / PPT;
+    }
+    __device__ __forceinline__ long long base(int n, int v, int Di, int Hi, int Wi) const {
+        const int x = v % Wi, q = v / Wi, y = q % Hi, z = q / Hi;
+        return ((((long long)n * (2 * Di) + 2 * z) * (2 * Hi) + 2 * y) * (2 * Wi) + 2 * x) * COUT + co0;
+    }
+    __device__ __forceinline__ long long tap_off(int jg, int Hi, int Wi) const {
+        const int tap = jg * (UN_GC / COUT) + tl;
+        return ((long long)((tap >> 2) * (2 * Hi) + ((tap >> 1) & 1)) * (2 * Wi) + (tap & 1)) * COUT;
+    }
+};
+
+}
+
+template <int CIN>
+__global__ __launch_bounds__(256) void up_stats_kernel(const bf16* __restrict__ X, const bf16* __restrict__ Wf,
+                                                       const float* __restrict__ bias, float* __restrict__ part, int Vin, int Hi,
+                                                       int Wi, int rows_per_chunk) {
+    constexpr int COUT = CIN / 2, NKC = CIN / 32, NT = CIN / 4, TPT = COUT / 16;
+    constexpr int RPI = 256 / (COUT / 8), MT = RPI / 64;
+    __shared__ float sm[2][RPI][COUT + 1];
+    const int lane = threadIdx.x & 63, wave = threadIdx.x >> 6, r = lane & 15, kg = lane >> 4;
+    const int n = blockIdx.y, chunk = blockIdx.x;
+    const int V = 8 * Vin, Wo = 2 * Wi, Ho = 2 * Hi;
+    const int v0 = chunk * rows_per_chunk, v1 = min(V, v0 + rows_per_chunk);
+    const bf16* Xn = X + (long long)n * Vin * CIN;
+    float bv[TPT], s0[MT][TPT][4], s1[MT][TPT][4];
+#pragma unroll
+    for (int q = 0; q < TPT; ++q) bv[q] = bias ? bias[q * 16 + r] : 0.f;
+#pragma unroll
+    for (int mt = 0; mt < MT; ++mt)
+#pragma unroll
+        for (int q = 0; q < TPT; ++q)
+#pragma unroll
+            for (int i = 0; i < 4; ++i) s0[mt][q][i] = s1[mt][q][i] = 0.f;
+    const int wv = __builtin_amdgcn_readfirstlane(wave);
+    int pox[MT], poy[MT], poz[MT];
+#pragma unroll
+    for (int mt = 0; mt < MT; ++mt) {
+        const int rb0 = v0 + (wv * MT + mt) * 16, q = rb0 / Wo;
+        pox[mt] = rb0 % Wo; poy[mt] = q % Ho; poz[mt] = q / Ho;
+    }
+    const int sdx = RPI % Wo, sdy = (RPI / Wo) % Ho, sdz = RPI / Wo / Ho;
+    for (int vb = v0; vb < v1; vb += RPI) {
+#pragma unroll
+        for (int mt = 0; mt < MT; ++mt) {
+            const int rb = vb + (wv * MT + mt) * 16;
+            const bool one_row = pox[mt] + 15 < Wo;
+            Vec16<bf16> a[NKC];
+            int tap[4];
+            {
+                const int v = rb + r;
+                int m;
+                if (one_row) {
+                    m = ((poz[mt] >> 1) * Hi + (poy[mt] >> 1)) * Wi + ((pox[mt] + r) >> 1);
+                    const int t2 = ((poz[mt] & 1) << 2) | ((poy[mt] & 1) << 1);
+#pragma unroll
+                    for (int i = 0; i < 4; ++i) tap[i] = rb + 4 * kg + i < v1 ? t2 | ((pox[mt] + 4 * kg + i) & 1) : -1;
+                } else {
+                    const int ox = v % Wo, q = v / Wo, oy = q % Ho, oz = q / Ho;
+                    m = ((oz >> 1) * Hi + (oy >> 1)) * Wi + (ox >> 1);
+                    const int vd = rb + 4 * kg;
+                    int dx = vd % Wo, dq = vd / Wo, dy = dq % Ho, dz = dq / Ho;
+#pragma unroll
+                    for (int i = 0; i < 4; ++i) {
+                        tap[i] = vd + i < v1 ? ((dz & 1) << 2) | ((dy & 1) << 1) | (dx & 1) : -1;
+                        if (++dx == Wo) { dx = 0; if (++dy == Ho) { dy = 0; ++dz; } }
+                    }
+                }
+#pragma unroll
+                for (int u = 0; u < NKC; ++u) {
+                    a[u].v = decltype(a[u].v){};
+                    if (v < v1) a[u] = ld16(Xn + (long long)m * CIN + u * 32 + 8 * kg);
+                }
+            }
+            float zs[TPT][4];
+#pragma unroll
+            for (int q = 0; q < TPT; ++q)
+#pragma unroll
+                for (int i = 0; i < 4; ++i) zs[q][i] = 0.f;
+            auto form_tap = [&](int t) {
+#pragma unroll
+                for (int q = 0; q < TPT; ++q) {
+                    f32x4 acc = f32x4{0.f, 0.f, 0.f, 0.f};
+#pragma unroll
+                    for (int u = 0; u < NKC; ++u) up_mma(acc, a[u], ld16(Wf + (((long long)u * NT + t * TPT + q) * 64 + lane) * 8));
+#pragma unroll
+                    for (int i = 0; i < 4; ++i)
+                        if (tap[i] == t) zs[q][i] = acc[i];
+                }
+            };
+            if (one_row) {
+                const int t2 = ((poz[mt] & 1) << 2) | ((poy[mt] & 1) << 1);
+                form_tap(t2);
+                form_tap(t2 | 1);
+            } else {
+#pragma unroll
+                for (int t = 0; t < 8; ++t) form_tap(t);
+            }
+#pragma unroll
+            for (int q = 0; q < TPT; ++q)
+#pragma unroll
+                for (int i = 0; i < 4; ++i) {
+                    if (tap[i] >= 0) {
+                        const float x = round_bf16(zs[q][i] + bv[q]);
+                        s0[mt][q][i] += x;
+                        s1[mt][q][i] += x * x;
+                    }
+                }
+            pox[mt] += sdx; if (pox[mt] >= Wo) { pox[mt] -= Wo; ++poy[mt]; }
+            poy[mt] += sdy; if (poy[mt] >= Ho) { poy[mt] -= Ho; ++poz[mt]; }
+            poz[mt] += sdz;
+        }
+    }
+#pragma unroll
+    for (int mt = 0; mt < MT; ++mt)
+#pragma unroll
+        for (int q = 0; q < TPT; ++q)
+#pragma unroll
+            for (int i = 0; i < 4; ++i) {
+                const int row = (wave * MT + mt) * 16 + 4 * kg + i;
+                sm[0][row][q * 16 + r] = s0[mt][q][i];
+                sm[1][row][q * 16 + r] = s1[mt][q][i];
+            }
+    __syncthreads();
+    if (threadIdx.x < COUT) {
+        const int c = threadIdx.x;
+        double d0 = 0.0, d1 = 0.0;
+        for (int q = 0; q < RPI; ++q) { d0 += (double)sm[0][q][c]; d1 += (double)sm[1][q][c]; }
+        float* d = part + (((long long)n * gridDim.x + chunk) * COUT + c) * 2;
+        d[0] = (float)d0;
+        d[1] = (float)d1;
+    }
+}
+
+template <int CIN>
+__global__ __launch_bounds__(256) UN_WAVES void up_apply_kernel(const bf16* __restrict__ X, const bf16* __restrict__ Wf,
+                                                       const float* __restrict__ bias, bf16* __restrict__ Y, int Vin, int Di,
+                                                       int Hi, int Wi, int tiles, int tiles_per_wg, int G,
+                                                       const float* __restrict__ stats, const float* __restrict__ gamma,
+                                                       const float* __restrict__ beta, int relu, const bf16* __restrict__ skip, const float* __restrict__ chan_scale) {
+    constexpr int COUT = CIN / 2, NKC = CIN / 32, NG = 8 * COUT / UN_GC, CPL = COUT / 16;
+    __shared__ __attribute__((aligned(16))) bf16 Ot[2][UN_ROWS * UN_OS];
+    constexpr int UNR = UN_UNROLL;
+    const int lane = threadIdx.x & 63, wave = threadIdx.x >> 6, r = lane & 15, kg = lane >> 4;
+    const int n = blockIdx.y, cpg = COUT / G;
+    const bf16* Xn = X + (long long)n * Vin * CIN;
+    float bv[CPL];
+#pragma unroll
+    for (int q = 0; q < CPL; ++q) bv[q] = bias ? bias[q * 16 + r] : 0.f;
+    const UpPiece<CIN> pp;
+    float sc[8], sh[8], dr[8];
+#pragma unroll
+    for (int k = 0; k < 8; ++k) {
+        const int c = pp.co0 + k, g = c / cpg;
+        const float mean = stats[((long long)n * G + g) * 2], rstd = stats[((long long)n * G + g) * 2 + 1];
+        const float gm = gamma ? gamma[c] : 1.f, bt = beta ? beta[c] : 0.f;
+        sc[k] = rstd * gm;
+        sh[k] = bt - mean * rstd * gm;
+        dr[k] = chan_scale ? chan_scale[(long long)n * COUT + c] : 1.f;
+    }
+    const int prow = threadIdx.x >> 3;
+    int buf = 0;
+    const int t0 = blockIdx.x * tiles_per_wg, t1 = min(tiles, t0 + tiles_per_wg);
+    for (int t = t0; t < t1; ++t) {
+        const int row0 = t * UN_ROWS;
+        Vec16<bf16> a[NKC];
+        up_load_a<CIN>(Xn, row0 + wave * 16 + r, Vin, kg, a);
+        const int v0 = row0 + prow, v1 = v0 + 32;
+        const bool ok0 = v0 < Vin, ok1 = v1 < Vin;
+        const long long b0 = ok0 ? pp.base(n, v0, Di, Hi, Wi) : 0, b1 = ok1 ? pp.base(n, v1, Di, Hi, Wi) : 0;
+#pragma unroll UNR
+        for (int jg = 0; jg < NG; ++jg) {
+            const long long to = pp.tap_off(jg, Hi, Wi);
+            Vec16<bf16> s0v, s1v;
+            s0v.v = s1v.v = decltype(s0v.v){};
+            if (skip) {
+                if (ok0) s0v = ld16(skip + b0 + to);
+                if (ok1) s1v = ld16(skip + b1 + to);
+            }
+            f32x4 acc[4];
+            up_group<CIN>(a, Wf, jg, lane, acc);
+            up_stage<CIN>(acc, bv, Ot[buf], wave, lane);
+            __syncthreads();
+#pragma unroll
+            for (int h = 0; h < 2; ++h) {
+                if (!(h ? ok1 : ok0)) continue;
+                const Vec16<bf16> x = ld16(Ot[buf] + (prow + 32 * h) * UN_OS + pp.pc * 8);
+                const Vec16<bf16>& s = h ? s1v : s0v;
+                Vec16<bf16> y;
+#pragma unroll
+                for (int k = 0; k < 8; ++k) {
+                    float v = x.get(k) * sc[k] + sh[k];
+                    if (relu) v = v < 0.f ? 0.f : v;
+                    v *= dr[k];
+                    if (skip) v += s.get(k);
+                    y.set(k, v);
+                }
+                st16(Y + (h ? b1 : b0) + to, y);
+            }
+            buf ^= 1;
+        }
+    }
+}
+
+template <int CIN>
+__global__ __launch_bounds__(256) UN_WAVES void up_bwd_stats_kernel(const bf16* __restrict__ X, const bf16* __restrict__ Wf,
+                                                           const float* __restrict__ bias, const bf16* __restrict__ GY,
+                                                           float* __restrict__ part, int Vin, int Di, int Hi, int Wi, int tiles,
+                                                           int tiles_per_chunk, int G, const float* __restrict__ stats,
+                                                           const float* __restrict__ gamma, const float* __restrict__ beta,
+                                                           int relu, const float* __restrict__ chan_scale) {
+    constexpr int COUT = CIN / 2, NKC = CIN / 32, NG = 8 * COUT / UN_GC, CPL = COUT / 16, PPT = COUT / 8;
+    __shared__ __attribute__((aligned(16))) bf16 Ot[2][UN_ROWS * UN_OS];
+    __shared__ float sm[4][COUT][2];
+    constexpr int UNR = CIN == 32 ? 1 : UN_UNROLL;
+    const int lane = threadIdx.x & 63, wave = threadIdx.x >> 6, r = lane & 15, kg = lane >> 4;
+    const int n = blockIdx.y, chunk = blockIdx.x, cpg = COUT / G;
+    const bf16* Xn = X + (long long)n * Vin * CIN;
+    float bv[CPL];
+#pragma unroll
+    for (int q = 0; q < CPL; ++q) bv[q] = bias ? bias[q * 16 + r] : 0.f;
+    const UpPiece<CIN> pp;
+    float mean[8], rstd[8], gm[8], bt[8], cs[8], a0[8], a1[8];
+#pragma unroll
+    for (int k = 0; k < 8; ++k) {
+        const int c = pp.co0 + k, g = c / cpg;
+        mean[k] = stats[((long long)n * G + g) * 2];
+        rstd[k] = stats[((long long)n * G + g) * 2 + 1];
+        gm[k] = gamma ? gamma[c] : 1.f;
+        bt[k] = beta ? beta[c] : 0.f;
+        cs[k] = chan_scale ? chan_scale[(long long)n * COUT + c] : 1.f;
+        a0[k] = a1[k] = 0.f;
+    }
+    const int prow = threadIdx.x >> 3;
+    int buf = 0;
+    const int t0 = chunk * tiles_per_chunk, t1 = min(tiles, t0 + tiles_per_chunk);
+    for (int t = t0; t < t1; ++t) {
+        const int row0 = t * UN_ROWS;
+        Vec16<bf16> a[NKC];
+        up_load_a<CIN>(Xn, row0 + wave * 16 + r, Vin, kg, a);
+        const int v0 = row0 + prow, v1 = v0 + 32;
+        const bool ok0 = v0 < Vin, ok1 = v1 < Vin;
+        const long long b0 = ok0 ? pp.base(n, v0, Di, Hi, Wi) : 0, b1 = ok1 ? pp.base(n, v1, Di, Hi, Wi) : 0;
+#pragma unroll UNR
+        for (int jg = 0; jg < NG; ++jg) {
+            const long long to = pp.tap_off(jg, Hi, Wi);
+            Vec16<bf16> g0v, g1v;
+            g0v.v = g1v.v = decltype(g0v.v){};
+            if (ok0) g0v = ld16(GY + b0 + to);
+            if (ok1) g1v = ld16(GY + b1 + to);
+            f32x4 acc[4];
+            up_group<CIN>(a, Wf, jg, lane, acc);
+            up_stage<CIN>(acc, bv, Ot[buf], wave, lane);
+            __syncthreads();
+#pragma unroll
+            for (int h = 0; h < 2; ++h) {
+                if (!(h ? ok1 : ok0)) continue;
+                const Vec16<bf16> x = ld16(Ot[buf] + (prow + 32 * h) * UN_OS + pp.pc * 8);
+                const Vec16<bf16>& gv = h ? g1v : g0v;
+#pragma unroll
+                for (int k = 0; k < 8; ++k) {
+                    const float xh = (x.get(k) - mean[k]) * rstd[k];
+                    float g = gv.get(k) * cs[k];
+                    if (relu && !(gm[k] * xh + bt[k] > 0.f)) g = 0.f;
+                    a0[k] += g;
+                    a1[k] += g * xh;
+                }
+            }
+            buf ^= 1;
+        }
+    }
+#pragma unroll
+    for (int k = 0; k < 8; ++k) {
+#pragma unroll
+        for (int o = PPT; o < 64; o <<= 1) { a0[k] += __shfl_xor(a0[k], o, 64); a1[k] += __shfl_xor(a1[k], o, 64); }
+        if (lane < PPT) { sm[wave][lane * 8 + k][0] = a0[k]; sm[wave][lane * 8 + k][1] = a1[k]; }
+    }
+    __syncthreads();
+    if (threadIdx.x < COUT) {
+        const int c = threadIdx.x;
+        const double d0 = (double)sm[0][c][0] + (double)sm[1][c][0] + (double)sm[2][c][0] + (double)sm[3][c][0];
+        const double d1 = (double)sm[0][c][1] + (double)sm[1][c][1] + (double)sm[2][c][1] + (double)sm[3][c][1];
+        float* d = part + (((long long)n * gridDim.x + chunk) * COUT + c) * 2;
+        d[0] = (float)d0;
+        d[1] = (float)d1;
+    }
+}
+
+template <int CIN>
+__global__ __launch_bounds__(256) UN_WAVES void up_bwd_apply_kernel(const bf16* __restrict__ X, const bf16* __restrict__ Wf,
+                                                           const float* __restrict__ bias, const bf16* __restrict__ GY,
+                                                           bf16* __restrict__ GZ, int Vin, int Di, int Hi, int Wi, int tiles, int tiles_per_wg, int G,
+                                                           const float* __restrict__ stats, const float* __restrict__ gamma,
+                                                           const float* __restrict__ beta, const float* __restrict__ ab, int relu,
+                                                           const float* __restrict__ chan_scale) {
+    constexpr int COUT = CIN / 2, NKC = CIN / 32, NG = 8 * COUT / UN_GC, CPL = COUT / 16;
+    __shared__ __attribute__((aligned(16))) bf16 Ot[2][UN_ROWS * UN_OS];
+    constexpr int UNR = UN_UNROLL_BWD_APPLY;
+    const int lane = threadIdx.x & 63, wave = threadIdx.x >> 6, r = lane & 15, kg = lane >> 4;
+    const int n = blockIdx.y, cpg = COUT / G;
+    const bf16* Xn = X + (long long)n * Vin * CIN;
+    float bv[CPL];
+#pragma unroll
+    for (int q = 0; q < CPL; ++q) bv[q] = bias ? bias[q * 16 + r] : 0.f;
+    const UpPiece<CIN> pp;
+    const float inv_cnt = 1.f / (8.f * (float)Vin * (float)cpg);
+    float mu[8], rs[8], gmv[8], btv[8], pa[8], pb[8], dr[8];
+#pragma unroll
+    for (int k = 0; k < 8; ++k) {
+        const int c = pp.co0 + k, g = c / cpg;
+        mu[k] = stats[((long long)n * G + g) * 2];
+        rs[k] = stats[((long long)n * G + g) * 2 + 1];
+        gmv[k] = gamma ? gamma[c] : 1.f;
+        btv[k] = beta ? beta[c] : 0.f;
+        pa[k] = ab[((long long)n * G + g) * 2] * inv_cnt;
+        pb[k] = ab[((long long)n * G + g) * 2 + 1] * inv_cnt;
+        dr[k] = chan_scale ? chan_scale[(long long)n * COUT + c] : 1.f;
+    }
+    const int prow = threadIdx.x >> 3;
+    int buf = 0;
+    const int t0 = blockIdx.x * tiles_per_wg, t1 = min(tiles, t0 + tiles_per_wg);
+    for (int t = t0; t < t1; ++t) {
+        const int row0 = t * UN_ROWS;
+        Vec16<bf16> a[NKC];
+        up_load_a<CIN>(Xn, row0 + wave * 16 + r, Vin, kg, a);
+        const int v0 = row0 + prow, v1 = v0 + 32;
+        const bool ok0 = v0 < Vin, ok1 = v1 < Vin;
+        const long long b0 = ok0 ? pp.base(n, v0, Di, Hi, Wi) : 0, b1 = ok1 ? pp.base(n, v1, Di, Hi, Wi) : 0;
+#pragma unroll UNR
+        for (int jg = 0; jg < NG; ++jg) {
+            const long long to = pp.tap_off(jg, Hi, Wi);
+            Vec16<bf16> g0v, g1v;
+            g0v.v = g1v.v = decltype(g0v.v){};
+            if (ok0) g0v = ld16(GY + b0 + to);
+            if (ok1) g1v = ld16(GY + b1 + to);
+            f32x4 acc[4];
+            up_group<CIN>(a, Wf, jg, lane, acc);
+            up_stage<CIN>(acc, bv, Ot[buf], wave, lane);
+            __syncthreads();
+#pragma unroll
+            for (int h = 0; h < 2; ++h) {
+                if (!(h ? ok1 : ok0)) continue;
+                const Vec16<bf16> x = ld16(Ot[buf] + (prow + 32 * h) * UN_OS + pp.pc * 8);
+                const Vec16<bf16>& gv = h ? g1v : g0v;
+                Vec16<bf16> o;
+#pragma unroll
+                for (int k = 0; k < 8; ++k) {
+                    const float xh = (x.get(k) - mu[k]) * rs[k];
+                    float g = gv.get(k) * dr[k];
+                    if (relu && !(gmv[k] * xh + btv[k] > 0.f)) g = 0.f;
+                    o.set(k, rs[k] * (gmv[k] * g - (pa[k] + xh * pb[k])));
+                }
+                st16(GZ + (h ? b1 : b0) + to, o);
+            }
+            buf ^= 1;
+        }
+    }
+}
+
+namespace {
+
+struct UpPlan { int Vin, tiles, chunks, tiles_per_chunk, tiles_per_wg, apply_wgs, stat_chunks, stat_rows; };
+
+bool up_served(int dtype, int Cin, int Cout, int G) {
+    return dtype == DYCON_BF16 && (Cin == 32 || Cin == 64) && Cout * 2 == Cin && (G == 16 || G == Cout);
+}
+
+UpPlan up_plan(int B, int Di, int Hi, int Wi) {
+    UpPlan p;
+    p.Vin = Di * Hi * Wi;
+    p.tiles = cdiv(p.Vin, UN_ROWS);
+    p.tiles_per_chunk = cdiv(p.tiles, UN_MAX_CHUNKS);
+    const int V = 8 * p.Vin;
+    p.stat_rows = cdiv(V, UN_MAX_CHUNKS) < 128 ? 128 : cdiv(V, UN_MAX_CHUNKS);
+    p.stat_chunks = cdiv(V, p.stat_rows);
+    p.chunks = cdiv(p.tiles, p.tiles_per_chunk);
+    const long long per = (long long)B * p.tiles / UN_APPLY_WGS;
+    p.tiles_per_wg = per < 1 ? 1 : per > 4 ? 4 : (int)per;
+    p.apply_wgs = cdiv(p.tiles, p.tiles_per_wg);
+    return p;
+}
+
+int up_check(const char* who, int dtype, int B, int Di, int Hi, int Wi, int Cin, int Cout, int G) {
+    DYCON_REQUIRE(B > 0 && Di > 0 && Hi > 0 && Wi > 0 && B <= 65535, "%s: bad shape (%d, %d, %d, %d)", who, B, Di, Hi, Wi);
+    DYCON_REQUIRE(8ll * Di * Hi * Wi < (1ll << 31) - 256, "%s: %d x %d x %d exceeds 2^31 output voxels per sample", who, Di, Hi, Wi);
+    DYCON_REQUIRE(up_served(dtype, Cin, Cout, G), "%s: %d -> %d channels in %d groups (dtype %d) is not served (ask dycon_upnorm_served)",
+                  who, Cin, Cout, G, dtype);
+    return DYCON_OK;
+}
+
+bool aligned16(const void* a, const void* b = nullptr, const void* c = nullptr, const void* d = nullptr, const void* e = nullptr) {
+    return (((uintptr_t)a | (uintptr_t)b | (uintptr_t)c | (uintptr_t)d | (uintptr_t)e) & 15) == 0;
+}
+
+}
+
+extern "C" int dycon_upnorm_served(int dtype, int Cin, int Cout, int G) { return up_served(dtype, Cin, Cout, G) ? 1 : 0; }
+
+extern "C" int dycon_upnorm_chunks(int Di, int Hi, int Wi) {
+    if (Di <= 0 || Hi <= 0 || Wi <= 0 || 8ll * Di * Hi * Wi >= (1ll << 31) - 256) return 0;
+    return up_plan(1, Di, Hi, Wi).chunks;
+}
+
+extern "C" int dycon_upnorm_stats_chunks(int Di, int Hi, int Wi) {
+    if (Di <= 0 || Hi <= 0 || Wi <= 0 || 8ll * Di * Hi * Wi >= (1ll << 31) - 256) return 0;
+    return up_plan(1, Di, Hi, Wi).stat_chunks;
+}
+
+extern "C" int dycon_upnorm_stats(const void* x, const void* wfrag, const float* bias, int dtype, int B, int Di, int Hi, int Wi,
+                                  int Cin, int Cout, int G, float* part, size_t part_bytes, dycon_stream_t stream) {
+    DYCON_REQUIRE(x && wfrag && part, "upnorm_stats: null pointer");
+    if (int e = up_check("upnorm_stats", dtype, B, Di, Hi, Wi, Cin, Cout, G)) return e;
+    DYCON_REQUIRE(aligned16(x, wfrag), "upnorm_stats: x and wfrag must be 16-byte aligned");
+    const UpPlan p = up_plan(B, Di, Hi, Wi);
+    DYCON_REQUIRE(part_bytes >= (size_t)B * p.stat_chunks * Cout * 2 * sizeof(float), "upnorm_stats: partials too small");
+    dim3 grid(p.stat_chunks, B);
+    if (Cin == 32) up_stats_kernel<32><<<grid, 256, 0, stream>>>((const bf16*)x, (const bf16*)wfrag, bias, part, p.Vin, Hi, Wi, p.stat_rows);
+    else up_stats_kernel<64><<<grid, 256, 0, stream>>>((const bf16*)x, (const bf16*)wfrag, bias, part, p.Vin, Hi, Wi, p.stat_rows);
+    DYCON_LAUNCH_CHECK();
+    return DYCON_OK;
+}
+
+extern "C" int dycon_upnorm_apply(const void* x, const void* wfrag, const float* bias, void* y, int dtype, int B, int Di, int Hi,
+                                  int Wi, int Cin, int Cout, int G, const float* stats, const float* gamma, const float* beta,
+                                  int relu, const void* skip, const float* chan_scale, dycon_stream_t stream) {
+    DYCON_REQUIRE(x && wfrag && y && stats, "upnorm_apply: null pointer");
+    if (int e = up_check("upnorm_apply", dtype, B, Di, Hi, Wi, Cin, Cout, G)) return e;
+    DYCON_REQUIRE(aligned16(x, wfrag, y, skip), "upnorm_apply: x, wfrag, y and skip must be 16-byte aligned");
+    const UpPlan p = up_plan(B, Di, Hi, Wi);
+    dim3 grid(p.apply_wgs, B);
+#define DYCON_UA(CI) up_apply_kernel<CI><<<grid, 256, 0, stream>>>((const bf16*)x, (const bf16*)wfrag, bias, (bf16*)y, p.Vin, Di, Hi, Wi, p.tiles, p.tiles_per_wg, G, stats, gamma, beta, relu, (const bf16*)skip, chan_scale)
+    if (Cin == 32) DYCON_UA(32); else DYCON_UA(64);
+#undef DYCON_UA
+    DYCON_LAUNCH_CHECK();
+    return DYCON_OK;
+}
+
+extern "C" int dycon_upnorm_bwd_stats(const void* x, const void* wfrag, const float* bias, const void* gy, int dtype, int B, int Di,
+                                      int Hi, int Wi, int Cin, int Cout, int G, const float* stats, const float* gamma,
+                                      const float* beta, int relu, const float* chan_scale, float* part, size_t part_bytes,
+                                      dycon_stream_t stream) {
+    DYCON_REQUIRE(x && wfrag && gy && stats && part, "upnorm_bwd_stats: null pointer");
+    if (int e = up_check("upnorm_bwd_stats", dtype, B, Di, Hi, Wi, Cin, Cout, G)) return e;
+    DYCON_REQUIRE(aligned16(x, wfrag, gy), "upnorm_bwd_stats: x, wfrag and gy must be 16-byte aligned");
+    const UpPlan p = up_plan(B, Di, Hi, Wi);
+    DYCON_REQUIRE(part_bytes >= (size_t)B * p.chunks * Cout * 2 * sizeof(float), "upnorm_bwd_stats: partials too small");
+    dim3 grid(p.chunks, B);
+#define DYCON_UBS(CI) up_bwd_stats_kernel<CI><<<grid, 256, 0, stream>>>((const bf16*)x, (const bf16*)wfrag, bias, (const bf16*)gy, part, p.Vin, Di, Hi, Wi, p.tiles, p.tiles_per_chunk, G, stats, gamma, beta, relu, chan_scale)
+    if (Cin == 32) DYCON_UBS(32); else DYCON_UBS(64);
+#undef DYCON_UBS
+    DYCON_LAUNCH_CHECK();
+    return DYCON_OK;
+}
+
+extern "C" int dycon_upnorm_bwd_apply(const void* x, const void* wfrag, const float* bias, const void* gy, void* gz, int dtype, int B,
+                                      int Di, int Hi, int Wi, int Cin, int Cout, int G, const float* stats, const float* gamma,
+                                      const float* beta, const float* ab, int relu, const float* chan_scale, dycon_stream_t stream) {
+    DYCON_REQUIRE(x && wfrag && gy && gz && stats && ab, "upnorm_bwd_apply: null pointer");
+    if (int e = up_check("upnorm_bwd_apply", dtype, B, Di, Hi, Wi, Cin, Cout, G)) return e;
+    DYCON_REQUIRE(aligned16(x, wfrag, gy, gz), "upnorm_bwd_apply: x, wfrag, gy and gz must be 16-byte aligned");
+    const UpPlan p = up_plan(B, Di, Hi, Wi);
+    dim3 grid(p.apply_wgs, B);
+#define DYCON_UBA(CI) up_bwd_apply_kernel<CI><<<grid, 256, 0, stream>>>((const bf16*)x, (const bf16*)wfrag, bias, (const bf16*)gy, (bf16*)gz, p.Vin, Di, Hi, Wi, p.tiles, p.tiles_per_wg, G, stats, gamma, beta, ab, relu, chan_scale)
+    if (Cin == 32) DYCON_UBA(32); else DYCON_UBA(64);
+#undef DYCON_UBA
+    DYCON_LAUNCH_CHECK();
+    return DYCON_OK;
+}
diff --git a/dycon_paper_replication_amd/engine.py b/dycon_paper_replication_amd/engine.py
--- a/dycon_paper_replication_amd/engine.py
+++ b/dycon_paper_replication_amd/engine.py
@@ -185,6 +185,8 @@
         self.fuse_finish = False
         self.conv_stats = False
         self.conv_stats96 = False
+        self.fuse_up = False
+        self.fuse_up_train = False
         self._stat_parts = {}
         self._deferred = {}
         self._pending_dparams = []
@@ -363,59 +365,96 @@
                 y = ops.conv_gemm(x, wf, b, mode, Cout, Cout)
 
         if self.recording:
-            def wgrad(gy):
-                gw, gb = self.g[name + ".weight"], self.g[name + ".bias"]
-                wkey = (name, tuple(x.shape[:4]))
-                ws = self._wws.get(wkey)
-                if kind == "deconv":
-                    if ws is None:
-                        ws = self._wws[wkey] = (ops._ws(ops.query("dycon_colsum_workspace", gy.numel() // gy.shape[-1], gy.shape[-1]), gy),
-                                                ops.conv_wgrad_workspace(gy, x, CONV_K2S2))
-                    ops.colsum(gy, gb, ws=ws[0])
-                    ops.conv_wgrad(gy, x, gw, CONV_K2S2, 1, 8, Cout * 8, ws=ws[1])
-                else:
-                    if ws is None:
-                        ws = self._wws[wkey] = ops.conv_wgrad_workspace(x, gy, mode)
-                    ops.conv_wgrad(x, gy, gw, mode, 1 if T > 1 else 0, T, Cin * T, dbias=gb, ws=ws)
-                if self.on_param_grads is not None:
-                    self.on_param_grads(name + ".weight")
-
+            def bwd():
+                self._conv_bwd(name, x, self._take(y), kind, need_gx, skinny)
+            self.tape.append(bwd)
+        return y
+
+    def _conv_bwd(self, name, x, gy, kind, need_gx, skinny):
+        w = self.p[name + ".weight"]
+        if kind == "deconv":
+            Cin, Cout = w.shape[0], w.shape[1]
+        else:
+            Cout, Cin = w.shape[0], w.shape[1]
+        T = {"k3": 27, "k2s2": 8, "deconv": 8, "1x1": 1}[kind]
+        mode = {"k3": CONV_K3, "k2s2": CONV_K2S2, "deconv": CONV_1X1, "1x1": CONV_1X1}[kind]
+
+        def wgrad(gy):
+            gw, gb = self.g[name + ".weight"], self.g[name + ".bias"]
+            wkey = (name, tuple(x.shape[:4]))
+            ws = self._wws.get(wkey)
+            if kind == "deconv":
+                if ws is None:
+                    ws = self._wws[wkey] = (ops._ws(ops.query("dycon_colsum_workspace", gy.numel() // gy.shape[-1], gy.shape[-1]), gy),
+                                            ops.conv_wgrad_workspace(gy, x, CONV_K2S2))
+                ops.colsum(gy, gb, ws=ws[0])
+                ops.conv_wgrad(gy, x, gw, CONV_K2S2, 1, 8, Cout * 8, ws=ws[1])
+            else:
+                if ws is None:
+                    ws = self._wws[wkey] = ops.conv_wgrad_workspace(x, gy, mode)
+                ops.conv_wgrad(x, gy, gw, mode, 1 if T > 1 else 0, T, Cin * T, dbias=gb, ws=ws)
+            if self.on_param_grads is not None:
+                self.on_param_grads(name + ".weight")
+
+        if self.wgrad_stream is not None:
+            wst = self.wgrad_stream
+            if self.wgrad_stream2 is not None:
+                self._wg_flip = (self._wg_flip + 1) % 2
+                wst = (self.wgrad_stream, self.wgrad_stream2)[self._wg_flip]
+            ops.fork(ops.cur_stream(), wst)
+            with ops.on_stream(wst, light=True):
+                self._flush_dparams()
+                wgrad(gy)
+            gy.record_stream(wst)
+        else:
+            wgrad(gy)
+        if not need_gx:
+            return
+        cur = self._peek(x)
+        if skinny:
+            wd = self._pk((name, "tcn_d"), "tcn", w, 1, Cout, Cin, Cin, 0, Cin, 0, 1)
+            gx = ops.conv_direct(gy, wd, None, CONV_1X1, Cin, x.dtype, out=cur, accumulate=cur is not None)
+        elif kind == "k3":
+            if ops.conv_plan_for(gy, CONV_K3, Cin, Cin).weights == CONV_W_CHUNK16:
+                wd = self._pk_chunked16((name, "d48"), w, 3, Cin, 1, Cin * 27, 27, flip=True)
+            else:
+                wd = self._pk((name, "d"), "frag", w, 27, Cout, Cin, Cin, 1, Cin * 27, 0, 27, flip=True)
+            gx = ops.conv_gemm(gy, wd, None, CONV_K3, Cin, Cin, out=cur, accumulate=cur is not None)
+        elif kind == "k2s2":
+            wd = self._pk((name, "d"), "frag", w, 1, Cout, 8 * Cin, Cin, 0, Cin * 8, 1, 8)
+            gx = ops.conv_gemm(gy, wd, None, CONV_1X1, 8 * Cin, Cin, scatter=True, out=cur, accumulate=cur is not None)
+        elif kind == "deconv":
+            wd = self._pk((name, "d"), "frag", w, 8, Cout, Cin, Cin, 1, 8, 0, Cout * 8)
+            gx = ops.conv_gemm(gy, wd, None, CONV_K2S2, Cin, Cin, out=cur, accumulate=cur is not None)
+        else:
+            wd = self._pk((name, "d"), "frag", w, 1, Cout, Cin, Cin, 0, Cin, 0, 1)
+            gx = ops.conv_gemm(gy, wd, None, CONV_1X1, Cin, Cin, out=cur, accumulate=cur is not None)
+        self._put(x, gx)
+
+    def _up_block(self, name, t, skip, kind, training):
+        cname, nname = f"{name}.conv.0", f"{name}.conv.1"
+        w, b = self.p[cname + ".weight"], self.p[cname + ".bias"]
+        Cin, Cout = w.shape[0], w.shape[1]
+        G = 16 if kind == "gn" else Cout
+        V = 8 * t.shape[1] * t.shape[2] * t.shape[3]
+        if not ((self.fuse_up_train if self.recording else self.fuse_up) and kind in ("gn", "in") and self.dtype == torch.bfloat16 and t.dtype == torch.bfloat16
+                and ops.upnorm_served(t, Cout, G) and not ops.norm_fwd_is_fused(t, V, Cout, G)):
+            return self._norm(nname, self._conv(cname, t, "deconv"), kind, skip=skip, training=training)
+        gamma, beta = (self.p[nname + ".weight"], self.p[nname + ".bias"]) if kind == "gn" else (None, None)
+        wf = self._pk((cname, "f"), "frag", w, 1, Cin, 8 * Cout, Cout, 0, Cout * 8, 1, 8)
+        stats = ops.upnorm_stats(t, wf, b, Cout, G, ops.upnorm_workspace(t, Cout, G))
+        y = ops.upnorm_apply(t, wf, b, Cout, G, stats, gamma, beta, True, skip)
+        if self.recording:
             def bwd():
                 gy = self._take(y)
-                if self.wgrad_stream is not None:
-                    wst = self.wgrad_stream
-                    if self.wgrad_stream2 is not None:
-                        self._wg_flip = (self._wg_flip + 1) % 2
-                        wst = (self.wgrad_stream, self.wgrad_stream2)[self._wg_flip]
-                    ops.fork(ops.cur_stream(), wst)
-                    with ops.on_stream(wst, light=True):
-                        self._flush_dparams()
-                        wgrad(gy)
-                    gy.record_stream(wst)
-                else:
-                    wgrad(gy)
-                if not need_gx:
-                    return
-                cur = self._peek(x)
-                if skinny:
-                    wd = self._pk((name, "tcn_d"), "tcn", w, 1, Cout, Cin, Cin, 0, Cin, 0, 1)
-                    gx = ops.conv_direct(gy, wd, None, CONV_1X1, Cin, x.dtype, out=cur, accumulate=cur is not None)
-                elif kind == "k3":
-                    if ops.conv_plan_for(gy, CONV_K3, Cin, Cin).weights == CONV_W_CHUNK16:
-                        wd = self._pk_chunked16((name, "d48"), w, 3, Cin, 1, Cin * 27, 27, flip=True)
-                    else:
-                        wd = self._pk((name, "d"), "frag", w, 27, Cout, Cin, Cin, 1, Cin * 27, 0, 27, flip=True)
-                    gx = ops.conv_gemm(gy, wd, None, CONV_K3, Cin, Cin, out=cur, accumulate=cur is not None)
-                elif kind == "k2s2":
-                    wd = self._pk((name, "d"), "frag", w, 1, Cout, 8 * Cin, Cin, 0, Cin * 8, 1, 8)
-                    gx = ops.conv_gemm(gy, wd, None, CONV_1X1, 8 * Cin, Cin, scatter=True, out=cur, accumulate=cur is not None)
-                elif kind == "deconv":
-                    wd = self._pk((name, "d"), "frag", w, 8, Cout, Cin, Cin, 1, 8, 0, Cout * 8)
-                    gx = ops.conv_gemm(gy, wd, None, CONV_K2S2, Cin, Cin, out=cur, accumulate=cur is not None)
-                else:
-                    wd = self._pk((name, "d"), "frag", w, 1, Cout, Cin, Cin, 0, Cin, 0, 1)
-                    gx = ops.conv_gemm(gy, wd, None, CONV_1X1, Cin, Cin, out=cur, accumulate=cur is not None)
-                self._put(x, gx)
+                if skip is not None:
+                    self._give(skip, gy)
+                dg = self.g[nname + ".weight"] if gamma is not None else None
+                db = self.g[nname + ".bias"] if beta is not None else None
+                gz = ops.upnorm_bwd(t, wf, b, gy, Cout, G, stats, ops.upnorm_workspace(t, Cout, G), gamma, beta, True, dg, db)
+                if self.on_param_grads is not None and gamma is not None:
+                    self.on_param_grads(nname + ".weight")
+                self._conv_bwd(cname, t, gz, "deconv", True, False)
             self.tape.append(bwd)
         return y
 
@@ -793,7 +832,7 @@
                               training=training)
 
         def up(name, t, skip):
-            return self._norm(f"{name}.conv.1", self._conv(f"{name}.conv.0", t, "deconv"), nk, skip=skip, training=training)
+            return self._up_block(name, t, skip, nk, training)
 
         if self._fuses_first_block(x, nk, training):
             x1 = self._first_block("block_one", x, nk, training)
diff --git a/dycon_paper_replication_amd/ops.py b/dycon_paper_replication_amd/ops.py
--- a/dycon_paper_replication_amd/ops.py
+++ b/dycon_paper_replication_amd/ops.py
@@ -497,6 +497,58 @@
     call("dycon_norm_sum_dparams", _p(ws), Nb, C, _p(dgamma), _p(dbeta), _s())
 
 
+def upnorm_served(x, Cout, G):
+    return bool(query("dycon_upnorm_served", dt(x), x.shape[-1], Cout, G))
+
+
+def upnorm_workspace(x, Cout, G):
+    B, D, H, W, _ = x.shape
+    chunks = max(query("dycon_upnorm_chunks", D, H, W), query("dycon_upnorm_stats_chunks", D, H, W))
+    return _ws((B * chunks * Cout + B * G) * 2 * 4, x)
+
+
+def _upnorm_geo(x, Cout):
+    B, D, H, W, Cin = x.shape
+    nz = B * D * H * W * 8 * Cout * _es(x)
+    return B, D, H, W, Cin, query("dycon_upnorm_chunks", D, H, W), x.numel() * _es(x) + Cin * 8 * Cout * _es(x), nz
+
+
+def upnorm_stats(x, wfrag, bias, Cout, G, ws, eps=1e-5):
+    B, D, H, W, Cin, _, nx, nz = _upnorm_geo(x, Cout)
+    chunks = query("dycon_upnorm_stats_chunks", D, H, W)
+    stats = torch.empty(B * G * 2, dtype=torch.float32, device=x.device)
+    with _Region("upnorm_stats", nx, 2 * 8 * B * D * H * W * Cin * 8 * Cout + 3 * (nz // _es(x))):
+        call("dycon_upnorm_stats", _p(x), _p(wfrag), _p(bias), dt(x), B, D, H, W, Cin, Cout, G, _p(ws), ws.numel() * 4, _s())
+        call("dycon_norm_stats_parts", dt(x), B, 8 * D * H * W, Cout, G, eps, _p(stats), None, None, 0.1, _p(ws), chunks, _s())
+    return stats
+
+
+def upnorm_apply(x, wfrag, bias, Cout, G, stats, gamma=None, beta=None, relu=True, skip=None, chan_scale=None, out=None):
+    B, D, H, W, Cin, _, nx, nz = _upnorm_geo(x, Cout)
+    if out is None:
+        out = torch.empty((B, 2 * D, 2 * H, 2 * W, Cout), dtype=x.dtype, device=x.device)
+    with _Region("upnorm_apply", nx + nz * (2 if skip is not None else 1), 2 * B * D * H * W * Cin * 8 * Cout + 3 * out.numel()):
+        call("dycon_upnorm_apply", _p(x), _p(wfrag), _p(bias), _p(out), dt(x), B, D, H, W, Cin, Cout, G, _p(stats), _p(gamma), _p(beta),
+             int(relu), _p(skip), _p(chan_scale), _s())
+    return out
+
+
+def upnorm_bwd(x, wfrag, bias, gy, Cout, G, stats, ws, gamma=None, beta=None, relu=True, dgamma=None, dbeta=None, chan_scale=None, out=None):
+    B, D, H, W, Cin, chunks, nx, nz = _upnorm_geo(x, Cout)
+    if out is None:
+        out = torch.empty_like(gy)
+    ab = ws[B * chunks * Cout * 2:]
+    mm = 2 * B * D * H * W * Cin * 8 * Cout
+    with _Region("upnorm_bwd", 2 * nx + 3 * nz, 2 * mm + 12 * gy.numel(),
+                 parts=[("up_bwd_stats", nx + nz, mm + 6 * gy.numel()), ("up_bwd_apply", nx + 2 * nz, mm + 6 * gy.numel())]):
+        call("dycon_upnorm_bwd_stats", _p(x), _p(wfrag), _p(bias), _p(gy), dt(x), B, D, H, W, Cin, Cout, G, _p(stats), _p(gamma), _p(beta),
+             int(relu), _p(chan_scale), _p(ws), ws.numel() * 4, _s())
+        call("dycon_norm_bwd_parts", B, Cout, G, _p(gamma), _p(ws), chunks, _p(ab), _p(dgamma), _p(dbeta), _s())
+        call("dycon_upnorm_bwd_apply", _p(x), _p(wfrag), _p(bias), _p(gy), _p(out), dt(x), B, D, H, W, Cin, Cout, G, _p(stats), _p(gamma),
+             _p(beta), _p(ab), int(relu), _p(chan_scale), _s())
+    return out
+
+
 def maxpool2_fwd(x):
     B, D, H, W, C = x.shape
     y = torch.empty((B, D // 2, H // 2, W // 2, C), dtype=x.dtype, device=x.device)
diff --git a/include/dycon_hip.h b/include/dycon_hip.h
--- a/include/dycon_hip.h
+++ b/include/dycon_hip.h
@@ -167,6 +167,23 @@
                         dycon_stream_t stream);
 int dycon_upconv_k3(const void* x, const void* wfrag, const float* bias, void* y, int dtype, int B,
                     int Di, int Hi, int Wi, int Cin, int Cout, dycon_stream_t stream);
+int dycon_upnorm_served(int dtype, int Cin, int Cout, int G);
+int dycon_upnorm_chunks(int Di, int Hi, int Wi);
+int dycon_upnorm_stats_chunks(int Di, int Hi, int Wi);
+int dycon_upnorm_stats(const void* x, const void* wfrag, const float* bias, int dtype, int B, int Di, int Hi, int Wi,
+                       int Cin, int Cout, int G, float* part, size_t part_bytes, dycon_stream_t stream);
+int dycon_upnorm_apply(const void* x, const void* wfrag, const float* bias, void* y, int dtype, int B, int Di, int Hi,
+                       int Wi, int Cin, int Cout, int G, const float* stats, const float* gamma, const float* beta,
+                       int relu, const void* skip, const float* chan_scale, dycon_stream_t stream);
+int dycon_upnorm_bwd_stats(const void* x, const void* wfrag, const float* bias, const void* gy, int dtype, int B, int Di,
+                           int Hi, int Wi, int Cin, int Cout, int G, const float* stats, const float* gamma,
+                           const float* beta, int relu, const float* chan_scale, float* part, size_t part_bytes,
+                           dycon_stream_t stream);
+int dycon_norm_bwd_parts(int Nb, int C, int G, const float* gamma, const float* part, int chunks, float* ab, float* dgamma,
+                         float* dbeta, dycon_stream_t stream);
+int dycon_upnorm_bwd_apply(const void* x, const void* wfrag, const float* bias, const void* gy, void* gz, int dtype, int B,
+                           int Di, int Hi, int Wi, int Cin, int Cout, int G, const float* stats, const float* gamma,
+                           const float* beta, const float* ab, int relu, const float* chan_scale, dycon_stream_t stream);
 int dycon_copy_channels(const void* src, int lds, int soff, void* dst, int ldd, int doff,
                         long long rows, int C, int dtype, dycon_stream_t stream);
 int dycon_relu_fwd(const void* z, const void* skip, const float* chan_scale, void* y, int dtype, int B, long long V, int C,
```
